# snuspl/rnb

Measured on AMD Instinct MI355X. Metric: videos/sec (whole node) + p50/p99 end-to-end latency, R(2+1)D-34 8-frame clips, higher is better.
Workload: dtype fp32

## Files before the change

csrc/conv_h3.hip:

```cpp
#include <type_traits>
#include <hip/hip_runtime.h>
#include <stdint.h>

#include "x6d_common.h"

#include "h3_common.h"

#ifdef H3_PHASE_TIMING
__device__ unsigned long long* h3_phase_buf;
#define H3_PHASE(k)                                                                   \
  do {                                                                                \
    if (threadIdx.x == 0 && (k) < 16) {                                               \
      h3_phase_buf[(size_t)blockIdx.x * 16 + (k)] = __builtin_amdgcn_s_memtime();     \
      if ((k) == 0) {                                                                 \
        unsigned hw, xcc;                                                             \
        asm volatile("s_getreg_b32 %0, hwreg(HW_REG_HW_ID)" : "=s"(hw));              \
        asm volatile("s_getreg_b32 %0, hwreg(HW_REG_XCC_ID)" : "=s"(xcc));            \
        h3_phase_buf[(size_t)blockIdx.x * 16 + 14] = ((unsigned long long)xcc << 32) | hw; \
      }                                                                               \
    }                                                                                 \
  } while (0)
#else
#define H3_PHASE(k) do {} while (0)
#endif
// ... 188 lines not shown

  const int nsteps16 = p.K_pad / 16;
  int s_begin = 0, s_end = nsteps16;
  if (p.KH == 1 && p.KW == 1 && p.KT > 1) {
    int n0, t0, n1, t1, hh, ww;
    f32_decode_row(p, p0, n0, t0, hh, ww);
    f32_decode_row(p, min(p0 + P_TILE, p.M) - 1, n1, t1, hh, ww);
    n0 = __builtin_amdgcn_readfirstlane(n0);
    n1 = __builtin_amdgcn_readfirstlane(n1);
    t0 = __builtin_amdgcn_readfirstlane(t0);
    t1 = __builtin_amdgcn_readfirstlane(t1);
    if (n0 == n1) {
      const int dt_lo = max(0, p.PT - t1 * p.ST);
      const int dt_hi = min(p.KT - 1, p.T - 1 + p.PT - t0 * p.ST);
      if (dt_hi >= dt_lo) {
        s_begin = (dt_lo * p.Cin_p) / 16;
        s_end = min(nsteps16, ((dt_hi + 1) * p.Cin_p + 15) / 16);
      }
    }
  }
  int t_begin = s_begin / 2, t_end = (s_end + 1) / 2;
  if (ksplit > 1) {
    const int len = t_end - t_begin;
    const int a = t_begin + (int)((long long)len * kidx / ksplit);
    const int b = t_begin + (int)((long long)len * (kidx + 1) / ksplit);
    t_begin = a;
    t_end = b;
  }
  const bool sums_mode = AFF && st.aff.sums != nullptr;
  if (t_begin < t_end) issue(t_begin, 0, !sums_mode);
  if constexpr (AFF) {
    if (sums_mode) {
      constexpr int NT = 64 * NW;
      constexpr int KG = (H3_AFF_SUMS_MAX + NT - 1) / NT;
      constexpr int KL = (H3_AFF_CLIPS * 64 + NT - 1) / NT;
      const int E = st.aff.nseg * p.Cin_p;
      double a1[KG + KL], a2[KG + KL];
      float gm[KG + KL], bt[KG + KL];
      int rows[KG + KL], dst[KG + KL];
#pragma unroll
      for (int k = 0; k < KG + KL; ++k) {
        int v = -1, c = 0;
        dst[k] = -1;
        if (k < KG) {
          const int i = threadIdx.x + k * NT;
          if (i < E) {
            v = i / p.Cin_p;
            c = i - v * p.Cin_p;
            dst[k] = i;
          }
        } else if (t_begin < t_end) {
          const int j = threadIdx.x + (k - KG) * NT;
          const int ci = j >> 6, sub = (j >> 5) & 1, ch = j & 15;
          const int clip = clip_lo + ci;
          if (j < H3_AFF_CLIPS * 64) {
            dst[k] = -2 - j;
            if (clip < p.N && clip * rows_per_clip < p0 + P_TILE) {
              v = st.in_seg[clip];
              c = ((2 * t_begin + sub) * 16) % p.Cin_p + ch;
            }
          }
        }
        const double* sp = st.aff.sums + (size_t)(v < 0 ? 0 : v) * 2 * st.aff.sums_c;
        a1[k] = v >= 0 ? sp[c] : 0.0;
        a2[k] = v >= 0 ? sp[st.aff.sums_c + c] : 0.0;
        gm[k] = v >= 0 ? st.aff.gamma[c] : 0.f;
        bt[k] = v >= 0 ? st.aff.beta[c] : 0.f;
        rows[k] = v >= 0 ? (st.aff.coffs[v + 1] - st.aff.coffs[v]) * st.aff.rpc : 0;
      }
      float* ssw = const_cast<float*>(st.in_ss);
      float* l0 = (float*)(lds + ACT_BYTES + W_BYTES);
#pragma unroll
      for (int k = 0; k < KG + KL; ++k) {
        if (dst[k] == -1) continue;
        float mu = 0.f, va = 0.f;
        if (rows[k] > 0) {
          const double m = a1[k] / (double)rows[k];
          mu = (float)m;
          va = (float)fmax(a2[k] / (double)rows[k] - m * m, 0.0);
        }
        const float sc = rows[k] > 0 ? gm[k] * rsqrtf(va + st.aff.eps) : 0.f;
        const float sh = rows[k] > 0 ? bt[k] - mu * sc : 0.f;
        if (dst[k] >= 0) {
          const int v = dst[k] / p.Cin_p, c = dst[k] - v * p.Cin_p;
          ssw[(size_t)v * 2 * p.Cin_p + c] = sc;
          ssw[(size_t)v * 2 * p.Cin_p + p.Cin_p + c] = sh;
        } else {
          const int j = -2 - dst[k];
          l0[j] = ((j >> 4) & 1) ? sh : sc;
        }
      }
    }
  }
  if (wave >= NW / 2) __builtin_amdgcn_s_setprio(1);
  x6d_wait_vm<0>();
  x6d_barrier();
  for (int t = t_begin; t < t_end; ++t) {
    const int it = t - t_begin;
    if (t + 1 < t_end) issue(t + 1, (it + 1) & 1);
    if constexpr (AFF) {
      const __attribute__((address_space(4))) int* tab =
          (const __attribute__((address_space(4))) int*)(p.ktab + t * 8);
      ey_cur[0] = tab[1];
      ey_cur[1] = tab[9];
    }
    H3B bf[TP];
#pragma unroll
    for (int tp = 0; tp < TP; ++tp) bf[tp] = load_b(it & 1, tp);
#pragma unroll
    for (int tc = 0; tc < TC; ++tc) mma_tc(it & 1, tc, bf);
    x6d_wait_vm<0>();
    x6d_barrier();
  }

  const float out_scale = st.out_scale;
#pragma unroll
  for (int tp = 0; tp < TP; ++tp)
#pragma unroll
    for (int tc = 0; tc < TC; ++tc) acc[tp][tc] *= out_scale;
  if (ksplit > 1) {
    const uint32_t ws_bytes = (uint32_t)min((long long)ksplit * p.M * p.Cout_p * 4, 0x7FFFFF00LL);
    const __amdgpu_buffer_rsrc_t wsr =
        __builtin_amdgcn_make_buffer_rsrc((void*)st.ws, (short)0, ws_bytes, 0x00020000);
#pragma unroll
    for (int tp = 0; tp < TP; ++tp) {
      const int m = p0 + (wp * TP + tp) * 16 + frow;
#pragma unroll
      for (int tc = 0; tc < TC; ++tc) {
        const int c = c0 + (wc * TC + tc) * 16 + 4 * fq;
        const uint32_t off = (m < p.M && c < p.Cout_p)
                                 ? (uint32_t)((((long long)kidx * p.M + m) * p.Cout_p + c) * 4)
                                 : X6D_INVALID;
        __builtin_amdgcn_raw_buffer_store_b128(acc[tp][tc], wsr, off, 0, 0);
      }
    }
    return;
  }
  x6d_epilogue<TP, TC, NW, C_TILE, ST>(p, st, acc, p0, p.M, p0 + P_TILE, c0, wp, wc, lane, lds,
                                       NS * BUF);
}

struct H3Band {
  int f, r0;
  int rows;
  int prows;
  int g0, u0;
  bool mixed;
};
template <bool ON>
static __device__ __forceinline__ int h3_per_chunk(int v) {
  if constexpr (ON) asm volatile("" : "+v"(v));
  return v;
}
template <bool STK, bool AFF>
static __device__ __forceinline__ void h3_patch_entry(const ConvF32Params& p, const H3Band& bd,
                                                      int it, int npx, int W2, int qd, int n0,
                                                      uint32_t& src, int& dst) {
  const int H = p.H, W = p.W;
  const int q = it >> 2;
  const int hy = q / W2, hx = q - hy * W2;
  const int x = hx - 1;
  int fy = bd.f, y = bd.r0 - 1 + hy;
  bool ok = it < 4 * npx && x >= 0 && x < W;
  if constexpr (STK) {
    const int u = bd.u0 - 1 + hy;
    fy = f32_fast_div(max(u, 0), p.mG, p.sG);
    y = u - fy * (H + 1);
    ok = ok && u >= 0 && y < H && fy < p.N * p.T;
  } else {
    ok = ok && y >= 0 && y < H;
  }
  src = ok ? (uint32_t)((((fy * H + y) * W + x) * p.Cin_p + qd * 4) * 4) : X6D_INVALID;
  dst = it < 4 * npx ? q * 128 : -1;
  if constexpr (STK && AFF) {
    if (ok) dst |= (f32_fast_div(fy, p.mTo, p.sTo) - n0) << 17;
  }
}
template <bool STK>
static __device__ __forceinline__ int h3_patch_pixel(const ConvF32Params& p, const H3Band& bd,
                                                     int pp, int R, int W2) {
  const int W = p.W;
  const int py = pp / W;
  if constexpr (STK) {
    const int hy = py + f32_fast_div(bd.g0 + py, p.mHo, p.sHo) - bd.f;
    return pp < bd.rows * W ? hy * W2 + (pp - py * W) : 0;
  } else {
    return pp < R * W ? py * W2 + (pp - py * W) : 0;
  }
}
static __device__ __forceinline__ void h3_entry_ss(const ConvF32Params& p, const X6DStats& st,
                                                   int n0, int d, int qd, int chunk,
                                                   x6f32x4& sc0, x6f32x4& sc1, x6f32x4& sh0,
                                                   x6f32x4& sh1) {
  const float* ss = st.in_ss + qd * 4 + chunk * 32 +
                    (size_t)st.in_seg[n0 + (d >> 17)] * 2 * p.Cin_p;
  sc0 = *(const x6f32x4*)ss;
  sc1 = *(const x6f32x4*)(ss + 16);
  sh0 = *(const x6f32x4*)(ss + p.Cin_p);
  sh1 = *(const x6f32x4*)(ss + p.Cin_p + 16);
}
template <bool STK, bool AFF>
static __device__ __forceinline__ H3Band h3_band(const ConvF32Params& p, const X6DStats& st,
                                                 int band, int R) {
  H3Band b;
  if constexpr (STK) {
    b.g0 = band * R;
    b.f = f32_fast_div(b.g0, p.mHo, p.sHo);
    b.r0 = b.g0 - b.f * p.H;
    b.rows = min(R, p.N * p.T * p.H - b.g0);
    const int fl = f32_fast_div(b.g0 + b.rows - 1, p.mHo, p.sHo);
    b.u0 = b.g0 + b.f;
    b.prows = b.rows + 2 + (fl - b.f);
    b.mixed = false;
    if constexpr (AFF)
      b.mixed = st.in_seg[f32_fast_div(b.f, p.mTo, p.sTo)] !=
                st.in_seg[f32_fast_div(fl, p.mTo, p.sTo)];
  } else {
    const int bands = (p.H + R - 1) / R;
    b.f = band / bands;
    b.r0 = (band - b.f * bands) * R;
    b.rows = min(R, p.H - b.r0);
    b.prows = R + 2;
    b.g0 = b.u0 = 0;
    b.mixed = false;
  }
  return b;
}

template <int NW, int TP, int TC, int HALO_PX, int G, bool ST, bool AFF, int MINB = 1,
          bool STK = false>
__global__ __launch_bounds__(64 * NW, MINB)
void conv_h3r_kernel(const ConvF32Params p, const X6DStats st) {
  constexpr int P_TILE = NW * TP * 16, C_TILE = TC * 16;
  constexpr int HALO_BYTES = HALO_PX * 128;
  constexpr int W_BYTES = C_TILE * 128;
  constexpr int W_TOTAL = C_TILE / 8;
  constexpr int W_INSTR = (W_TOTAL + NW - 1) / NW;
  constexpr int NT = 64 * NW;
  constexpr int ITEMS = (HALO_PX * 4 + NT - 1) / NT;
  static_assert(NT % 4 == 0, "a lane keeps one channel quad");
  __shared__ __attribute__((aligned(16))) char lds[HALO_BYTES + 2 * G * W_BYTES];
  char* const wbuf = lds + HALO_BYTES;

  const int lane = threadIdx.x & 63;
  const int wave = __builtin_amdgcn_readfirstlane(threadIdx.x >> 6);
  const int frow = lane & 15, fq = lane >> 4;
  const int W = p.W, H = p.H, W2 = p.W + 2;
  const int R = p.ST;

  const int nwg = gridDim.x, bid = blockIdx.x;
  const int q8 = nwg >> 3, r8 = nwg & 7, xcd = bid & 7;
  const int wgid = (xcd < r8 ? xcd * (q8 + 1) : r8 * (q8 + 1) + (xcd - r8) * q8) + (bid >> 3);
  const int ctile = wgid % p.n_ctiles;
  const int band = wgid / p.n_ctiles;
  const H3Band bd = h3_band<STK, AFF>(p, st, band, R);
  const int f = bd.f, r0 = bd.r0;
  const int c0 = ctile * C_TILE;
  const int p0 = (f * H + r0) * W;
  const int m_end = p0 + bd.rows * W;
  const int nck = p.Cin_p / 32;

  const x6d_u32x4 wr = x6d_rsrc(p.w, (uint32_t)(p.K_pad / 32) * (uint32_t)p.w_rows * 128u);
  auto issue_w = [&](int s, int buf) {
    const uint32_t wbase = ((uint32_t)s * (uint32_t)p.w_rows + (uint32_t)c0) * 128u;
#pragma unroll
    for (int j = 0; j < W_INSTR; ++j) {
      const int instr = (W_TOTAL % NW == 0) ? wave + NW * j : min(wave + NW * j, W_TOTAL - 1);
      x6d_dma16(wr, wbase + (uint32_t)(instr * 1024 + lane * 16),
                wbuf + buf * W_BYTES + instr * 1024);
    }
  };

  const __amdgpu_buffer_rsrc_t xr =
      __builtin_amdgcn_make_buffer_rsrc((void*)p.x, (short)0, p.x_bytes, 0x00020000);
  const int npx = bd.prows * W2;
  const int qd = threadIdx.x & 3;
  uint32_t src[ITEMS];
  int dst[ITEMS];
  static_assert(HALO_BYTES <= 1 << 17, "dst packs the entry's clip above bit 17");
  [[maybe_unused]] const int n0 = f32_fast_div(f, p.mTo, p.sTo);
#pragma unroll
  for (int i = 0; i < ITEMS; ++i) {
    h3_patch_entry<STK, AFF>(p, bd, threadIdx.x + i * NT, npx, W2, qd, n0, src[i], dst[i]);
  }
  const float* ssv = nullptr;
  if constexpr (AFF) ssv = st.in_ss + (size_t)st.in_seg[f / p.T] * 2 * p.Cin_p + qd * 4;
  const float in_scale = st.in_scale;
  constexpr int SB = MINB >= 4 ? 1 : AFF ? (NW > 8 ? 1 : (TP >= 4 ? 3 : ITEMS)) : ITEMS;
  auto stage = [&](int chunk, auto mix) {
    constexpr bool MIX = decltype(mix)::value;
    x6f32x4 sc0, sh0, sc1, sh1;
    if constexpr (AFF) {
      const float* ss = ssv + chunk * 32;
      sc0 = *(const x6f32x4*)ss;
      sc1 = *(const x6f32x4*)(ss + 16);
      sh0 = *(const x6f32x4*)(ss + p.Cin_p);
      sh1 = *(const x6f32x4*)(ss + p.Cin_p + 16);
    }
#pragma unroll
    for (int i0 = 0; i0 < ITEMS; i0 += SB) {
    x6f32x4 v0[SB], v1[SB];
#pragma unroll
    for (int k = 0; k < SB; ++k) {
      const int i = min(i0 + k, ITEMS - 1);
      const uint32_t o = src[i] == X6D_INVALID ? X6D_INVALID : src[i] + (uint32_t)(chunk * 128);
      v0[k] = __builtin_amdgcn_raw_buffer_load_b128(xr, o, 0, 0);
      v1[k] = __builtin_amdgcn_raw_buffer_load_b128(xr, o == X6D_INVALID ? o : o + 64u, 0, 0);
    }
#pragma unroll
    for (int k = 0; k < SB; ++k) {
      const int i = i0 + k;
      if (i >= ITEMS || dst[i] < 0) continue;
      const int d = h3_per_chunk<STK && AFF>(dst[i]), q = (d >> 7) & 1023;
      x6f32x4 a0 = v0[k], a1 = v1[k];
      if constexpr (AFF) {
        const float m = src[i] == X6D_INVALID ? 0.f : in_scale;
        if constexpr (MIX) h3_entry_ss(p, st, n0, d, qd, chunk, sc0, sc1, sh0, sh1);
#pragma unroll
        for (int j = 0; j < 4; ++j) {
          a0[j] = fmaxf(fmaf(a0[j], sc0[j], sh0[j]), 0.f) * m;
          a1[j] = fmaxf(fmaf(a1[j], sc1[j], sh1[j]), 0.f) * m;
        }
      } else {
        a0 *= in_scale;
        a1 *= in_scale;
      }
      uint32_t h[4], l[4];
      h3_split4(a0, h, l);
      h3_split4(a1, h + 2, l + 2);
      char* base = lds + (d & 0x1FFFF);
      *(wu32x4*)(base + (x6r_swz(2 * qd, q) << 4)) = (wu32x4){h[0], h[1], h[2], h[3]};
      *(wu32x4*)(base + (x6r_swz(2 * qd + 1, q) << 4)) = (wu32x4){l[0], l[1], l[2], l[3]};
    }
    }
  };

  int pq[TP];
#pragma unroll
  for (int tp = 0; tp < TP; ++tp) {
    const int pp = (wave * TP + tp) * 16 + frow;
    pq[tp] = h3_patch_pixel<STK>(p, bd, pp, R, W2);
  }

  x6f32x4 acc[TP][TC];
#pragma unroll
  for (int b = 0; b < TC; ++b) {
    const int c = c0 + b * 16 + 4 * fq;
    const float4 b4 = *(const float4*)(p.bias + c);
    const x6f32x4 bv = (x6f32x4){b4.x, b4.y, b4.z, b4.w} * st.acc_scale;
#pragma unroll
    for (int a = 0; a < TP; ++a) acc[a][b] = bv;
  }
  const int w_hh = x6_chunk(2 * fq, frow) << 4, w_ll = x6_chunk(2 * fq + 1, frow) << 4;

  constexpr int NG = (9 + G - 1) / G;
  auto issue_group = [&](int c, int g, int half) {
    for (int j = 0; j < G && g * G + j < 9; ++j) issue_w((g * G + j) * nck + c, half * G + j);
  };
  if (wave >= NW / 2) __builtin_amdgcn_s_setprio(1);
  H3_PHASE(0);
  issue_group(0, 0, 0);
  int half = 0;
  for (int c = 0; c < nck; ++c) {
    if constexpr (STK && AFF) {
      if (bd.mixed) stage(c, std::true_type{});
      else stage(c, std::false_type{});
    } else {
      stage(c, std::false_type{});
    }
    x6d_wait_vm<0>();
    x6d_barrier();
    H3_PHASE(1 + 2 * c);
#pragma unroll 1
    for (int g = 0; g < NG; ++g) {
      if (g + 1 < NG) issue_group(c, g + 1, half ^ 1);
      else if (c + 1 < nck) issue_group(c + 1, 0, half ^ 1);
      for (int j = 0; j < G && g * G + j < 9; ++j) {
        const int t = g * G + j;
        const int toff = (t / 3) * W2 + (t % 3);
        H3B bf[TP];
#pragma unroll
        for (int tp = 0; tp < TP; ++tp) {
          const int q = pq[tp] + toff;
          const char* base = lds + q * 128;
          bf[tp].h = *(const wu32x4*)(base + (x6r_swz(2 * fq, q) << 4));
          bf[tp].l = *(const wu32x4*)(base + (x6r_swz(2 * fq + 1, q) << 4));
        }
        const char* wb = wbuf + (half * G + j) * W_BYTES;
#pragma unroll
        for (int tc = 0; tc < TC; ++tc) {
          const char* wrow = wb + (tc * 16 + frow) * 128;
          const wu32x4 ah = *(const wu32x4*)(wrow + w_hh);
          const wu32x4 al = *(const wu32x4*)(wrow + w_ll);
#pragma unroll
          for (int tp = 0; tp < TP; ++tp) acc[tp][tc] = h3_mma(al, bf[tp].h, acc[tp][tc]);
#pragma unroll
          for (int tp = 0; tp < TP; ++tp) acc[tp][tc] = h3_mma(ah, bf[tp].l, acc[tp][tc]);
#pragma unroll
          for (int tp = 0; tp < TP; ++tp) acc[tp][tc] = h3_mma(ah, bf[tp].h, acc[tp][tc]);
        }
      }
      x6d_wait_vm<0>();
      x6d_barrier();
      half ^= 1;
    }
    H3_PHASE(2 + 2 * c);
  }
  x6d_epilogue<TP, TC, NW, C_TILE, ST, STK>(p, st, acc, p0, m_end, p0 + P_TILE, c0, wave, 0,
                                            lane, lds, HALO_BYTES + 2 * G * W_BYTES,
                                            st.out_scale);
  H3_PHASE(15);
}

template <int NW, int TP, int HALO_PX, int G, int MINB, bool ST, bool AFF, bool STK = false>
__global__ __launch_bounds__(64 * NW, MINB)
void conv_h3q_kernel(const ConvF32Params p, const X6DStats st) {
  constexpr int TC = 9;
  constexpr int P_TILE = NW * TP * 16, C_TILE = TC * 16;
  constexpr int HALO_BYTES = HALO_PX * 128;
  constexpr int W_BYTES = C_TILE * 128;
  constexpr int W_TOTAL = C_TILE / 8;
  constexpr int W_INSTR = (W_TOTAL + NW - 1) / NW;
  constexpr int NT = 64 * NW;
  constexpr int ITEMS = (HALO_PX * 4 + NT - 1) / NT;
  static_assert(TP <= TC - 1, "next-tap fragments are read during channel tiles 1..TP");
  __shared__ __attribute__((aligned(16))) char lds[HALO_BYTES + 2 * G * W_BYTES];
  char* const wbuf = lds + HALO_BYTES;

  const int lane = threadIdx.x & 63;
  const int wave = __builtin_amdgcn_readfirstlane(threadIdx.x >> 6);
  const int frow = lane & 15, fq = lane >> 4;
  const int W = p.W, H = p.H, W2 = p.W + 1;
  const int R = p.ST;

  const int nwg = gridDim.x, bid = blockIdx.x;
  const int q8 = nwg >> 3, r8 = nwg & 7, xcd = bid & 7;
  const int wgid = (xcd < r8 ? xcd * (q8 + 1) : r8 * (q8 + 1) + (xcd - r8) * q8) + (bid >> 3);
  const int ctile = wgid % p.n_ctiles;
  const int band = wgid / p.n_ctiles;
  const H3Band bd = h3_band<STK, AFF>(p, st, band, R);
  const int f = bd.f, r0 = bd.r0;
  const int c0 = ctile * C_TILE;
  const int p0 = (f * H + r0) * W;
  const int m_end = p0 + bd.rows * W;
  const int nck = p.Cin_p / 32;

  const x6d_u32x4 wr = x6d_rsrc(p.w, (uint32_t)(p.K_pad / 32) * (uint32_t)p.w_rows * 128u);
  auto issue_w = [&](int s, int buf) {
    const uint32_t wbase = ((uint32_t)s * (uint32_t)p.w_rows + (uint32_t)c0) * 128u;
#pragma unroll
    for (int j = 0; j < W_INSTR; ++j) {
      const int instr = (W_TOTAL % NW == 0) ? wave + NW * j : min(wave + NW * j, W_TOTAL - 1);
      x6d_dma16(wr, wbase + (uint32_t)(instr * 1024 + lane * 16),
                wbuf + buf * W_BYTES + instr * 1024);
    }
  };

  const __amdgpu_buffer_rsrc_t xr =
      __builtin_amdgcn_make_buffer_rsrc((void*)p.x, (short)0, p.x_bytes, 0x00020000);
  const int npx = bd.prows * W2 + 1;
  const int qd = threadIdx.x & 3;
  uint32_t src[ITEMS];
  int dst[ITEMS];
  static_assert(HALO_BYTES <= 1 << 17, "dst packs the entry's clip above bit 17");
  [[maybe_unused]] const int n0 = f32_fast_div(f, p.mTo, p.sTo);
#pragma unroll
  for (int i = 0; i < ITEMS; ++i) {
    h3_patch_entry<STK, AFF>(p, bd, threadIdx.x + i * NT, npx, W2, qd, n0, src[i], dst[i]);
  }
  const float* ssv = nullptr;
  if constexpr (AFF) ssv = st.in_ss + (size_t)st.in_seg[f / p.T] * 2 * p.Cin_p + qd * 4;
  const float in_scale = st.in_scale;
  constexpr int SB = AFF ? (NW == 4 && MINB == 1 ? 5 : 2) : 5;
  auto stage = [&](int chunk, auto mix) {
    constexpr bool MIX = decltype(mix)::value;
    x6f32x4 sc0, sh0, sc1, sh1;
    if constexpr (AFF) {
      const float* ss = ssv + chunk * 32;
      sc0 = *(const x6f32x4*)ss;
      sc1 = *(const x6f32x4*)(ss + 16);
      sh0 = *(const x6f32x4*)(ss + p.Cin_p);
      sh1 = *(const x6f32x4*)(ss + p.Cin_p + 16);
    }
#pragma unroll
    for (int i0 = 0; i0 < ITEMS; i0 += SB) {
      x6f32x4 v0[SB], v1[SB];
#pragma unroll
      for (int k = 0; k < SB; ++k) {
        const int i = min(i0 + k, ITEMS - 1);
        const uint32_t o = src[i] == X6D_INVALID ? X6D_INVALID : src[i] + (uint32_t)(chunk * 128);
        v0[k] = __builtin_amdgcn_raw_buffer_load_b128(xr, o, 0, 0);
        v1[k] = __builtin_amdgcn_raw_buffer_load_b128(xr, o == X6D_INVALID ? o : o + 64u, 0, 0);
      }
#pragma unroll
      for (int k = 0; k < SB; ++k) {
        const int i = i0 + k;
        if (i >= ITEMS || dst[i] < 0) continue;
        const int d = h3_per_chunk<STK && AFF>(dst[i]), q = (d >> 7) & 1023;
        x6f32x4 a0 = v0[k], a1 = v1[k];
        if constexpr (AFF) {
          const float m = src[i] == X6D_INVALID ? 0.f : in_scale;
          if constexpr (MIX) h3_entry_ss(p, st, n0, d, qd, chunk, sc0, sc1, sh0, sh1);
#pragma unroll
          for (int j = 0; j < 4; ++j) {
            a0[j] = fmaxf(fmaf(a0[j], sc0[j], sh0[j]), 0.f) * m;
            a1[j] = fmaxf(fmaf(a1[j], sc1[j], sh1[j]), 0.f) * m;
          }
        } else {
          a0 *= in_scale;
          a1 *= in_scale;
        }
        uint32_t h[4], l[4];
        h3_split4(a0, h, l);
        h3_split4(a1, h + 2, l + 2);
        char* base = lds + (d & 0x1FFFF);
        *(wu32x4*)(base + (x6r_swz(2 * qd, q) << 4)) = (wu32x4){h[0], h[1], h[2], h[3]};
        *(wu32x4*)(base + (x6r_swz(2 * qd + 1, q) << 4)) = (wu32x4){l[0], l[1], l[2], l[3]};
      }
    }
  };

  int pq[TP];
#pragma unroll
  for (int tp = 0; tp < TP; ++tp) {
    const int pp = (wave * TP + tp) * 16 + frow;
    pq[tp] = h3_patch_pixel<STK>(p, bd, pp, R, W2);
  }

  x6f32x4 acc[TP][TC];
#pragma unroll
  for (int b = 0; b < TC; ++b) {
    const int c = c0 + b * 16 + 4 * fq;
    const float4 b4 = *(const float4*)(p.bias + c);
    const x6f32x4 bv = (x6f32x4){b4.x, b4.y, b4.z, b4.w} * st.acc_scale;
#pragma unroll
    for (int a = 0; a < TP; ++a) acc[a][b] = bv;
  }
  const int w_hh = x6_chunk(2 * fq, frow) << 4, w_ll = x6_chunk(2 * fq + 1, frow) << 4;
  auto rd_bf = [&](H3B& b, int tap, int tp) {
    const int q = pq[tp] + (tap / 3) * W2 + (tap % 3);
    const char* base = lds + q * 128;
    b.h = *(const wu32x4*)(base + (x6r_swz(2 * fq, q) << 4));
    b.l = *(const wu32x4*)(base + (x6r_swz(2 * fq + 1, q) << 4));
  };
  auto rd_w = [&](wu32x4& ah, wu32x4& al, int jslot, int tc) {
    const char* wrow = wbuf + jslot * W_BYTES + (tc * 16 + frow) * 128;
    ah = *(const wu32x4*)(wrow + w_hh);
    al = *(const wu32x4*)(wrow + w_ll);
  };

  constexpr int NG = (9 + G - 1) / G;
  auto issue_group = [&](int c, int g, int half) {
    for (int j = 0; j < G && g * G + j < 9; ++j) issue_w((g * G + j) * nck + c, half * G + j);
  };
  H3_PHASE(0);
  issue_group(0, 0, 0);
  int half = 0;
  for (int c = 0; c < nck; ++c) {
    if constexpr (STK && AFF) {
      if (bd.mixed) stage(c, std::true_type{});
      else stage(c, std::false_type{});
    } else {
      stage(c, std::false_type{});
    }
    x6d_wait_vm<0>();
    x6d_barrier();
    H3_PHASE(1 + 2 * c);
#pragma unroll 1
    for (int g = 0; g < NG; ++g) {
      if (g + 1 < NG) issue_group(c, g + 1, half ^ 1);
      else if (c + 1 < nck) issue_group(c + 1, 0, half ^ 1);
      const int t0 = g * G;
      H3B bf[2][TP];
      wu32x4 wh[2], wl[2];
#pragma unroll
      for (int tp = 0; tp < TP; ++tp) rd_bf(bf[0][tp], t0, tp);
      rd_w(wh[0], wl[0], half * G, 0);
#pragma unroll
      for (int j = 0; j < G; ++j) {
        if (t0 + j >= 9) break;
        const bool more = j + 1 < G && t0 + j + 1 < 9;
#pragma unroll
        for (int tc = 0; tc < TC; ++tc) {
          const int cs = (j * TC + tc) & 1;
          if (tc + 1 < TC) rd_w(wh[cs ^ 1], wl[cs ^ 1], half * G + j, tc + 1);
          else if (more) rd_w(wh[cs ^ 1], wl[cs ^ 1], half * G + j + 1, 0);
          if (more && tc >= 1 && tc <= TP) rd_bf(bf[(j + 1) & 1][tc - 1], t0 + j + 1, tc - 1);
          const H3B (&b)[TP] = bf[j & 1];
#pragma unroll
          for (int tp = 0; tp < TP; ++tp) acc[tp][tc] = h3_mma(wl[cs], b[tp].h, acc[tp][tc]);
#pragma unroll
          for (int tp = 0; tp < TP; ++tp) acc[tp][tc] = h3_mma(wh[cs], b[tp].l, acc[tp][tc]);
#pragma unroll
          for (int tp = 0; tp < TP; ++tp) acc[tp][tc] = h3_mma(wh[cs], b[tp].h, acc[tp][tc]);
          __builtin_amdgcn_sched_barrier(0);
        }
      }
      x6d_wait_vm<0>();
      x6d_barrier();
      half ^= 1;
    }
    H3_PHASE(2 + 2 * c);
  }
  x6d_epilogue<TP, TC, NW, C_TILE, ST, STK>(p, st, acc, p0, m_end, p0 + P_TILE, c0, wave, 0,
                                            lane, lds, HALO_BYTES + 2 * G * W_BYTES,
                                            st.out_scale);
  H3_PHASE(15);
}

template <int NW, int TP, int TC, int HALO, int WB, int MINB, bool ST, bool AFF, int STK = 0>
__global__ __launch_bounds__(64 * NW, MINB)
void conv_h3t_kernel(const ConvF32Params p, const X6DStats st) {
  constexpr int ROWS = NW * TP * 16, C_TILE = TC * 16;
  static_assert(!STK || HALO == ROWS, "stacked: the patch is the block's T x P rows");
  constexpr int HALO_BYTES = HALO * 128;
  constexpr int TAP_BYTES = C_TILE * 128;
  constexpr int W_BYTES = 3 * TAP_BYTES;
  constexpr int W_TOTAL = W_BYTES / 1024;
  constexpr int W_INSTR = (W_TOTAL + NW - 1) / NW;
  constexpr int NT = 64 * NW;
  constexpr int ITEMS = (HALO * 4 + NT - 1) / NT;
  static_assert(NT % 4 == 0 && TAP_BYTES % 1024 == 0, "staging / DMA split");
  static_assert(TP <= TC * 3 - 1, "next-tap fragments are read during the channel tiles");
  __shared__ __attribute__((aligned(16))) char lds[HALO_BYTES + WB * W_BYTES];
  char* const wbuf = lds + HALO_BYTES;

  const int lane = threadIdx.x & 63;
  const int wave = __builtin_amdgcn_readfirstlane(threadIdx.x >> 6);
  const int frow = lane & 15, fq = lane >> 4;
  const int T = p.T, HW = p.H * p.W, P = p.ngroups;
  const int nck = (p.Cin_p + 31) / 32;

  const int nwg = gridDim.x, bid = blockIdx.x;
  const int q8 = nwg >> 3, r8 = nwg & 7, xcd = bid & 7;
  const int wgid = (xcd < r8 ? xcd * (q8 + 1) : r8 * (q8 + 1) + (xcd - r8) * q8) + (bid >> 3);
  const int ctile = wgid % p.n_ctiles;
  const int rest = wgid / p.n_ctiles;
  const int ptile = rest % p.n_ptiles;
  const int n = rest / p.n_ptiles;
  const int c0 = ctile * C_TILE, hw0 = ptile * P;

  const x6d_u32x4 wr = x6d_rsrc(p.w, (uint32_t)(p.K_pad / 32) * (uint32_t)p.w_rows * 128u);
  auto issue_w = [&](int c, int buf) {
#pragma unroll
    for (int j = 0; j < W_INSTR; ++j) {
      const int instr = (W_TOTAL % NW == 0) ? wave + NW * j : min(wave + NW * j, W_TOTAL - 1);
      const int k = instr / (TAP_BYTES / 1024), part = instr % (TAP_BYTES / 1024);
      const uint32_t s = (uint32_t)(k * nck + c);
      x6d_dma16(wr, (s * (uint32_t)p.w_rows + (uint32_t)c0) * 128u +
                        (uint32_t)(part * 1024 + lane * 16),
                wbuf + buf * W_BYTES + instr * 1024);
    }
  };

  const __amdgpu_buffer_rsrc_t xr =
      __builtin_amdgcn_make_buffer_rsrc((void*)p.x, (short)0, p.x_bytes, 0x00020000);
  const int nent = (T + 2) * P;
  const int qd = threadIdx.x & 3;
  uint32_t src[ITEMS];
  int dst[ITEMS];
  [[maybe_unused]] const int NG = p.N * HW, lgP = 31 - __clz(P);
  [[maybe_unused]] int n0 = 0, n1 = 0;
  [[maybe_unused]] bool mixed = false;
  if constexpr (STK) {
    n0 = __builtin_amdgcn_readfirstlane(f32_fast_div(hw0, p.mG, p.sG));
    n1 = __builtin_amdgcn_readfirstlane(f32_fast_div(min(hw0 + P, NG) - 1, p.mG, p.sG));
    if constexpr (AFF) mixed = st.in_seg[n0] != st.in_seg[n1];
#pragma unroll
// ... 473 lines not shown
                   const float* gamma, const float* beta, float eps, float* ss) {
  if (!sums || !coffs || !gamma || !beta || !ss) return -1;
  if (nseg <= 0 || C <= 0 || sums_c < C || rpc <= 0) return -2;
  BnAffSums a = {};
  a.sums = sums; a.sums_c = sums_c; a.nseg = nseg; a.rpc = rpc; a.coffs = coffs;
  a.gamma = gamma; a.beta = beta; a.eps = eps; a.ss = ss;
  g_bn_aff = a;
  g_bn_aff_used = 0;
  return 0;
}
void rnb_bn_aff_disarm() { g_bn_aff.ss = nullptr; }
int rnb_bn_aff_used() {
  const int u = g_bn_aff_used;
  g_bn_aff_used = 0;
  return u;
}

void rnb_h3_set_range_flag(int* flag) { g_h3_range_flag = flag; }
int* rnb_h3_range_flag() { return g_h3_range_flag; }

int rnb_conv_h3_num_configs() { return kNumH3Configs; }

int rnb_conv_h3_config_info(int id, int* p_tile, int* c_tile) {
  if (id < 0 || id >= kNumH3Configs) return -1;
  *p_tile = kH3Configs[id].p_tile;
  *c_tile = kH3Configs[id].c_tile;
  return 0;
}

int rnb_conv_h3_affine_ok(int config_id, int cin_p, int rows_per_clip) {
  if (config_id < 0 || config_id >= kNumH3Configs || cin_p % 16 != 0 || rows_per_clip <= 0)
    return 0;
  const int pt = kH3Configs[config_id].p_tile;
  return (pt - 1) / rows_per_clip + 2 <= H3_AFF_CLIPS ? 1 : 0;
}

int rnb_conv_h3_launch(const ConvF32Params* pp, int config_id, hipStream_t stream, double* sums,
                       const int* clip_seg, int stats_c, int ksplit, float* ws, float in_scale,
                       float out_scale, const float* in_ss, const int* in_seg) {
  if (config_id < 0 || config_id >= kNumH3Configs) return -1;
  ConvF32Params p = *pp;
  const ConvH3Config& cfg = kH3Configs[config_id];
  if (p.Cin_p % 4 != 0 || p.Cout_p % 4 != 0 || p.K_pad % 32 != 0) return -2;
  if (p.K_total > p.K_pad) return -3;
  if (p.M <= 0) return 0;
  if (p.y_stride < p.Cout_p || (p.res && p.res_stride < p.Cout_p)) return -4;
  if (p.y_stride % 4 != 0 || (p.res && p.res_stride % 4 != 0)) return -4;
  const long long xb = (long long)p.N * p.T * p.H * p.W * p.Cin_p * 4;
  if (xb > 0x7FFFFF00LL) return -5;
  if ((long long)p.M * p.y_stride * 4 > 0x7FFFFF00LL) return -6;
  if (p.res && (long long)p.M * p.res_stride * 4 > 0x7FFFFF00LL) return -6;
  if (p.KT > 8 || p.KH > 8 || p.KW > 8) return -10;
  if ((long long)(p.K_pad / 32) * p.w_rows * 128 > 0x7FFFFF00LL) return -11;
  if (!(in_scale > 0.f) || !(out_scale > 0.f)) return -15;
  p.x_bytes = (uint32_t)xb;
  f32_magic_div((uint32_t)p.Wo, &p.mWo, &p.sWo);
  f32_magic_div((uint32_t)p.Ho, &p.mHo, &p.sHo);
  f32_magic_div((uint32_t)p.To, &p.mTo, &p.sTo);
  p.row_mode = 0;
  p.n_ptiles = (p.M + cfg.p_tile - 1) / cfg.p_tile;
  p.n_ctiles = (p.Cout_p + cfg.c_tile - 1) / cfg.c_tile;
  const long long blocks = (long long)p.n_ptiles * p.n_ctiles;
  if (blocks > 0x7FFFFFFF) return -7;
  if (p.n_ctiles * cfg.c_tile > p.w_rows) return -8;
  if (!p.ktab) return -9;
  if (sums && (!clip_seg || stats_c < p.Cout_p)) return -12;
  X6DStats st;
  st.sums = sums;
  st.clip_seg = clip_seg;
  st.stats_c = stats_c;
  st.ksplit = 1;
  st.ws = nullptr;
  st.in_scale = in_scale;
  st.out_scale = out_scale;
  st.acc_scale = 1.f / out_scale;
  st.in_ss = in_ss;
  st.in_seg = in_seg;
  st.oflag = g_h3_range_flag;
  const bool aff = in_ss != nullptr;
  if (aff && (!in_seg || !rnb_conv_h3_affine_ok(config_id, p.Cin_p, p.To * p.Ho * p.Wo)))
    return -16;
  if (aff && g_bn_aff.ss == in_ss) {
    if (g_bn_aff.sums_c < p.Cin_p || (long long)g_bn_aff.nseg * p.Cin_p > H3_AFF_SUMS_MAX)
      return -18;
    st.aff = g_bn_aff;
    g_bn_aff_used = 1;
  }
  if (ksplit > 1) {
    if (!ws || ksplit > 16) return -14;
    st.ksplit = ksplit;
    st.ws = ws;
    hipLaunchKernelGGL(aff ? cfg.kernel_aff : cfg.kernel, dim3((unsigned)(blocks * ksplit)),
                       dim3(cfg.threads), 0, stream, p, st);
    return rnb_x6d_splitk_reduce(&p, &st, stream);
  }
  hipLaunchKernelGGL(aff ? (sums ? cfg.kernel_aff_st : cfg.kernel_aff)
                         : (sums ? cfg.kernel_st : cfg.kernel),
                     dim3((unsigned)blocks), dim3(cfg.threads), 0, stream, p, st);
  return (int)hipGetLastError();
}

typedef void (*ConvH3RKernel)(const ConvF32Params, const X6DStats);
struct ConvH3RConfig {
  int nw, tp, halo_px, q;
  ConvH3RKernel kernel[4];
  int halo_stk;
  ConvH3RKernel stacked[4];
};
#define H3RCFGM(NW, TP, HALO, G, MINB)                                             \
  {NW, TP, HALO, 0,                                                                \
   {conv_h3r_kernel<NW, TP, 9, HALO, G, false, false, MINB>,                       \
    conv_h3r_kernel<NW, TP, 9, HALO, G, true, false, MINB>,                        \
    conv_h3r_kernel<NW, TP, 9, HALO, G, false, true, MINB>,                        \
    conv_h3r_kernel<NW, TP, 9, HALO, G, true, true, MINB>},                        \
   HALO,                                                                           \
   {conv_h3r_kernel<NW, TP, 9, HALO, G, false, false, MINB, true>,                 \
    conv_h3r_kernel<NW, TP, 9, HALO, G, true, false, MINB, true>,                  \
    conv_h3r_kernel<NW, TP, 9, HALO, G, false, true, MINB, true>,                  \
    conv_h3r_kernel<NW, TP, 9, HALO, G, true, true, MINB, true>}}
#define H3RCFG(NW, TP, HALO, G) H3RCFGM(NW, TP, HALO, G, 1)
#define H3RCFG_PF(NW, TP, HALO, G)                                                 \
  {NW, TP, HALO, 0,                                                                \
   {conv_h3r_kernel<NW, TP, 9, HALO, G, false, false, 1>,                          \
    conv_h3r_kernel<NW, TP, 9, HALO, G, true, false, 1>,                           \
    conv_h3r_kernel<NW, TP, 9, HALO, G, false, true, 1>,                           \
    conv_h3r_kernel<NW, TP, 9, HALO, G, true, true, 1>},                           \
   0, {nullptr, nullptr, nullptr, nullptr}}
#define H3QCFG(NW, TP, HALO, HSTK, G, MINB)                                        \
  {NW, TP, HALO, 1,                                                                \
   {conv_h3q_kernel<NW, TP, HALO, G, MINB, false, false>,                          \
    conv_h3q_kernel<NW, TP, HALO, G, MINB, true, false>,                           \
    conv_h3q_kernel<NW, TP, HALO, G, MINB, false, true>,                           \
    conv_h3q_kernel<NW, TP, HALO, G, MINB, true, true>},                           \
   HSTK,                                                                           \
   {conv_h3q_kernel<NW, TP, HSTK, G, MINB, false, false, true>,                    \
    conv_h3q_kernel<NW, TP, HSTK, G, MINB, true, false, true>,                     \
    conv_h3q_kernel<NW, TP, HSTK, G, MINB, false, true, true>,                     \
    conv_h3q_kernel<NW, TP, HSTK, G, MINB, true, true, true>}}
#define H3QCFG_PF(NW, TP, HALO, G, MINB)                                           \
  {NW, TP, HALO, 1,                                                                \
   {conv_h3q_kernel<NW, TP, HALO, G, MINB, false, false>,                          \
    conv_h3q_kernel<NW, TP, HALO, G, MINB, true, false>,                           \
    conv_h3q_kernel<NW, TP, HALO, G, MINB, false, true>,                           \
    conv_h3q_kernel<NW, TP, HALO, G, MINB, true, true>},                           \
   0, {nullptr, nullptr, nullptr, nullptr}}
static const ConvH3RConfig kH3RConfigs[] = {
    H3RCFG(7, 4, 600, 1), H3RCFG_PF(14, 2, 600, 1), H3RCFG(7, 3, 480, 1),
    H3RCFG(7, 4, 600, 2), H3RCFG_PF(14, 2, 600, 2), H3RCFG(7, 3, 480, 2),
    H3QCFG(4, 7, 600, 600, 2, 1),
    H3QCFG(4, 4, 344, 352, 1, 2),
    H3QCFG_PF(8, 4, 640, 2, 1),
};

int rnb_conv_h3r_num_variants() { return (int)(sizeof(kH3RConfigs) / sizeof(kH3RConfigs[0])); }

static long long h3r_round_blocks(int variant) {
  static long long cache[16] = {};
  if (variant < 0 || variant >= 16) return 0;
  if (cache[variant] == 0) {
    int dev = 0, cus = 0, nb = 0;
    const ConvH3RConfig& cfg = kH3RConfigs[variant];
    if (hipGetDevice(&dev) == hipSuccess &&
        hipDeviceGetAttribute(&cus, hipDeviceAttributeMultiprocessorCount, dev) == hipSuccess &&
        hipOccupancyMaxActiveBlocksPerMultiprocessor(&nb, (const void*)cfg.kernel[0],
                                                     64 * cfg.nw, 0) == hipSuccess)
      cache[variant] = (long long)cus * nb;
    else
      (void)hipGetLastError();
    if (cache[variant] <= 0) cache[variant] = -1;
  }
  return cache[variant] > 0 ? cache[variant] : 0;
}

static int g_h3r_stack_small = 0;
void rnb_conv_h3r_stack_small(int on) { g_h3r_stack_small = on; }

static int h3r_rows(int variant, int H, int W, long long frames, int n_ctiles, bool* stacked) {
  const ConvH3RConfig& cfg = kH3RConfigs[variant];
  *stacked = false;
  if (H < 1 || W < 1) return 0;
  const int pitch = cfg.q ? W + 1 : W + 2, extra = cfg.q ? 1 : 0;
  const int R0 = cfg.nw * cfg.tp * 16 / W;
  const bool fits0 = R0 >= 1 && (R0 + 2) * pitch + extra <= cfg.halo_px;
  int R = R0;
  while (R >= 1 && (R + 2 + (R + H - 2) / H) * pitch + extra > cfg.halo_stk) --R;
  if (fits0 && (R < 1 || (H + R0 - 1) / R0 * R <= H)) return R0;
  if (fits0 && frames > 0 && !g_h3r_stack_small &&
      frames * ((H + R0 - 1) / R0) * n_ctiles <= h3r_round_blocks(variant))
    return R0;
  *stacked = R >= 1;
  return R >= 1 ? R : 0;
}

int rnb_conv_h3r_band_rows(int variant, int H, int W) {
  if (variant < 0 || variant >= rnb_conv_h3r_num_variants()) return 0;
  bool stacked;
  const int R = h3r_rows(variant, H, W, 0, 1, &stacked);
  return stacked ? R : (R < H ? R : H);
}

int rnb_conv_h3r_stacked(int variant, int N, int T, int H, int W, int Cout_p) {
  if (variant < 0 || variant >= rnb_conv_h3r_num_variants()) return 0;
  bool stacked;
  h3r_rows(variant, H, W, (long long)N * T, (Cout_p + 143) / 144, &stacked);
  return stacked ? 1 : 0;
}

int rnb_conv_h3r_pixels(int variant) {
  if (variant < 0 || variant >= rnb_conv_h3r_num_variants()) return 0;
  return kH3RConfigs[variant].nw * kH3RConfigs[variant].tp * 16;
}

long long rnb_conv_h3r_blocks(int variant, int N, int T, int H, int W, int Cout_p) {
  if (variant < 0 || variant >= rnb_conv_h3r_num_variants()) return 0;
  bool stacked;
  const long long frames = (long long)N * T;
  const int n_ctiles = (Cout_p + 143) / 144;
  const int R = h3r_rows(variant, H, W, frames, n_ctiles, &stacked);
  if (R == 0) return 0;
  const long long bands = stacked ? (frames * H + R - 1) / R : frames * ((H + R - 1) / R);
  return bands * n_ctiles;
}

int rnb_conv_h3r_occupancy(int variant, int stacked) {
  if (variant < 0 || variant >= rnb_conv_h3r_num_variants()) return -1;
  const ConvH3RConfig& cfg = kH3RConfigs[variant];
  int nb = 0;
  if (stacked && !cfg.stacked[0]) return -1;
  const hipError_t e = hipOccupancyMaxActiveBlocksPerMultiprocessor(
      &nb, (const void*)(stacked ? cfg.stacked[0] : cfg.kernel[0]), 64 * cfg.nw, 0);
  return e == hipSuccess ? nb : -(int)e;
}

int rnb_conv_h3r_launch(const ConvF32Params* pp, int variant, hipStream_t stream, double* sums,
                        const int* clip_seg, int stats_c, float in_scale, float out_scale,
                        const float* in_ss, const int* in_seg) {
  if (variant < 0 || variant >= rnb_conv_h3r_num_variants()) return -1;
  ConvF32Params p = *pp;
  const ConvH3RConfig& cfg = kH3RConfigs[variant];
  if (p.KT != 1 || p.KH != 3 || p.KW != 3 || p.PH != 1 || p.PW != 1 || p.PT != 0) return -2;
  if (p.SH != 1 || p.SW != 1 || p.ST != 1 || p.Cin_p % 32 != 0 || p.Cout_p % 4 != 0) return -2;
  if (p.K_pad < 9 * p.Cin_p || p.K_pad % 32 != 0) return -3;
  if (p.M <= 0) return 0;
  if (p.y_stride < p.Cout_p || p.y_stride % 4 != 0 || (p.res && (p.res_stride < p.Cout_p ||
                                                               p.res_stride % 4 != 0)))
    return -4;
  const long long xb = (long long)p.N * p.T * p.H * p.W * p.Cin_p * 4;
  if (xb > 0x7FFFFF00LL || (long long)p.M * p.y_stride * 4 > 0x7FFFFF00LL) return -5;
  if (p.res && (long long)p.M * p.res_stride * 4 > 0x7FFFFF00LL) return -6;
  bool stacked;
  const int R = h3r_rows(variant, p.H, p.W, (long long)p.N * p.T, (p.Cout_p + 143) / 144,
                         &stacked);
  if (R == 0) return -13;
  if ((long long)(p.K_pad / 32) * p.w_rows * 128 > 0x7FFFFF00LL) return -11;
  if (!(in_scale > 0.f) || !(out_scale > 0.f)) return -15;
  if (in_ss && !in_seg) return -16;
  p.x_bytes = (uint32_t)xb;
  f32_magic_div((uint32_t)p.Wo, &p.mWo, &p.sWo);
  f32_magic_div((uint32_t)p.Ho, &p.mHo, &p.sHo);
  f32_magic_div((uint32_t)p.To, &p.mTo, &p.sTo);
  f32_magic_div((uint32_t)p.H + 1u, &p.mG, &p.sG);
  p.ST = R;
  p.n_ctiles = (p.Cout_p + 143) / 144;
  if (p.n_ctiles * 144 > p.w_rows) return -8;
  const long long blocks = rnb_conv_h3r_blocks(variant, p.N, p.T, p.H, p.W, p.Cout_p);
  if (blocks > 0x7FFFFFFF) return -7;
  if (sums && (!clip_seg || stats_c < p.Cout_p)) return -12;
  X6DStats st;
  st.sums = sums;
  st.clip_seg = clip_seg;
  st.stats_c = stats_c;
  st.ksplit = 1;
  st.ws = nullptr;
  st.in_scale = in_scale;
  st.out_scale = out_scale;
  st.acc_scale = 1.f / out_scale;
  st.in_ss = in_ss;
  st.in_seg = in_seg;
  st.oflag = g_h3_range_flag;
  const int kid = (sums ? 1 : 0) + (in_ss ? 2 : 0);
  hipLaunchKernelGGL(stacked ? cfg.stacked[kid] : cfg.kernel[kid], dim3((unsigned)blocks),
                     dim3(64 * cfg.nw), 0, stream, p, st);
  return (int)hipGetLastError();
}

struct ConvH3TConfig {
  int rows, c_tile, halo, nw;
  void (*kernel)(const ConvF32Params, const X6DStats);
  void (*kernel_st)(const ConvF32Params, const X6DStats);
  void (*kernel_aff)(const ConvF32Params, const X6DStats);
  void (*kernel_aff_st)(const ConvF32Params, const X6DStats);
  int tp;
  void (*stacked[3][4])(const ConvF32Params, const X6DStats);
};
#define H3TSTK(NW, TP, TC, WB, MINB, STK)                                           \
  {conv_h3t_kernel<NW, TP, TC, NW * TP * 16, WB, MINB, false, false, STK>,          \
   conv_h3t_kernel<NW, TP, TC, NW * TP * 16, WB, MINB, true, false, STK>,           \
   conv_h3t_kernel<NW, TP, TC, NW * TP * 16, WB, MINB, false, true, STK>,           \
   conv_h3t_kernel<NW, TP, TC, NW * TP * 16, WB, MINB, true, true, STK>}
#define H3TPC(NW, TP, TC, HALO, WB, MINB)                                           \
  NW * TP * 16, TC * 16, HALO, NW,                                                   \
   conv_h3t_kernel<NW, TP, TC, HALO, WB, MINB, false, false>,                       \
   conv_h3t_kernel<NW, TP, TC, HALO, WB, MINB, true, false>,                        \
   conv_h3t_kernel<NW, TP, TC, HALO, WB, MINB, false, true>,                        \
   conv_h3t_kernel<NW, TP, TC, HALO, WB, MINB, true, true>, TP
#define H3TCFG(NW, TP, TC, HALO, WB, MINB)                                          \
  {H3TPC(NW, TP, TC, HALO, WB, MINB),                                               \
   {H3TSTK(NW, TP, TC, WB, MINB, 1), H3TSTK(NW, TP, TC, WB, MINB, 2),               \
    H3TSTK(NW, TP, TC, WB, MINB, 3)}}
#define H3TCFG_TP2(NW, TC, HALO, WB, MINB)                                          \
  {H3TPC(NW, 2, TC, HALO, WB, MINB),                                                \
   {H3TSTK(NW, 2, TC, WB, MINB, 1), {nullptr, nullptr, nullptr, nullptr},           \
    H3TSTK(NW, 2, TC, WB, MINB, 3)}}
static const ConvH3TConfig kH3TConfigs[] = {
    H3TCFG(8, 4, 4, 768, 2, 1), H3TCFG_TP2(8, 4, 512, 2, 1), H3TCFG_TP2(8, 8, 512, 2, 1),
    H3TCFG(4, 4, 4, 384, 1, 2),
};

int rnb_conv_h3t_num_variants() { return (int)(sizeof(kH3TConfigs) / sizeof(kH3TConfigs[0])); }

int rnb_conv_h3t_pixels(int variant, int T) {
  if (variant < 0 || variant >= rnb_conv_h3t_num_variants() || T < 2) return 0;
  const ConvH3TConfig& cfg = kH3TConfigs[variant];
  if (cfg.rows % T) return 0;
  const int P = cfg.rows / T;
  return (P % 16 == 0 && (T + 2) * P <= cfg.halo) ? P : 0;
}

static int g_h3t_form = 0;
void rnb_conv_h3t_form(int mode) { g_h3t_form = mode; }

static long long h3t_blocks(int variant, long long N, int T, int H, int W, int Cout_p,
                            int* stacked) {
  *stacked = 0;
  if (variant < 0 || variant >= rnb_conv_h3t_num_variants()) return 0;
  if (N < 1 || T < 2 || H < 1 || W < 1 || Cout_p < 1) return 0;
  const ConvH3TConfig& cfg = kH3TConfigs[variant];
  if (cfg.rows % T) return 0;
  const int P = cfg.rows / T;
  if (P % 16) return 0;
  const long long HW = (long long)H * W;
  const bool fits_pc = (T + 2) * P <= cfg.halo;
  const int stk_form = T == 2 ? 1 : T == cfg.tp ? 2 : T == 2 * cfg.tp ? 3 : 0;
  const bool fits_stk = stk_form && (P & (P - 1)) == 0 && N * HW + P <= 0x7FFFFFFFLL;
  if (!fits_pc && !fits_stk) return 0;
  const long long n_ctiles = (Cout_p + cfg.c_tile - 1) / cfg.c_tile;
  const long long pc = N * ((HW + P - 1) / P) * n_ctiles;
  const long long stk = (N * HW + P - 1) / P * n_ctiles;
  bool on;
  if (!fits_pc) on = true;
  else if (!fits_stk) on = false;
  else if (g_h3t_form != 0) on = g_h3t_form > 0;
  else on = stk < pc;
  *stacked = on ? stk_form : 0;
  return on ? stk : pc;
}

int rnb_conv_h3t_stacked(int variant, int N, int T, int H, int W, int Cout_p) {
  int stacked;
  h3t_blocks(variant, N, T, H, W, Cout_p, &stacked);
  return stacked ? 1 : 0;
}

long long rnb_conv_h3t_blocks(int variant, int N, int T, int H, int W, int Cout_p) {
  int stacked;
  return h3t_blocks(variant, N, T, H, W, Cout_p, &stacked);
}

int rnb_conv_h3t_occupancy(int variant, int stacked) {
  if (variant < 0 || variant >= rnb_conv_h3t_num_variants()) return -1;
  const ConvH3TConfig& cfg = kH3TConfigs[variant];
  int nb = 0;
  const hipError_t e = hipOccupancyMaxActiveBlocksPerMultiprocessor(
      &nb, (const void*)(stacked ? cfg.stacked[0][0] : cfg.kernel), 64 * cfg.nw, 0);
  return e == hipSuccess ? nb : -(int)e;
}

int rnb_conv_h3t_launch(const ConvF32Params* pp, int variant, hipStream_t stream, double* sums,
                        const int* clip_seg, int stats_c, float in_scale, float out_scale,
                        const float* in_ss, const int* in_seg) {
  if (variant < 0 || variant >= rnb_conv_h3t_num_variants()) return -1;
  ConvF32Params p = *pp;
  const ConvH3TConfig& cfg = kH3TConfigs[variant];
  if (p.KT != 3 || p.KH != 1 || p.KW != 1 || p.PT != 1 || p.PH != 0 || p.PW != 0) return -2;
  if (p.ST != 1 || p.SH != 1 || p.SW != 1 || p.Cin_p % 16 != 0 || p.Cout_p % 4 != 0) return -2;
  const int nck = (p.Cin_p + 31) / 32;
  if (p.K_pad != 3 * 32 * nck) return -3;
  if (p.M <= 0) return 0;
  if (p.M != p.N * p.T * p.H * p.W) return -3;
  if (p.y_stride < p.Cout_p || p.y_stride % 4 != 0 || (p.res && (p.res_stride < p.Cout_p ||
                                                               p.res_stride % 4 != 0)))
    return -4;
  const long long xb = (long long)p.N * p.T * p.H * p.W * p.Cin_p * 4;
  if (xb > 0x7FFFFF00LL || (long long)p.M * p.y_stride * 4 > 0x7FFFFF00LL) return -5;
  if (p.res && (long long)p.M * p.res_stride * 4 > 0x7FFFFF00LL) return -6;
  int stacked;
  const long long blocks = h3t_blocks(variant, p.N, p.T, p.H, p.W, p.Cout_p, &stacked);
  if (blocks == 0) return -13;
  const int P = cfg.rows / p.T;
  if ((long long)(p.K_pad / 32) * p.w_rows * 128 > 0x7FFFFF00LL) return -11;
  if (!(in_scale > 0.f) || !(out_scale > 0.f)) return -15;
  if (in_ss && !in_seg) return -16;
  p.x_bytes = (uint32_t)xb;
  p.ngroups = P;
  p.n_ctiles = (p.Cout_p + cfg.c_tile - 1) / cfg.c_tile;
  p.n_ptiles = stacked ? (int)(blocks / p.n_ctiles) : (p.H * p.W + P - 1) / P;
  f32_magic_div((uint32_t)(p.H * p.W), &p.mG, &p.sG);
  if (p.n_ctiles * cfg.c_tile > p.w_rows) return -8;
  if (blocks > 0x7FFFFFFF) return -7;
  if (sums && (!clip_seg || stats_c < p.Cout_p)) return -12;
  X6DStats st;
  st.sums = sums;
  st.clip_seg = clip_seg;
  st.stats_c = stats_c;
  st.ksplit = 1;
  st.ws = nullptr;
  st.in_scale = in_scale;
  st.out_scale = out_scale;
  st.acc_scale = 1.f / out_scale;
  st.in_ss = in_ss;
  st.in_seg = in_seg;
  st.oflag = g_h3_range_flag;
  const bool aff = in_ss != nullptr;
  hipLaunchKernelGGL(stacked ? cfg.stacked[stacked - 1][(sums ? 1 : 0) + (aff ? 2 : 0)]
                     : aff   ? (sums ? cfg.kernel_aff_st : cfg.kernel_aff)
                             : (sums ? cfg.kernel_st : cfg.kernel),
                     dim3((unsigned)blocks), dim3(64 * cfg.nw), 0, stream, p, st);
  return (int)hipGetLastError();
}

}
```

csrc/x6d_common.h:

```cpp
#pragma once
#include <hip/hip_runtime.h>
#include <stdint.h>

#include "conv_f32_common.h"
#include "x6_common.h"

#define X6D_INVALID 0xFFFFFFF0u

static __device__ __forceinline__ int x6d_swz(int c, int r) {
  return c ^ ((0x6C >> (2 * ((r >> 2) & 3))) & 3);
}

template <int N>
static __device__ __forceinline__ void x6d_wait_vm() {
  asm volatile("s_waitcnt vmcnt(%0)" ::"n"(N) : "memory");
}
static __device__ __forceinline__ void x6d_barrier() {
  asm volatile("s_waitcnt lgkmcnt(0)\n\ts_barrier" ::: "memory");
}

typedef unsigned int x6d_u32x4 __attribute__((ext_vector_type(4)));
static __device__ __forceinline__ x6d_u32x4 x6d_rsrc(const void* base, uint32_t bytes) {
  const uint64_t a = (uint64_t)base;
  return (x6d_u32x4){(uint32_t)a, (uint32_t)(a >> 32) & 0xFFFFu, bytes, 0x00020000u};
}
static __device__ __forceinline__ void x6d_dma16(const x6d_u32x4& rsrc, uint32_t voff,
                                                 const char* lds_dst) {
  asm volatile("buffer_load_dwordx4 %0, %1, 0 offen lds" ::"v"(voff), "s"(rsrc),
               "{m0}"((uint32_t)(uintptr_t)lds_dst)
               : "memory");
}

struct BnAffSums {
  const double* sums;
  int sums_c, nseg, rpc;
  const int* coffs;
  const float* gamma;
  const float* beta;
  float eps;
  float* ss;
};

struct X6DStats {
  double* sums;
  const int* clip_seg;
  int stats_c;
  int ksplit;
  float* ws;
  float in_scale, out_scale, acc_scale;
  const float* in_ss;
  const int* in_seg;
  int* oflag = nullptr;
  BnAffSums aff = {};
};

static __device__ __forceinline__ bool x6d_nonfinite(const x6f32x4& v) {
  return __builtin_amdgcn_classf(v[0], 0x207) | __builtin_amdgcn_classf(v[1], 0x207) |
         __builtin_amdgcn_classf(v[2], 0x207) | __builtin_amdgcn_classf(v[3], 0x207);
}

static __device__ __forceinline__ int x6r_swz(int slot, int q) {
  return slot ^ ((0x03701465 >> (4 * (q & 7))) & 7);
}

extern "C" int rnb_x6d_splitk_reduce(const ConvF32Params* p, const X6DStats* st,
                                     hipStream_t stream);

static __device__ __forceinline__ float x6d_dpp_add(float v, int ctrl_sel) {
  int t;
  const int iv = __float_as_int(v);
  switch (ctrl_sel) {
    case 0: t = __builtin_amdgcn_update_dpp(iv, iv, 0xB1, 0xF, 0xF, false); break;
    case 1: t = __builtin_amdgcn_update_dpp(iv, iv, 0x4E, 0xF, 0xF, false); break;
    case 2: t = __builtin_amdgcn_update_dpp(iv, iv, 0x141, 0xF, 0xF, false); break;
    default: t = __builtin_amdgcn_update_dpp(iv, iv, 0x140, 0xF, 0xF, false); break;
  }
  return v + __int_as_float(t);
}
static __device__ __forceinline__ float x6d_row16_sum(float v) {
  v = x6d_dpp_add(v, 0);
  v = x6d_dpp_add(v, 1);
  v = x6d_dpp_add(v, 2);
  return x6d_dpp_add(v, 3);
}

#define X6D_MSEG_MAX 8
template <int TP, int TC, int NW, int CT_ALL, bool ST, bool MSEG = false>
static __device__ __forceinline__ void x6d_epilogue(const ConvF32Params& p, const X6DStats& st,
                                                    x6f32x4 (&acc)[TP][TC], int p0, int m_end,
                                                    int p_hi, int c0, int wp, int wc, int lane,
                                                    char* lds, int lds_bytes,
                                                    float acc_mul = 1.f) {
  const int frow = lane & 15, fq = lane >> 4;
  const uint32_t y_bytes = (uint32_t)p.M * (uint32_t)p.y_stride * 4u;
  const __amdgpu_buffer_rsrc_t yr =
      __builtin_amdgcn_make_buffer_rsrc((void*)p.y, (short)0, y_bytes, 0x00020000);
  const bool has_res = p.res != nullptr;
  const __amdgpu_buffer_rsrc_t rr = __builtin_amdgcn_make_buffer_rsrc(
      (void*)(has_res ? p.res : p.y), (short)0,
      has_res ? (uint32_t)p.M * (uint32_t)p.res_stride * 4u : 0u, 0x00020000);
  bool bad = false;
  if constexpr (!ST) {
#pragma unroll
    for (int tp = 0; tp < TP; ++tp) {
      const int m = p0 + (wp * TP + tp) * 16 + frow;
      x6f32x4 r[TC];
#pragma unroll
      for (int tc = 0; tc < TC; ++tc) {
        const int c = c0 + (wc * TC + tc) * 16 + 4 * fq;
        const bool ok = has_res && m < m_end && c < p.Cout_p;
        r[tc] = has_res ? __builtin_amdgcn_raw_buffer_load_b128(
                              rr, ok ? (uint32_t)(m * p.res_stride + c) * 4u : X6D_INVALID, 0, 0)
                        : (x6f32x4){0.f, 0.f, 0.f, 0.f};
      }
#pragma unroll
      for (int tc = 0; tc < TC; ++tc) {
        const int c = c0 + (wc * TC + tc) * 16 + 4 * fq;
        const bool ok = m < m_end && c < p.Cout_p;
        x6f32x4 v = acc[tp][tc] * acc_mul + r[tc];
        if (st.oflag != nullptr && ok) bad |= x6d_nonfinite(v);
        if (p.relu) {
#pragma unroll
          for (int j = 0; j < 4; ++j) v[j] = fmaxf(v[j], 0.f);
        }
        __builtin_amdgcn_raw_buffer_store_b128(
            v, yr, ok ? (uint32_t)(m * p.y_stride + c) * 4u : X6D_INVALID, 0, 0);
      }
    }
  } else {
    constexpr int NT = 64 * NW;
    int na, nz, t_, h_, w_;
    f32_decode_row(p, p0, na, t_, h_, w_);
    f32_decode_row(p, min(p_hi, m_end) - 1, nz, t_, h_, w_);
    const int seg_lo = __builtin_amdgcn_readfirstlane(st.clip_seg[__builtin_amdgcn_readfirstlane(na)]);
    const int seg_hi = __builtin_amdgcn_readfirstlane(st.clip_seg[__builtin_amdgcn_readfirstlane(nz)]);
    const int nseg = seg_hi - seg_lo + 1;
    const bool in_lds = nseg * CT_ALL * 16 <= lds_bytes;
    const bool uni = MSEG ? nseg <= X6D_MSEG_MAX && in_lds : nseg == 1;
    [[maybe_unused]] int sl[MSEG ? TP : 1];
    if constexpr (MSEG) {
#pragma unroll
      for (int tp = 0; tp < TP; ++tp) {
        const int m = p0 + (wp * TP + tp) * 16 + frow;
        sl[tp] = m < m_end ? 0 : -1;
        if (nseg > 1 && uni && m < m_end) {
          int n;
          f32_decode_row(p, m, n, t_, h_, w_);
          sl[tp] = st.clip_seg[n] - seg_lo;
        }
      }
    }
    double* red = (double*)lds;
    if (in_lds)
      for (int i = threadIdx.x; i < nseg * CT_ALL * 2; i += NT) red[i] = 0.0;
    __syncthreads();
#pragma unroll
    for (int tc = 0; tc < TC; ++tc) {
      const int cl = (wc * TC + tc) * 16 + 4 * fq;
      const int c = c0 + cl;
      x6f32x4 r[TP];
#pragma unroll
      for (int tp = 0; tp < TP; ++tp) {
        const int m = p0 + (wp * TP + tp) * 16 + frow;
        const bool ok = has_res && m < m_end && c < p.Cout_p;
        r[tp] = has_res ? __builtin_amdgcn_raw_buffer_load_b128(
                              rr, ok ? (uint32_t)(m * p.res_stride + c) * 4u : X6D_INVALID, 0, 0)
                        : (x6f32x4){0.f, 0.f, 0.f, 0.f};
      }
      float s1[4] = {0.f, 0.f, 0.f, 0.f}, s2[4] = {0.f, 0.f, 0.f, 0.f};
#pragma unroll
      for (int tp = 0; tp < TP; ++tp) {
        const int m = p0 + (wp * TP + tp) * 16 + frow;
        const bool ok = m < m_end && c < p.Cout_p;
        x6f32x4 v = acc[tp][tc] * acc_mul + r[tp];
        if (st.oflag != nullptr && ok) bad |= x6d_nonfinite(v);
        if (p.relu) {
#pragma unroll
          for (int j = 0; j < 4; ++j) v[j] = fmaxf(v[j], 0.f);
        }
        __builtin_amdgcn_raw_buffer_store_b128(
            v, yr, ok ? (uint32_t)(m * p.y_stride + c) * 4u : X6D_INVALID, 0, 0);
        if constexpr (MSEG) r[tp] = v;
        if (!ok) continue;
#pragma unroll
        for (int j = 0; j < 4; ++j) {
          s1[j] += v[j];
          s2[j] = fmaf(v[j], v[j], s2[j]);
        }
      }
      if (uni) {
        if constexpr (MSEG) {
#pragma unroll 1
          for (int s = 0; s < nseg; ++s) {
            if (nseg > 1) {
#pragma unroll
              for (int j = 0; j < 4; ++j) s1[j] = s2[j] = 0.f;
#pragma unroll
              for (int tp = 0; tp < TP; ++tp) {
                if (sl[tp] != s) continue;
#pragma unroll
                for (int j = 0; j < 4; ++j) {
                  s1[j] += r[tp][j];
                  s2[j] = fmaf(r[tp][j], r[tp][j], s2[j]);
                }
// ... 72 lines not shown
```

rnb_amd/models/r2p1d/engine.py:

```python
from __future__ import annotations

import bisect
import os
import time
from typing import Dict, List, Optional, Sequence, Tuple

import torch

from ...ops.bn import BatchNormBatch
from ...ops.conv import ConvGeom, ConvLayer, StemConv, fold_bn, pad_to, CH_ALIGN
from ...ops.conv21 import FusedSTConv
from ...ops.conv_f32 import (F32_ALIGN, WINOT_MIN_T, ConvLayerF32, RangeGuard, full_range,
                              h3_enabled)
from ...ops.video import (Head, IN_CHANNELS_P, ndhwc_to_ncdhw, ncdhw_to_ndhwc,
                          packed_input_shape)
from .network import (DEFAULT_CLIP_LENGTH, LAYER_CHANNELS, LAYER_INPUT_CTHW,
                      LAYER_OUTPUT_CTHW, R2Plus1DLayerWrapper, SpatioTemporalConv,
                      check_clip_length, intermediate_channels, layer_geometry)

DEFAULT_BUCKETS = (1, 2, 3, 4, 5, 6, 8, 10, 12, 15, 16, 20, 24, 30, 32, 40, 45, 48,
                   60, 64, 80, 96, 128)


def geometric_buckets(max_clips: int, ratio: float = 1.125, dense: int = 8,
                      align: int = 4, fine_from: int = 0, fine_step: int = 8) -> List[int]:
    out = list(range(1, min(dense, max_clips) + 1))
    s = dense
    while s < max_clips:
        if fine_from and s >= fine_from:
            s = min(max_clips, (s // fine_step + 1) * fine_step)
        else:
            s = min(max_clips, max(s + align, -(-int(s * ratio) // align) * align))
        out.append(s)
    return sorted(set(out) | {max_clips})


def parse_bucket_step(step, max_clips: int) -> Optional[List[int]]:
    if step is None or step == "" or step == 0:
        return None
    if isinstance(step, str) and step.startswith("geo"):
        fine = int(step[3:]) if step[3:] else 0
        return geometric_buckets(max_clips, fine_from=96 if fine else 0, fine_step=fine or 8)
    n = int(step)
    return sorted(set(range(n, max_clips + 1, n)) | {1, max_clips})


def boundary_channels_p(layer_idx: int, dtype=torch.bfloat16) -> int:
    align = F32_ALIGN if dtype == torch.float32 else CH_ALIGN
    if layer_idx == 1:
        return align if dtype == torch.float32 else IN_CHANNELS_P
    return pad_to(LAYER_INPUT_CTHW[layer_idx][0], align)


def boundary_shape(layer_idx: int, n: int, dtype=torch.bfloat16,
                   clip_length: int = DEFAULT_CLIP_LENGTH) -> Tuple[int, ...]:
    c, t, h, w = layer_geometry(clip_length)[0][layer_idx]
    return (n, t, h, w, boundary_channels_p(layer_idx, dtype))


CONV_MAX_BYTES = 0x7FFFFF00
BN_MAX_ELEMS = 0x7FFFFFFF * 4


def activation_elems_per_clip(start_idx: int, end_idx: int, dtype=torch.float32,
                              clip_length: int = DEFAULT_CLIP_LENGTH) -> int:
    inp, out = layer_geometry(clip_length)
    f32 = dtype == torch.float32
    align = F32_ALIGN if f32 else CH_ALIGN
    worst = 0
    for idx in range(start_idx, end_idx + 1):
        c, t, h, w = inp[idx]
        cp = boundary_channels_p(idx, dtype)
        worst = max(worst, t * h * w * cp)
        cin, cout = LAYER_CHANNELS[idx]
        ho, wo = (h // 2, w // 2) if idx != 2 else (h, w)
        kernel = (3, 7, 7) if idx == 1 else (3, 3, 3)
        mids = [intermediate_channels(cin, cout, kernel)]
        if idx > 1:
            mids.append(intermediate_channels(cout, cout, kernel))
        midp = max(pad_to(m, 16 if f32 else align) for m in mids)
        worst = max(worst, t * ho * wo * midp)
        if out[idx] is not None:
            co, to, ho2, wo2 = out[idx]
            worst = max(worst, to * ho2 * wo2 * pad_to(co, align))
    return worst


def max_clips_limit(start_idx: int, end_idx: int, dtype=torch.float32,
                    clip_length: int = DEFAULT_CLIP_LENGTH) -> int:
    per = activation_elems_per_clip(start_idx, end_idx, dtype, clip_length)
    if dtype == torch.float32:
        return BN_MAX_ELEMS // per
    return CONV_MAX_BYTES // (2 * per)


def check_max_clips(max_clips: int, start_idx: int, end_idx: int, dtype=torch.float32,
                    clip_length: int = DEFAULT_CLIP_LENGTH) -> int:
    fit = max_clips_limit(start_idx, end_idx, dtype, clip_length)
    if int(max_clips) > fit:
        raise ValueError("max_clips %d is too large at clip_length %d for layers %d..%d (%s): "
                         "the largest activation passes the kernels' per-launch limit; the "
                         "largest max_clips that fits is %d"
                         % (max_clips, clip_length, start_idx, end_idx,
                            "fp32" if dtype == torch.float32 else "bf16", fit))
    return int(max_clips)


class PlanOp:
    __slots__ = ("kind", "layer", "src", "dst", "res", "bn", "bn_relu", "fuse")

    def __init__(self, kind, layer, src, dst, res=None, bn=None, bn_relu=False):
        self.kind, self.layer, self.src, self.dst, self.res = kind, layer, src, dst, res
        self.bn, self.bn_relu = bn, bn_relu
        self.fuse = None


class R2P1DEngine:
    def __init__(self, net: R2Plus1DLayerWrapper, device: torch.device,
                 backend: str = "hip", bn_mode: str = "eval", dtype=torch.bfloat16,
                 clip_length: int = DEFAULT_CLIP_LENGTH):
        self.clip_length = check_clip_length(clip_length)
        self.layer_in, self.layer_out = layer_geometry(self.clip_length)
        if backend not in ("hip", "torch", "module"):
            raise ValueError("unknown backend %r" % backend)
        if bn_mode not in ("eval", "batch"):
            raise ValueError("bn_mode must be 'eval' or 'batch'")
        dtype = _as_dtype(dtype)
        if dtype not in (torch.bfloat16, torch.float32):
            raise ValueError("dtype must be bfloat16 or float32, got %s" % dtype)
        self.net = net
        self.device = device
        self.backend = backend
        self.bn_mode = bn_mode
        self.dtype = dtype
        self.f32 = dtype == torch.float32
        self.pack_stem = os.environ.get("RNB_STEM_PACK", "1") != "0" and not self.f32
        self.start_idx, self.end_idx = net.start_idx, net.end_idx
        self.num_classes = getattr(net, "num_classes", 400)
        self.ops: List[PlanOp] = []
        self.head: Optional[Head] = None
        self._n = 0
        self.fused_choices: Dict[str, Optional[int]] = {}
        if backend == "module":
            self.module = net.to(device)
            self.module.train(bn_mode == "batch")
        else:
            self._build(net.res2plus1d)
            if self.end_idx == 5:
                self.head = Head(net.linear, device)
        self.range_guard = (RangeGuard() if backend == "hip" and self.f32 and h3_enabled()
                            and device.type == "cuda"
                            and os.environ.get("RNB_H3_GUARD", "1") != "0" else None)
        self._run_flat: Optional[torch.Tensor] = None
        self._run_pre: Optional[torch.Tensor] = None
        if (self.range_guard is not None and self.bn_mode == "batch"
                and os.environ.get("RNB_RUNNING_SHADOW", "1") != "0"):
            self._flatten_running()

    def _flatten_running(self) -> None:
        bns = [op.bn for op in self.ops if op.bn is not None]
        if not bns:
            return
        step = [pad_to(b.channels, 64) for b in bns]
        flat = torch.zeros(2 * sum(step), dtype=torch.float32, device=self.device)
        at = 0
        for b, s in zip(bns, step):
            for name in ("running_mean", "running_var"):
                view = flat[at:at + b.channels]
                view.copy_(getattr(b, name))
                setattr(b, name, view)
                at += s
        self._run_flat = flat

    def running_shadow(self) -> Optional[torch.Tensor]:
        return None if self._run_flat is None else torch.empty_like(self._run_flat)

    def _name(self) -> str:
        self._n += 1
        return "t%d" % self._n

    def _conv(self, conv: torch.nn.Conv3d, bn, relu: bool, name: str,
              src: str, dst: str, cin_pad: int = 0, cout_pad: int = 0) -> ConvLayer:
        w, b = fold_bn(conv.weight, conv.bias, bn)
        geom = ConvGeom(cin=conv.in_channels, cout=conv.out_channels,
                        kernel=tuple(conv.kernel_size), stride=tuple(conv.stride),
                        padding=tuple(conv.padding),
                        align=F32_ALIGN if self.f32 else CH_ALIGN,
                        cin_pad=cin_pad, cout_pad=cout_pad)
        T, H, W = self._thw[src]
        self._thw[dst] = geom.out_thw(T, H, W)
        nominal = geom
        kt, pt, st = geom.kernel[0], geom.padding[0], geom.stride[0]
        if T == 1 and kt == 2 * pt + 1 and st == 1 and kt > 1:
            w = w[:, :, pt:pt + 1].contiguous()
            geom = ConvGeom(cin=geom.cin, cout=geom.cout, kernel=(1,) + geom.kernel[1:],
                            stride=geom.stride, padding=(0,) + geom.padding[1:],
                            align=geom.align, cin_pad=cin_pad, cout_pad=cout_pad)
        if self.f32:
            layer = ConvLayerF32(w, b, geom, relu, self.device, name)
        elif self.pack_stem and StemConv.eligible(geom):
            layer = StemConv(w, b, geom, relu, self.device, name)
        else:
            layer = ConvLayer(w, b, geom, relu, self.device, name)
        layer.nominal_geom = nominal
        return layer

    def _stconv(self, st: SpatioTemporalConv, src: str, post_bn, relu: bool,
                res: Optional[str], name: str) -> str:
        mid = self._name()
        tc = st.temporal_conv
        T = self._thw[src][0]
        pad = 0
        if (self.f32 and tuple(tc.kernel_size) == (3, 1, 1) and tuple(tc.stride) == (1, 1, 1)
                and tuple(tc.padding) == (1, 0, 0) and tc.in_channels % 16
                and T >= WINOT_MIN_T and os.environ.get("RNB_PAD_MID16", "1") != "0"):
            pad = (tc.in_channels + 15) // 16 * 16
        self._append(st.spatial_conv, st.bn, True, None, name + ".spatial", src, mid,
                     cout_pad=pad)
        dst = self._name()
        self._append(st.temporal_conv, post_bn, relu, res, name + ".temporal", mid, dst,
                     cin_pad=pad)
        sp, tp = self.ops[-2], self.ops[-1]
        if (not self.f32 and sp.bn is None and tp.bn is None
                and FusedSTConv.eligible(sp.layer, tp.layer)):
            sp.fuse = FusedSTConv(sp.layer, tp.layer)
        return dst

    def _append(self, conv, bn, relu: bool, res: Optional[str], name: str, src: str, dst: str,
                cin_pad: int = 0, cout_pad: int = 0):
        if self.bn_mode == "batch" and bn is not None:
            layer = self._conv(conv, None, False, name, src, dst, cin_pad, cout_pad)
            if self.f32 and os.environ.get("RNB_BN_EPILOGUE_STATS", "1") == "1":
                layer.tune_with_stats = True
            bnop = BatchNormBatch(bn, layer.geom.cout_p, self.device)
            self.ops.append(PlanOp("conv", layer, src, dst, res, bn=bnop, bn_relu=relu))
        else:
            self.ops.append(PlanOp("conv", self._conv(conv, bn, relu, name, src, dst, cin_pad,
                                                      cout_pad), src, dst, res))

    def _block(self, blk, src: str, name: str) -> str:
        if blk.downsample:
            res = self._stconv(blk.downsampleconv, src, blk.downsamplebn, False, None,
                               name + ".downsample")
        else:
            res = src
        h = self._stconv(blk.conv1, src, blk.bn1, True, None, name + ".conv1")
        return self._stconv(blk.conv2, h, blk.bn2, True, res, name + ".conv2")

    def _build(self, body):
        cur = "x"
        self._thw = {"x": tuple(self.layer_in[self.start_idx][1:])}
        for idx in range(self.start_idx, self.end_idx + 1):
            if idx == 1:
                cur = self._stconv(body.conv1, cur, None, False, None, "conv1")
            else:
                layer = getattr(body, "conv%d" % idx)
                cur = self._block(layer.block1, cur, "conv%d.block1" % idx)
                for j, blk in enumerate(layer.blocks):
                    cur = self._block(blk, cur, "conv%d.blocks.%d" % (idx, j))
        self.out_name = cur
        last = {}
        for i, op in enumerate(self.ops):
            last[op.src] = i
            if op.res is not None:
                last[op.res] = i
        self._free_after = [[] for _ in self.ops]
        for name, i in last.items():
            if name not in ("x", self.out_name):
                self._free_after[i].append(name)
        uses = {}
        for op in self.ops:
            uses[op.src] = uses.get(op.src, 0) + 1
            if op.res is not None:
                uses[op.res] = uses.get(op.res, 0) + 1
        h3_defer = os.environ.get("RNB_H3_DEFER", "1") != "0"
        self._defer_ok = [
            i + 1 < len(self.ops) and op.bn is not None and op.bn_relu and op.res is None
            and self.f32 and uses.get(op.dst, 0) == 1 and self.ops[i + 1].src == op.dst
            and (getattr(self.ops[i + 1].layer, "winot_ok", False)
                 or (h3_defer and h3_enabled() and self.ops[i + 1].layer.geom.cin_p % 16 == 0))
            for i, op in enumerate(self.ops)]
        if self.bn_mode == "batch" and self.f32:
            for i, ok in enumerate(self._defer_ok):
                if ok and not getattr(self.ops[i + 1].layer, "winot_ok", False):
                    self.ops[i + 1].layer.tune_with_affine = True

    @property
    def in_channels_p(self) -> int:
        return boundary_channels_p(self.start_idx, self.dtype)

    def input_shape(self, n: int, packed: bool = False) -> Tuple[int, ...]:
        shape = boundary_shape(self.start_idx, n, self.dtype, self.clip_length)
        if not packed:
            return shape
        if not self.accepts_packed_input:
            raise ValueError("this engine's first op does not take a packed input")
        return packed_input_shape(*shape[:4])

    @property
    def accepts_packed_input(self) -> bool:
        return (self.backend != "module" and bool(self.ops)
                and isinstance(self.ops[0].layer, StemConv) and self.ops[0].bn is None)

    def output_shape(self, n: int) -> Tuple[int, ...]:
        if self.end_idx == 5:
            return (n, self.num_classes)
        return boundary_shape(self.end_idx + 1, n, self.dtype, self.clip_length)

    def output_dtype(self):
        return torch.float32 if self.end_idx == 5 else self.dtype

    def flops_per_clip(self) -> int:
        total = 0
        c, t, h, w = self.layer_in[self.start_idx]
        shapes = {"x": (t, h, w)}
        for op in self.ops:
            g = getattr(op.layer, "nominal_geom", op.layer.geom)
            T, H, W = shapes[op.src]
            total += g.flops(1, T, H, W)
            shapes[op.dst] = g.out_thw(T, H, W)
        if self.head is not None:
            total += 2 * self.head.channels * self.head.num_classes
        return total

    def conv_layers(self) -> List[ConvLayer]:
        return [op.layer for op in self.ops if op.kind == "conv"]

    def uses_h3(self) -> bool:
        from ...ops.conv_f32 import is_h3
        for layer in self.conv_layers():
            cfg = getattr(layer, "_config", None)
            if isinstance(cfg, dict) and any(is_h3(c) for c in cfg.values()):
                return True
        return False

    @property
    def supports_out_indirect(self) -> bool:
        return (self.backend == "hip" and self.f32 and self.bn_mode == "batch"
                and self.end_idx < 5 and bool(self.ops) and self.ops[-1].bn is not None)

    def forward(self, x: torch.Tensor, out: Optional[torch.Tensor] = None,
                packed: bool = False, clip_offsets=None,
                clip_offsets_dev: Optional[torch.Tensor] = None,
                out_indirect: Optional[torch.Tensor] = None,
                running_shadow: Optional[torch.Tensor] = None) -> torch.Tensor:
        if packed and not self.accepts_packed_input:
            raise ValueError("this engine's first op does not take a packed input")
        if self.backend == "module":
            cin = LAYER_INPUT_CTHW[self.start_idx][0]
            if x.dim() == 5 and x.shape[-1] == self.in_channels_p and x.shape[1] != cin:
                x = ndhwc_to_ncdhw(x, cin)
            y = self.module(x.to(self.device).float())
            if self.end_idx == 5:
                return y.float()
            return ncdhw_to_ndhwc(y, boundary_channels_p(self.end_idx + 1, self.dtype),
                                  dtype=self.dtype)
        if x.shape[0] == 0:
            return torch.zeros(self.output_shape(0), dtype=self.output_dtype(),
                               device=x.device)
        hip = self.backend == "hip"
        if running_shadow is not None and self._run_flat is not None:
            running_shadow.copy_(self._run_flat)
        if hip and self.range_guard is not None:
            self.range_guard.activate()
        bufs: Dict[str, torch.Tensor] = {"x": x}
        coffs = None
        defer = os.environ.get("RNB_BN_DEFER", "1") != "0"
        stats_fuse = os.environ.get("RNB_BN_EPILOGUE_STATS", "1") == "1"
        clip_seg = None
        if self.bn_mode == "batch" and clip_offsets_dev is not None and hip:
            coffs = clip_offsets_dev
            clip_offsets = None
        elif self.bn_mode == "batch" and clip_offsets is not None:
            clip_offsets = [int(o) for o in clip_offsets]
            if clip_offsets[0] != 0 or clip_offsets[-1] != x.shape[0]:
                raise ValueError("clip_offsets must span [0, %d]" % x.shape[0])
            if hip:
                coffs = torch.tensor(clip_offsets, dtype=torch.int32).to(x.device,
                                                                          non_blocking=True)
        from ...ops import bn as bn_mod
        batch_running = (hip and self.f32 and self.bn_mode == "batch"
                         and os.environ.get("RNB_BN_BATCH_RUNNING", "1") == "1")
        if batch_running:
            from ...ops.native import kernels
            kernels().bn_seg_set_defer_running(True)
            bn_mod._RUN_SINK[0] = []
        try:
            y, coffs = self._forward_ops(x, bufs, coffs, clip_offsets, hip, defer, stats_fuse,
                                         clip_seg, packed, out_indirect)
            if batch_running and bn_mod._RUN_SINK[0]:
                self._running_batched(bn_mod._RUN_SINK[0], coffs)
        finally:
            if batch_running:
                kernels().bn_seg_set_defer_running(False)
                bn_mod._RUN_SINK[0] = None
            if hip and self.range_guard is not None:
                from ...ops.native import kernels as _k
                _k().h3_set_range_flag(0)
        if self.head is not None:
            y = self.head.forward(y, out) if hip else self.head.forward_torch(y)
        elif out is not None:
            out.copy_(y)
            y = out
        return y

    def _running_batched(self, bns, coffs) -> None:
        from ...ops.bn import running_table_channels, running_table_key, running_update_table
        from ...ops.native import kernels
        key = running_table_key(bns)
        cache = self.__dict__.setdefault("_run_tables", {})
        tab = cache.get(key)
        if tab is None:
            tab = cache[key] = running_update_table(bns, self.device)
        kernels().bn_seg_running_batched(tab.data_ptr(), len(bns), running_table_channels(bns),
                                         coffs.data_ptr(), coffs.numel() - 1,
                                         torch.cuda.current_stream(self.device).cuda_stream)

    def _forward_ops(self, x, bufs, coffs, clip_offsets, hip, defer, stats_fuse, clip_seg,
                     packed, out_indirect):
        skip = False
        pending = None
        free_after = self._free_after
        from ...ops import bn as bn_mod
        aff_max = min(2304, int(os.environ.get("RNB_BN_AFF_SUMS_MAX", "2304"))) if hip else 0
        aff_videos = int(os.environ.get("RNB_BN_AFF_SUMS_VIDEOS", "1"))
        pending_aff = None
        from ...ops.native import kernels as _kn

        def consume(fn):
            nonlocal pending_aff
            if pending_aff is None:
                return fn()
            _kn().bn_aff_arm(*pending_aff)
            try:
                out = fn()
                if not _kn().bn_aff_used():
                    raise RuntimeError("a deferred BN's rows were left to a conv that did not "
                                       "compute them from the sums")
                return out
            finally:
                _kn().bn_aff_disarm()
                pending_aff = None

        for i, op in enumerate(self.ops):
            if skip:
                skip = False
                for name in free_after[i]:
                    bufs.pop(name, None)
                continue
            src = bufs[op.src]
            if hip and op.fuse is not None and op.fuse.use_for(src.shape):
                nxt = self.ops[i + 1]
                res = bufs[nxt.res] if nxt.res is not None else None
                bufs[nxt.dst] = op.fuse.forward_hip(src, res)
                skip = True
                for name in free_after[i]:
                    bufs.pop(name, None)
                continue
            res = bufs[op.res] if op.res is not None else None
            if op.bn is not None:
                if hip:
                    kw = {}
                    if pending is not None:
                        kw["in_affine"] = pending
                        pending = None
                    sums = None
                    if (self.f32 and stats_fuse
                            and op.layer.emits_output_stats(src.shape)):
                        if clip_seg is None:
                            clip_seg = self._clip_segments(coffs, x.shape[0], x.device)
                        nvid = 1 if coffs is None else coffs.numel() - 1
                        sums = op.bn.epilogue_sums(nvid, x.device)
                        kw["out_stats"] = (sums, clip_seg)
                    if coffs is None and self.f32:
                        coffs = torch.tensor([0, x.shape[0]], dtype=torch.int32,
                                             device=x.device)
                    y = consume(lambda: op.layer.forward_hip(src, None, **kw))
                    thw = y.shape[1] * y.shape[2] * y.shape[3]
                    deferred = (defer and self._defer_ok[i] and self.f32
                                and self.ops[i + 1].layer.accepts_input_affine(y.shape))
                    if deferred:
                        if clip_seg is None:
                            clip_seg = self._clip_segments(coffs, x.shape[0], x.device)
                        if (sums is not None and aff_max > 0 and bn_mod._RUN_SINK[0] is not None
                                and coffs.numel() - 1 <= aff_videos
                                and (coffs.numel() - 1) * op.bn.channels_p <= aff_max
                                and self.ops[i + 1].layer.takes_sums_affine(y.shape)):
                            ss, pending_aff = op.bn.aff_args(coffs, sums, thw)
                            bn_mod._RUN_SINK[0].append((op.bn, sums, thw))
                            pending = (ss, clip_seg)
                            self.bn_aff_sums = getattr(self, "bn_aff_sums", 0) + 1
                        else:
                            pending = (op.bn.scale_shift_f32(y, coffs, sums, rpc=thw), clip_seg)
                    else:
                        ind = out_indirect if i == len(self.ops) - 1 else None
                        from ...ops import bn as bn_mod
                        if (sums is not None and bn_mod._RUN_SINK[0] is not None
                                and os.environ.get("RNB_BN_APPLY_SUMS", "1") != "0"):
                            y = op.bn.apply_from_sums(y, res, op.bn_relu, out=y, segments=coffs,
                                                      sums=sums, rpc=thw, out_ind=ind)
                        else:
                            y = op.bn.forward_hip(y, res, op.bn_relu, out=y, segments=coffs,
                                                  sums=sums, rpc=thw, out_ind=ind)
                else:
                    y = op.layer.forward_torch(src, None, out_dtype=self.dtype)
                    y = op.bn.forward_torch(y, res, op.bn_relu, out_dtype=self.dtype,
                                            clip_offsets=clip_offsets)
            elif packed and i == 0:
                y = (op.layer.forward_hip(src, res, prepacked=True) if hip
                     else op.layer.forward_torch(src, res, prepacked=True))
            elif hip:
                if pending is not None:
                    aff = pending
                    y = consume(lambda: op.layer.forward_hip(src, res, in_affine=aff))
                    pending = None
                else:
                    y = op.layer.forward_hip(src, res)
            else:
                y = op.layer.forward_torch(src, res, out_dtype=self.dtype)
            bufs[op.dst] = y
            del src, res
            for name in free_after[i]:
                bufs.pop(name, None)
        return bufs[self.out_name], coffs

    __call__ = forward

    def forward_checked(self, x: torch.Tensor, out: Optional[torch.Tensor] = None,
                        clip_offsets=None) -> torch.Tensor:
        if self.range_guard is not None and self._run_flat is not None:
            if self._run_pre is None:
                self._run_pre = self.running_shadow()
        y = self.forward(x, out=out, clip_offsets=clip_offsets, running_shadow=self._run_pre)
        if self.range_guard is not None:
            torch.cuda.current_stream(self.device).synchronize()
            self.range_fallback(x, y, clip_offsets, pre=self._run_pre)
        return y

    def range_fallback(self, x: torch.Tensor, y: torch.Tensor, clip_offsets=None,
                       pre: Optional[torch.Tensor] = None) -> bool:
        g = self.range_guard
        if g is None or not g.tripped():
            return False
        g.reset()
        snap = None
        if pre is not None and self._run_flat is not None:
            self._run_flat.copy_(pre)
        else:
            bns = [op.bn for op in self.ops
                   if op.bn is not None and getattr(op.bn, "update_running", False)
                   and hasattr(op.bn, "running_mean")]
            snap = [(b, b.running_mean.clone(), b.running_var.clone()) for b in bns]
        with full_range():
            z = self.forward(x, clip_offsets=clip_offsets)
        for b, rm, rv in snap or ():
            b.running_mean.copy_(rm)
            b.running_var.copy_(rv)
        y.copy_(z)
        torch.cuda.current_stream(self.device).synchronize()
        g.reset()
        g.fallbacks += 1
        return True

    @staticmethod
    def _clip_segments(coffs: Optional[torch.Tensor], n: int, device) -> torch.Tensor:
        if coffs is None:
            return torch.zeros(n, dtype=torch.int32, device=device)
        idx = torch.arange(n, dtype=coffs.dtype, device=device)
        seg = torch.searchsorted(coffs[1:].contiguous(), idx, right=True)
        return seg.clamp_(max=coffs.numel() - 2).to(torch.int32).contiguous()

    def autotune(self, n: int, reps: int = 3) -> Dict[str, int]:
        assert self.backend == "hip"
        self.fused_choices = {}
        if self.range_guard is not None:
            from ...ops.native import kernels
            kernels().h3_set_range_flag(0)
        x = torch.randn(self.input_shape(n), device=self.device).to(self.dtype)
        bufs = {"x": x}
        chosen = {}
        for i, op in enumerate(self.ops):
            src = bufs[op.src]
            res = bufs[op.res] if op.res is not None else None
            if op.bn is not None:
                res = None
            chosen[op.layer.name] = op.layer.autotune(src, res, reps)
            bufs[op.dst] = op.layer.forward_hip(src, res)
            if self.f32:
                del src, res
                for name in self._free_after[i]:
                    bufs.pop(name, None)
        for i, op in enumerate(self.ops):
            if op.fuse is None or not op.fuse.supported(bufs[op.src].shape):
                continue
            nxt = self.ops[i + 1]
            src = bufs[op.src]
            res = bufs[nxt.res] if nxt.res is not None else None
            best, t_best = None, _time(
                lambda: nxt.layer.forward_hip(op.layer.forward_hip(src), res), reps)
            for v in op.fuse.VARIANTS:
                t = _time(lambda: op.fuse.forward_hip(src, res, variant=v), reps)
                if t < t_best:
                    best, t_best = v, t
            op.fuse.set_choice(src.shape, best)
            self.fused_choices[op.fuse.name] = best
        torch.cuda.synchronize(self.device)
        del bufs
        torch.cuda.empty_cache()
        return chosen


def _as_dtype(d):
    if isinstance(d, torch.dtype):
        return d
    names = {"bf16": torch.bfloat16, "bfloat16": torch.bfloat16, "fp32": torch.float32,
             "float32": torch.float32, "float": torch.float32}
    if d not in names:
        raise ValueError("unknown dtype %r (use 'fp32' or 'bf16')" % (d,))
    return names[d]


def _time(fn, reps: int) -> float:
    fn()
    start, end = torch.cuda.Event(enable_timing=True), torch.cuda.Event(enable_timing=True)
    start.record()
    for _ in range(reps):
        fn()
    end.record()
    end.synchronize()
    return start.elapsed_time(end) / reps


class GraphedEngine:

    def __init__(self, engine: R2P1DEngine, max_clips: int,
                 buckets: Sequence[int] = DEFAULT_BUCKETS, autotune: bool = True,
                 warmup: int = 1):
        assert engine.backend == "hip"
        if engine.bn_mode == "batch" and not engine.f32:
            raise ValueError("graphed bn_mode='batch' (per-video statistics) is fp32 only")
        self.engine = engine
        self.clip_length = engine.clip_length
        check_max_clips(max_clips, engine.start_idx, engine.end_idx, engine.dtype,
                        engine.clip_length)
        self.batch_bn = engine.bn_mode == "batch"
        self.offsets: Dict[int, torch.Tensor] = {}
        self._pinned = [torch.zeros(max_clips + 1, dtype=torch.int32).pin_memory()
                        if self.batch_bn and torch.cuda.is_available() else None
                        for _ in range(4)]
        self._pinned_ev = [None] * 4
        self._pinned_i = 0
        self.device = engine.device
        self.buckets = sorted({b for b in buckets if b < max_clips} | {max_clips})
        self.autotune = autotune
        self.warmup = warmup
        self.graphs: Dict[int, Tuple[torch.cuda.CUDAGraph, torch.Tensor, torch.Tensor]] = {}
        self.pool = None
        self.capture_s = 0.0
        self._last = None
        self._run_pre: Dict[int, torch.Tensor] = {}
        self._replays: Dict[int, int] = {}
        self.indirect_out = engine.supports_out_indirect and torch.cuda.is_available()
        self._dst: Dict[int, torch.Tensor] = {}
        self._dst_val: Dict[int, int] = {}
        self._pinned_dst = [torch.zeros(1, dtype=torch.int64).pin_memory()
                            if self.indirect_out else None for _ in range(4)]
        self._pinned_dst_ev = [None] * 4
        self._pinned_dst_i = 0

    @property
    def range_guard(self):
        return self.engine.range_guard

    def uses_h3(self) -> bool:
        return self.engine.uses_h3()

# ... 167 lines not shown
```

rnb_amd/ops/conv_f32.py:

```python
from __future__ import annotations

import math
import os
from typing import Dict, Optional, Tuple

import torch
import torch.nn.functional as F

from . import tuning
from .conv import ConvGeom, pad_to

F32_ALIGN = 4
F32_BK = 32
F32_ROW_SLACK = 256


_DEV_NAMES: Dict[int, str] = {}


def _device_name(device) -> str:
    if device is None or getattr(device, "type", "cpu") != "cuda":
        return "cpu"
    idx = device.index if device.index is not None else torch.cuda.current_device()
    if idx not in _DEV_NAMES:
# ... 195 lines not shown
    u32 = wmat.float().cpu()
    h = u32.bfloat16()
    r = u32 - h.float()
    m = r.bfloat16()
    lo = (r - m.float()).bfloat16()
    steps = K // 16

    def lay(t):
        return t.reshape(rows, steps, 4, 4)
    hh, mm, ll = lay(h), lay(m), lay(lo)
    chunks = torch.stack([torch.cat([hh, mm], -1), torch.cat([hh, ll], -1)], dim=-2)
    logical = chunks.reshape(rows, steps, 8, 8)
    sw = torch.tensor([_X6_S[(rr % 16) >> 1] for rr in range(rows)], dtype=torch.int64)
    idx = torch.arange(8, dtype=torch.int64)[None, :] ^ sw[:, None]
    phys = logical.gather(2, idx[:, None, :, None].expand_as(logical))
    return phys.permute(1, 0, 2, 3).contiguous().view(torch.int16)


_WINO_SWZ = (0, 2, 3, 1)


def h3w_weights(w: torch.Tensor, cin_p: int, cout: int, tc: int):
    co, ci = w.shape[:2]
    g = w.detach().double().cpu().reshape(co, ci, 3, 3)
    G = torch.tensor(_WINO_G, dtype=torch.float64)
    u = torch.einsum("ik,ockl,jl->ocij", G, g, G).reshape(co, ci, 16)
    ct = 16 * tc
    nb = (cout + ct - 1) // ct
    full = torch.zeros(nb * ct, cin_p, 16, dtype=torch.float64)
    full[:co, :ci] = u
    m = float(full.abs().max()) if full.numel() else 0.0
    sw = 0 if m == 0.0 else H3_W_TOP_LOG2 - int(math.floor(math.log2(m)))
    a = full * (2.0 ** sw)
    h = a.half()
    lo = (a - h.double()).half()

    def lay(t):
        return t.reshape(nb, ct, cin_p // 16, 4, 4, 16).permute(2, 0, 5, 1, 3, 4)
    logical = torch.cat([lay(h), lay(lo)], -1)
    s = torch.tensor([_WINO_SWZ[(r % 16) >> 2] for r in range(ct)], dtype=torch.int64)
    idx = torch.arange(4, dtype=torch.int64)[None, :] ^ s[:, None]
    phys = logical.gather(4, idx[None, None, None, :, :, None].expand_as(logical))
    return phys.contiguous().view(torch.int16), sw


def x6_enabled() -> bool:
    return os.environ.get("RNB_X6", "1") != "0"


def wino_default(temporal: bool) -> int:
    if temporal:
        return WINOTX_BASE if x6_enabled() else WINOT_DEFAULT
    return WINO_DEFAULT

_WINO_G = ((1.0, 0.0, 0.0), (0.5, 0.5, 0.5), (0.5, -0.5, 0.5), (0.0, 0.0, 1.0))


def winograd_weights(w: torch.Tensor, cout: int, tc: int, x6: bool = False) -> torch.Tensor:
    co, ci = w.shape[:2]
    g = w.detach().double().reshape(co, ci, 3, 3)
    G = torch.tensor(_WINO_G, dtype=torch.float64)
    u = torch.einsum("ik,ockl,jl->oc ij".replace(" ", ""), G, g, G)
    ct = 16 * tc
    nb = (cout + ct - 1) // ct
    full = torch.zeros(nb * ct, ci, 16, dtype=torch.float64)
    full[:co] = u.reshape(co, ci, 16)
    if x6:
        return x6_pack(full, tc)
    t = full.reshape(nb, ct, ci // 16, 16, 16).permute(2, 0, 4, 1, 3)
    return t.contiguous().float()


_X6_S = (0, 1, 0, 1, 6, 7, 6, 7)


def x6_pack(u: torch.Tensor, tc: int) -> torch.Tensor:
    rows, ci, X = u.shape
    ct = 16 * tc
    nb = rows // ct
    u32 = u.float()
    h = u32.bfloat16()
    r = u32 - h.float()
    m = r.bfloat16()
    lo = (r - m.float()).bfloat16()

    def lay(t):
        return t.reshape(nb, ct, ci // 16, 4, 4, X).permute(2, 0, 5, 1, 3, 4)
    hh, mm, ll = lay(h), lay(m), lay(lo)
    chunks = torch.stack([torch.cat([hh, mm], -1), torch.cat([hh, ll], -1)], dim=-2)
    logical = chunks.reshape(ci // 16, nb, X, ct, 8, 8)
    s = torch.tensor([_X6_S[(rr % 16) >> 1] for rr in range(ct)], dtype=torch.int64)
    idx = torch.arange(8, dtype=torch.int64)[None, :] ^ s[:, None]
    phys = logical.gather(4, idx[None, None, None, :, :, None].expand_as(logical))
    return phys.contiguous().view(torch.int16)


_WINO_G43 = ((1 / 4, 0.0, 0.0), (-1 / 6, -1 / 6, -1 / 6), (-1 / 6, 1 / 6, -1 / 6),
             (1 / 24, 1 / 12, 1 / 6), (1 / 24, -1 / 12, 1 / 6), (0.0, 0.0, 1.0))


def winograd_t_weights(w: torch.Tensor, cout: int, tc: int, x6: bool = False) -> torch.Tensor:
    co, ci = w.shape[:2]
    g = w.detach().double().reshape(co, ci, 3)
    G = torch.tensor(_WINO_G43, dtype=torch.float64)
    u = torch.einsum("ik,ock->oci", G, g)
    ct = 16 * tc
    nb = (cout + ct - 1) // ct
    full = torch.zeros(nb * ct, ci, 6, dtype=torch.float64)
    full[:co] = u
    if x6:
        return x6_pack(full, tc)
    t = full.reshape(nb, ct, ci // 16, 16, 6).permute(2, 0, 4, 1, 3)
    return t.contiguous().float()


class ConvLayerF32:

    dtype = torch.float32

    def __init__(self, weight: torch.Tensor, bias: torch.Tensor, geom: ConvGeom,
                 relu: bool, device: torch.device, name: str = ""):
        assert geom.align == F32_ALIGN, geom
        assert weight.shape == (geom.cout, geom.cin) + tuple(geom.kernel), (weight.shape, geom)
        self.geom = geom
        self.relu = bool(relu)
        self.name = name
        self.device = device
        kt, kh, kw = geom.kernel
        cin_p, cout_p = geom.cin_p, geom.cout_p
        self.k_total = kt * kh * kw * cin_p
        self.k_pad = pad_to(self.k_total, F32_BK)
        w = torch.zeros(geom.cout, kt, kh, kw, cin_p, dtype=torch.float32)
        w[..., :geom.cin] = weight.detach().float().permute(0, 2, 3, 4, 1)
        wmat = torch.zeros(cout_p + F32_ROW_SLACK, self.k_pad, dtype=torch.float32)
        wmat[:geom.cout, :self.k_total] = w.reshape(geom.cout, -1)
        b = torch.zeros(cout_p + F32_ROW_SLACK, dtype=torch.float32)
        b[:geom.cout] = bias.detach().float()
        self.wmat = wmat.to(device).contiguous()
        self.bias = b.to(device).contiguous()
        self.w_ref = weight.detach().float().to(device)
        self.b_ref = bias.detach().float().to(device)
        self._config: Dict[Tuple[int, int, int, int], int] = {}
        self._ktab: Dict[Tuple[int, int, int], torch.Tensor] = {}
        self.wino_ok = (geom.kernel == (1, 3, 3) and geom.stride == (1, 1, 1)
                        and geom.padding == (0, 1, 1) and geom.cin_p % 16 == 0)
        self.winot_ok = (geom.kernel == (3, 1, 1) and geom.stride == (1, 1, 1)
                         and geom.padding == (1, 0, 0) and geom.cin_p % 16 == 0)
        self.wino_ids = (WINO_SPATIAL if self.wino_ok else
                         WINO_TEMPORAL if self.winot_ok else set())
        self._wino_u: Dict[Tuple[int, int], torch.Tensor] = {}
        self.k16 = pad_to(self.k_total, 16)
        self.tune_with_stats = False
        self.tune_with_affine = False
        self._x6d = None
        self._h3d = None
        self._h3t = None
        self._h3stem = None
        self._x6k_ws: Dict[int, torch.Tensor] = {}
        self._h3w: Dict[int, Tuple[torch.Tensor, int]] = {}

    def ksplit_for(self, cid: int, x_shape) -> int:
        from .native import kernels
        if is_h3k(cid):
            pt, ct = kernels().h3_configs[H3K_CONFIGS[cid - H3K_BASE]]
            nsteps = self.k_pad // 32
        else:
            pt, ct = kernels().x6_configs[X6K_CONFIGS[cid - X6K_BASE]]
            nsteps = self.k16 // 16
        N, T, H, W, _ = x_shape
        To, Ho, Wo = self.geom.out_thw(T, H, W)
        blocks = math.ceil(N * To * Ho * Wo / pt) * math.ceil(self.geom.cout_p / ct)
        return int(max(1, min(16, X6K_TARGET_BLOCKS // max(blocks, 1), nsteps // 8)))

    def x6k_workspace(self, numel: int) -> torch.Tensor:
        ws = self._x6k_ws.get(numel)
        if ws is None:
            ws = self._x6k_ws[numel] = torch.empty(numel, dtype=torch.float32, device=self.device)
        return ws

    def x6d_buffers(self):
        if self._x6d is None:
            rows = self.geom.cout_p + X6_ROW_SLACK
            w = torch.zeros(rows, self.k16, dtype=torch.float32)
            w[:self.geom.cout, :self.k_total] = self.wmat[:self.geom.cout, :self.k_total].cpu()
            b = torch.zeros(rows, dtype=torch.float32)
            b[:self.geom.cout] = self.bias[:self.geom.cout].cpu()
            self._x6d = (x6_direct_weights(w).to(self.device), b.to(self.device))
        return self._x6d

    def h3d_buffers(self):
        if self._h3d is None:
            rows = self.geom.cout_p + X6_ROW_SLACK
            w = torch.zeros(rows, self.k_pad, dtype=torch.float32)
            w[:self.geom.cout, :self.k_total] = self.wmat[:self.geom.cout, :self.k_total].cpu()
            b = torch.zeros(rows, dtype=torch.float32)
            b[:self.geom.cout] = self.bias[:self.geom.cout].cpu()
            sw = h3_weight_scale_log2(w)
            self._h3d = (h3_direct_weights(w, sw).to(self.device), b.to(self.device),
                         float(2.0 ** H3_IN_LOG2), float(2.0 ** -(H3_IN_LOG2 + sw)))
        return self._h3d

    @property
    def h3t_k_pad(self) -> int:
        return 3 * 32 * ((self.geom.cin_p + 31) // 32)

    def h3t_buffers(self):
        if self.geom.cin_p % 32 == 0:
            return self.h3d_buffers()
        if self._h3t is None:
            rows, cin, kp = self.geom.cout_p + X6_ROW_SLACK, self.geom.cin_p, self.h3t_k_pad
            w = torch.zeros(rows, kp, dtype=torch.float32)
            tap = kp // 3
            src = self.wmat[:self.geom.cout, :self.k_total].cpu()
            for k in range(3):
                w[:self.geom.cout, k * tap:k * tap + cin] = src[:, k * cin:(k + 1) * cin]
            b = torch.zeros(rows, dtype=torch.float32)
            b[:self.geom.cout] = self.bias[:self.geom.cout].cpu()
            sw = h3_weight_scale_log2(w)
            self._h3t = (h3_direct_weights(w, sw).to(self.device), b.to(self.device),
                         float(2.0 ** H3_IN_LOG2), float(2.0 ** -(H3_IN_LOG2 + sw)))
        return self._h3t

    def h3t_ok(self, x_shape=None) -> bool:
        return (self.winot_ok and self.geom.cin_p % 16 == 0
                and (x_shape is None or x_shape[1] >= 2))

    def h3t_fits(self, variant: int, x_shape) -> bool:
        from .native import kernels
        if x_shape is None:
            return True
        N, T, H, W, _ = x_shape
        return kernels().conv_h3t_blocks(variant, N, T, H, W, self.geom.cout_p) > 0

    def h3p_ok(self, x_shape=None) -> bool:
        if not self.h3t_ok(x_shape) or os.environ.get("RNB_H3P", "1") == "0":
            return False
        from .native import kernels
        if x_shape is None:
            return kernels().conv_h3p_ok(8, 16, 16, self.geom.cin_p, self.geom.cout_p)
        _, T, H, W, _ = x_shape
        return kernels().conv_h3p_ok(T, H, W, self.geom.cin_p, self.geom.cout_p)

    def h3u_fits(self, variant: int, x_shape) -> bool:
        from .native import kernels
        return x_shape is None or kernels().conv_h3u_pixels(variant, x_shape[1]) > 0

    def wino_u(self, tc: int, m: int = 2, co0: int = 0, nco: Optional[int] = None,
               x6: bool = False) -> torch.Tensor:
        nco = self.geom.cout_p - co0 if nco is None else nco
        key = (m, tc, co0, nco, x6)
        u = self._wino_u.get(key)
        if u is None:
            fn = {2: winograd_weights, -4: winograd_t_weights}[m]
            w = self.w_ref[co0:co0 + nco].cpu()
            if w.shape[1] < self.geom.cin_p:
                w = torch.cat([w, w.new_zeros((w.shape[0], self.geom.cin_p - w.shape[1])
                                              + tuple(w.shape[2:]))], dim=1)
            u = self._wino_u[key] = fn(w, nco, tc, x6=x6).to(self.device)
        return u

    def h3w_u(self, tc: int) -> Tuple[torch.Tensor, int]:
        got = self._h3w.get(tc)
        if got is None:
            u, sw = h3w_weights(self.w_ref, self.geom.cin_p, self.geom.cout_p, tc)
            got = self._h3w[tc] = (u.to(self.device), sw)
        return got

    def _launch_h3w(self, x, y, residual, cid, stream, in_affine=None, out_stats=None):
        from .native import WinoParams, kernels
        g = self.geom
        N, T, H, W, C = x.shape
        if not (self.wino_ok and x.is_contiguous() and y.is_contiguous() and C == g.cin_p
                and tuple(y.shape[:4]) == (N, T, H, W) and y.shape[-1] >= g.cout_p
                and (residual is None or (residual.is_contiguous()
                                          and tuple(residual.shape[:4]) == (N, T, H, W)
                                          and residual.shape[-1] >= g.cout_p))):
            raise ValueError("%s: h3w operands do not match the conv geometry: x %s y %s"
                             % (self.name, tuple(x.shape), tuple(y.shape)))
        k = kernels()
        variant = cid - H3W_BASE
        u, sw = self.h3w_u(k.conv_h3w_tc(variant))
        p = WinoParams()
        p.x, p.u = x.data_ptr(), u.data_ptr()
        p.bias = self.bias.data_ptr()
        p.res = residual.data_ptr() if residual is not None else None
        p.y = y.data_ptr()
        p.F, p.H, p.W, p.Cin = N * T, H, W, C
        p.Cout = g.cout_p
        p.y_stride = y.shape[-1]
        p.res_stride = residual.shape[-1] if residual is not None else 0
        p.relu = 1 if self.relu else 0
        p.clip_frames = T
        if in_affine is not None:
            ss, aseg = in_affine
            if (ss.dim() != 3 or ss.shape[1:] != (2, C) or ss.dtype != torch.float32
                    or not ss.is_contiguous() or aseg.dtype != torch.int32
                    or aseg.numel() != N or not aseg.is_contiguous()):
                raise ValueError("%s: input BN scale/shift %s / clip_seg %s do not match x %s"
                                 % (self.name, tuple(ss.shape), tuple(aseg.shape),
                                    tuple(x.shape)))
            p.in_ss, p.clip_seg = ss.data_ptr(), aseg.data_ptr()
        out_seg = 0
        if out_stats is not None:
            sums, clip_seg = out_stats
            if (sums.dim() != 3 or sums.shape[1] != 2 or sums.shape[2] < g.cout_p
                    or sums.dtype != torch.float64 or not sums.is_contiguous()
# ... 72 lines not shown
        g = self.geom
        N, T, H, W, C = x.shape
        if not (x.is_contiguous() and y.is_contiguous() and C == g.cin_p
                and tuple(y.shape[:4]) == (N, T, H, W) and y.shape[-1] >= g.cout_p
                and (residual is None or (residual.is_contiguous()
                                          and tuple(residual.shape[:4]) == (N, T, H, W)
                                          and residual.shape[-1] >= g.cout_p))):
            raise ValueError("%s: Winograd operands do not match the conv geometry: x %s y %s "
                             "res %s" % (self.name, tuple(x.shape), tuple(y.shape),
                                         None if residual is None else tuple(residual.shape)))
        p = WinoParams()
        p.x = x.data_ptr()
        if ft:
            p.F, p.H, p.W = N, T, H * W
        else:
            p.F, p.H, p.W = N * T, H, W
        p.Cin = C
        assert p.F * p.H * p.W * C == x.numel()
        p.y_stride = y.shape[-1]
        p.res_stride = residual.shape[-1] if residual is not None else 0
        p.relu = 1 if self.relu else 0
        if in_affine is not None:
            ss, clip_seg = in_affine
            if not ft:
                raise ValueError("%s: deferred input BN needs the temporal Winograd kernel"
                                 % self.name)
            if (ss.dim() != 3 or ss.shape[1:] != (2, C) or ss.dtype != torch.float32
                    or not ss.is_contiguous() or clip_seg.dtype != torch.int32
                    or clip_seg.numel() != N):
                raise ValueError("%s: input BN scale/shift %s / clip_seg %s do not match x %s"
                                 % (self.name, tuple(ss.shape), tuple(clip_seg.shape),
                                    tuple(x.shape)))
            p.in_ss, p.clip_seg = ss.data_ptr(), clip_seg.data_ptr()
        sums = None
        if out_stats is not None:
            sums, clip_seg = out_stats
            if (sums.dim() != 3 or sums.shape[1] != 2 or sums.shape[2] < g.cout_p
                    or sums.dtype != torch.float64 or not sums.is_contiguous()
                    or clip_seg.dtype != torch.int32 or clip_seg.numel() != N
                    or (in_affine is not None and in_affine[1].data_ptr() != clip_seg.data_ptr())):
                raise ValueError("%s: output BN sums %s / clip_seg %s do not match y %s"
                                 % (self.name, tuple(sums.shape), tuple(clip_seg.shape),
                                    tuple(y.shape)))
            p.clip_seg = clip_seg.data_ptr()
            p.clip_frames, p.stats_c = T, sums.shape[2]
        k = kernels()
        launch = ((k.winot_x6 if ft else k.wino_x6) if x6 else
                  (k.winot_f32 if ft else k.wino_f32))
        for co0, nco, tc, variant in self.wino_parts(cid):
            u = self.wino_u(tc, m, co0, nco, x6=x6)
            assert u.shape[0] * 16 == C and u.shape[1] * 16 * tc >= nco
            p.u = u.data_ptr()
            p.bias = self.bias.data_ptr() + 4 * co0
            p.res = residual.data_ptr() + 4 * co0 if residual is not None else None
            p.y = y.data_ptr() + 4 * co0
            p.Cout = nco
            if sums is not None:
                p.out_stats = sums.data_ptr() + 8 * co0
            launch(p, variant, stream.cuda_stream)

    def out_shape(self, x_shape) -> Tuple[int, int, int, int, int]:
        N, T, H, W, _ = x_shape
        To, Ho, Wo = self.geom.out_thw(T, H, W)
        return (N, To, Ho, Wo, self.geom.cout_p)

    def ktab(self, T: int, H: int, W: int, device) -> torch.Tensor:
        key = (T, H, W)
        tab = self._ktab.get(key)
        if tab is None:
            g = self.geom
            kt, kh, kw = g.kernel
            if max(kt, kh, kw) > 8:
                raise ValueError("kernel extent > 8 not supported by the gather table")
            k = torch.arange(self.k_pad // 4, dtype=torch.int64) * 4
            tap, c = k // g.cin_p, k % g.cin_p
            dw, dh, dt = tap % kw, (tap // kw) % kh, tap // (kw * kh)
            delta = (((dt * H + dh) * W + dw) * g.cin_p + c) * 4
            req = (1 << dt) | (1 << (8 + dh)) | (1 << (16 + dw))
            valid = k < self.k_total
            delta = torch.where(valid, delta, torch.zeros_like(delta))
            req = torch.where(valid, req, torch.full_like(req, -(1 << 31)))
            tab = torch.stack([delta, req], dim=1).to(torch.int32).contiguous().to(device)
            self._ktab[key] = tab
        return tab

    def params(self, x: torch.Tensor, y: torch.Tensor, residual: Optional[torch.Tensor],
               n0: int = 0, n1: Optional[int] = None, x6: bool = False, h3: bool = False,
               h3t: bool = False):
        from .native import ConvParams
        g = self.geom
        N, T, H, W, C = x.shape
        n1 = N if n1 is None else n1
        if C != g.cin_p:
            raise ValueError("%s: input has %d channels, expected %d" % (self.name, C, g.cin_p))
        _, To, Ho, Wo, Co = y.shape
        xs, ys = T * H * W * C * 4, To * Ho * Wo * Co * 4
        p = ConvParams()
        p.x = x.data_ptr() + n0 * xs
        p.w, p.bias = self.wmat.data_ptr(), self.bias.data_ptr()
        if residual is not None:
            p.res = residual.data_ptr() + n0 * To * Ho * Wo * residual.shape[-1] * 4
        else:
            p.res = None
        p.y = y.data_ptr() + n0 * ys
        p.N, p.T, p.H, p.W, p.Cin_p = n1 - n0, T, H, W, g.cin_p
        p.To, p.Ho, p.Wo = To, Ho, Wo
        p.KT, p.KH, p.KW = g.kernel
        p.ST, p.SH, p.SW = g.stride
        p.PT, p.PH, p.PW = g.padding
        p.Cout_p = g.cout_p
        p.y_stride = Co
        p.res_stride = residual.shape[-1] if residual is not None else 0
        p.K_total, p.K_pad = self.k_total, self.k_pad
        p.M = (n1 - n0) * To * Ho * Wo
        p.relu = 1 if self.relu else 0
        p.w_rows = self.wmat.shape[0]
        p.ktab = self.ktab(T, H, W, x.device).data_ptr()
        p.row_mode = 0
        if h3t:
            wx, bx, _, _ = self.h3t_buffers()
            p.w, p.bias = wx.data_ptr(), bx.data_ptr()
            p.K_pad, p.w_rows = self.h3t_k_pad, bx.shape[0]
        elif h3:
            wx, bx, _, _ = self.h3d_buffers()
            p.w, p.bias = wx.data_ptr(), bx.data_ptr()
            p.K_pad, p.w_rows = self.k_pad, bx.shape[0]
        elif x6:
            wx, bx = self.x6d_buffers()
            p.w, p.bias = wx.data_ptr(), bx.data_ptr()
            p.K_pad, p.w_rows = self.k16, bx.shape[0]
        return p

    def chunk_clips(self, x_shape, y_shape, res_stride: int = 0) -> int:
        from .native import kernels
        limit = kernels().f32_max_bytes
        _, T, H, W, C = x_shape
        _, To, Ho, Wo, Co = y_shape
        per = max(T * H * W * C, To * Ho * Wo * max(Co, res_stride)) * 4
        return max(1, limit // per)

    def heuristic_config(self, M: int) -> int:
        from .native import kernels
        best, best_cost = 0, None
        cp = self.geom.cout_p
        for cid, (pt, ct) in enumerate(kernels().f32_configs):
            nblk = math.ceil(M / pt) * math.ceil(cp / ct)
            work = math.ceil(M / pt) * pt * math.ceil(cp / ct) * ct
            waves = math.ceil(nblk / 512.0)
            cost = work * (1.0 + 8.0 / pt + 8.0 / ct) * (waves * 512.0 / max(nblk, 1)) ** 0.5
            if best_cost is None or cost < best_cost:
                best, best_cost = cid, cost
        return best

    def _tune_key(self, x_shape, device) -> str:
        kind = ("f32st" if self.tune_with_stats else "f32") + \
            ("aff" if self.tune_with_affine else "")
        return tuning.make_key(kind, self.geom, tuple(x_shape[:4]), _device_name(device))

    def config_for(self, x_shape) -> int:
        cid = self._config_for(x_shape)
        if _FULL_RANGE[0] and is_h3(cid):
            N, T, H, W, _ = x_shape
            To, Ho, Wo = self.geom.out_thw(T, H, W)
            cid = self.heuristic_config(N * To * Ho * Wo)
            if os.environ.get("RNB_WINOGRAD", "1") != "0":
                if self.wino_ok:
                    cid = wino_default(False)
                elif self.winot_ok and T >= WINOT_MIN_T:
                    cid = wino_default(True)
        return cid

    def _config_for(self, x_shape) -> int:
        key = tuple(x_shape[:4])
        cid = self._config.get(key)
        if cid is None:
            tkey = self._tune_key(x_shape, self.device)
            cid = tuning.get(tkey)
            if cid is None:
                N, T, H, W, _ = x_shape
                cid = tuning.nearest(tkey, N * T * H * W)
            if cid is not None and cid in WINO_ALL and cid not in self.wino_ids:
                cid = None
            if cid is not None and is_x6d(cid) and not is_h3(cid) and not x6_enabled():
                cid = None
            if cid is not None and is_h3(cid) and not h3_enabled():
                cid = None
            if (cid is not None and cid not in WINO_ALL and not is_x6d(cid)
                    and cid >= len(_configs())):
                cid = None
            if cid is None:
                N, T, H, W, _ = x_shape
                To, Ho, Wo = self.geom.out_thw(T, H, W)
                cid = self.heuristic_config(N * To * Ho * Wo)
                if os.environ.get("RNB_WINOGRAD", "1") != "0":
                    if self.wino_ok:
                        cid = wino_default(False)
                    elif self.winot_ok and T >= WINOT_MIN_T:
                        cid = wino_default(True)
            self._config[key] = cid
        return cid

    def h3r_ok(self, x_shape=None) -> bool:
        return self.wino_ok and self.geom.cin_p % 32 == 0

    def h3r_fits(self, variant: int, x_shape, efficient: bool = True) -> bool:
        if x_shape is None:
            return True
        from .native import kernels
        _, T, H, W, _ = x_shape
        rows = kernels().conv_h3r_band_rows(variant, H, W)
        if rows < 1:
            return False
        return not efficient or 2 * rows * W >= kernels().conv_h3r_pixels(variant)

    def h3stem_ok(self, x_shape=None) -> bool:
        g = self.geom
        return (tuple(g.kernel) == (1, 7, 7) and tuple(g.stride) == (1, 2, 2)
                and tuple(g.padding) == (0, 3, 3) and g.cin_p == 4)

    def h3stem_fits(self, variant: int, x_shape, efficient: bool = True) -> bool:
        if x_shape is None:
            return True
        from .native import kernels
        _, T, H, W, _ = x_shape
        _, Ho, Wo = self.geom.out_thw(T, H, W)
        rows = kernels().conv_h3stem_rows(variant, Ho, Wo)
        if rows < 1:
            return False
        return not efficient or 2 * rows * Wo >= H3STEM_PIXELS[variant]

    def h3stem_buffers(self):
        if self._h3stem is None:
            rows = self.geom.cout_p + X6_ROW_SLACK
            w = torch.zeros(rows, 7 * 32, dtype=torch.float32)
            src = self.wmat[:self.geom.cout, :self.k_total].cpu()
            for dy in range(7):
                w[:self.geom.cout, dy * 32:dy * 32 + 28] = src[:, dy * 28:(dy + 1) * 28]
            b = torch.zeros(rows, dtype=torch.float32)
            b[:self.geom.cout] = self.bias[:self.geom.cout].cpu()
            sw = h3_weight_scale_log2(w)
            self._h3stem = (h3_direct_weights(w, sw).to(self.device), b.to(self.device),
                            float(2.0 ** H3_IN_LOG2), float(2.0 ** -(H3_IN_LOG2 + sw)))
        return self._h3stem

    def h3s_ok(self, x_shape=None) -> bool:
        g = self.geom
        return (tuple(g.kernel) == (1, 3, 3) and tuple(g.stride) == (1, 2, 2)
                and tuple(g.padding) == (0, 1, 1) and g.cin_p % 32 == 0)

    def h3s_fits(self, variant: int, x_shape, efficient: bool = True) -> bool:
        if x_shape is None:
            return True
        from .native import kernels
        _, T, H, W, _ = x_shape
        _, Ho, Wo = self.geom.out_thw(T, H, W)
        rows = kernels().conv_h3s_rows(variant, Ho, Wo)
        if rows < 1:
            return False
        return not efficient or 2 * rows * Wo >= H3S_PIXELS[variant]

    def affine_ok(self, cid: int, x_shape) -> bool:
        if is_h3s(cid) or is_h3stem(cid):
            return False
        if (cid in WINO_TEMPORAL or is_h3r(cid) or is_h3t(cid) or is_h3u(cid)
                or is_h3p(cid) or is_h3w(cid)):
            return True
        if not is_h3(cid):
            return False
        from .native import kernels
        conf = H3K_CONFIGS[cid - H3K_BASE] if is_h3k(cid) else cid - H3D_BASE
        _, T, H, W, _ = x_shape
        To, Ho, Wo = self.geom.out_thw(T, H, W)
        return kernels().conv_h3_affine_ok(conf, self.geom.cin_p, To * Ho * Wo)

    def _launch_all(self, x, y, residual, cid, stream, in_affine=None, out_stats=None):
        from .native import kernels
        k = kernels()
        N = x.shape[0]
        if cid in WINO_ALL:
            step = self.chunk_clips(x.shape, y.shape,
                                    residual.shape[-1] if residual is not None else 0)
            for n0 in range(0, N, step):
                n1 = min(N, n0 + step)
                aff = None if in_affine is None else (in_affine[0], in_affine[1][n0:n1])
                ost = None if out_stats is None else (out_stats[0], out_stats[1][n0:n1])
                self._launch_wino(x[n0:n1], y[n0:n1],
                                  residual[n0:n1] if residual is not None else None, cid,
                                  stream, aff, ost)
            return
        if is_h3w(cid):
            step = self.chunk_clips(x.shape, y.shape,
                                    residual.shape[-1] if residual is not None else 0)
            for n0 in range(0, N, step):
                n1 = min(N, n0 + step)
                aff = None if in_affine is None else (in_affine[0], in_affine[1][n0:n1])
                ost = None if out_stats is None else (out_stats[0], out_stats[1][n0:n1])
                self._launch_h3w(x[n0:n1], y[n0:n1],
                                 residual[n0:n1] if residual is not None else None, cid,
                                 stream, aff, ost)
            return
        x6 = is_x6d(cid)
        if (in_affine is not None and not is_h3(cid)) or (out_stats is not None and not x6):
            raise ValueError("%s: fused input BN needs a temporal Winograd or h3 config, "
                             "output BN statistics a Winograd, x6 or h3 direct config"
                             % self.name)
        if in_affine is not None:
            ss, aseg = in_affine
            C = x.shape[-1]
            if (ss.dim() != 3 or ss.shape[1:] != (2, C) or ss.dtype != torch.float32
                    or not ss.is_contiguous() or aseg.dtype != torch.int32
                    or aseg.numel() != N or not aseg.is_contiguous()):
                raise ValueError("%s: input BN scale/shift %s / clip_seg %s do not match x %s"
                                 % (self.name, tuple(ss.shape), tuple(aseg.shape),
                                    tuple(x.shape)))
        if out_stats is not None:
            sums, clip_seg = out_stats
            if (sums.dim() != 3 or sums.shape[1] != 2 or sums.shape[2] < self.geom.cout_p
                    or sums.dtype != torch.float64 or not sums.is_contiguous()
                    or clip_seg.dtype != torch.int32 or clip_seg.numel() != N
                    or not clip_seg.is_contiguous()):
                raise ValueError("%s: output BN sums %s / clip_seg %s do not match y %s"
                                 % (self.name, tuple(sums.shape), tuple(clip_seg.shape),
                                    tuple(y.shape)))
        step = self.chunk_clips(x.shape, y.shape,
                                residual.shape[-1] if residual is not None else 0)
        h3 = is_h3(cid)
        h3t = is_h3t(cid) or is_h3u(cid) or is_h3p(cid)
        for n0 in range(0, N, step):
            p = self.params(x, y, residual, n0, min(N, n0 + step), x6=x6 and not h3, h3=h3,
                            h3t=h3t)
            if h3t:
                _, _, s_in, s_out = self.h3t_buffers()
                aff = ((in_affine[0].data_ptr(), in_affine[1].data_ptr() + 4 * n0)
                       if in_affine is not None else (0, 0))
                launch, v = ((k.conv_h3u, cid - H3U_BASE) if is_h3u(cid)
                             else (k.conv_h3p, H3P_BPC[cid - H3P_BASE]) if is_h3p(cid)
                             else (k.conv_h3t, cid - H3T_BASE))
                if out_stats is not None:
                    launch(p, v, stream.cuda_stream, s_in, s_out,
                           out_stats[0].data_ptr(), out_stats[1].data_ptr() + 4 * n0,
                           out_stats[0].shape[2], *aff)
                else:
                    launch(p, v, stream.cuda_stream, s_in, s_out, 0, 0, 0, *aff)
            elif is_h3stem(cid):
                if in_affine is not None:
                    raise ValueError("%s: the stem kernel takes no input BN" % self.name)
                wx, bx, s_in, s_out = self.h3stem_buffers()
                p.w, p.bias = wx.data_ptr(), bx.data_ptr()
                p.K_pad, p.w_rows = 7 * 32, bx.shape[0]
                if out_stats is not None:
                    k.conv_h3stem(p, cid - H3STEM_BASE, stream.cuda_stream, s_in, s_out,
                                  out_stats[0].data_ptr(), out_stats[1].data_ptr() + 4 * n0,
                                  out_stats[0].shape[2])
                else:
                    k.conv_h3stem(p, cid - H3STEM_BASE, stream.cuda_stream, s_in, s_out)
            elif is_h3s(cid):
                if in_affine is not None:
                    raise ValueError("%s: the stride-2 row-band kernel takes no input BN"
                                     % self.name)
                _, _, s_in, s_out = self.h3d_buffers()
                if out_stats is not None:
                    k.conv_h3s(p, cid - H3S_BASE, stream.cuda_stream, s_in, s_out,
                               out_stats[0].data_ptr(), out_stats[1].data_ptr() + 4 * n0,
                               out_stats[0].shape[2])
                else:
                    k.conv_h3s(p, cid - H3S_BASE, stream.cuda_stream, s_in, s_out)
            elif is_h3r(cid):
                _, _, s_in, s_out = self.h3d_buffers()
                aff = ((in_affine[0].data_ptr(), in_affine[1].data_ptr() + 4 * n0)
                       if in_affine is not None else (0, 0))
                if out_stats is not None:
                    k.conv_h3r(p, cid - H3R_BASE, stream.cuda_stream, s_in, s_out,
                               out_stats[0].data_ptr(), out_stats[1].data_ptr() + 4 * n0,
                               out_stats[0].shape[2], *aff)
                else:
                    k.conv_h3r(p, cid - H3R_BASE, stream.cuda_stream, s_in, s_out, 0, 0, 0, *aff)
            elif h3:
                _, _, s_in, s_out = self.h3d_buffers()
                ks, ws = 1, None
                conf = cid - H3D_BASE
                if is_h3k(cid):
                    conf = H3K_CONFIGS[cid - H3K_BASE]
                    ks = self.ksplit_for(cid, x[n0:min(N, n0 + step)].shape)
                    ws = self.x6k_workspace(ks * p.M * self.geom.cout_p) if ks > 1 else None
                aff = ((in_affine[0].data_ptr(), in_affine[1].data_ptr() + 4 * n0)
                       if in_affine is not None else (0, 0))
                if out_stats is not None:
                    k.conv_h3(p, conf, stream.cuda_stream, s_in, s_out, out_stats[0].data_ptr(),
                              out_stats[1].data_ptr() + 4 * n0, out_stats[0].shape[2], ks,
                              ws.data_ptr() if ws is not None else 0, *aff)
                else:
                    k.conv_h3(p, conf, stream.cuda_stream, s_in, s_out, 0, 0, 0, ks,
                              ws.data_ptr() if ws is not None else 0, *aff)
            elif is_x6r(cid):
                if not self.wino_ok:
                    raise ValueError("%s: the row-band x6 kernel takes 1x3x3 stride-1 convs"
                                     % self.name)
                if out_stats is not None:
                    k.conv_x6r(p, cid - X6R_BASE, stream.cuda_stream, out_stats[0].data_ptr(),
                               out_stats[1].data_ptr() + 4 * n0, out_stats[0].shape[2])
                else:
                    k.conv_x6r(p, cid - X6R_BASE, stream.cuda_stream)
            elif is_x6k(cid):
                ks = self.ksplit_for(cid, x[n0:min(N, n0 + step)].shape)
                ws = self.x6k_workspace(ks * p.M * self.geom.cout_p) if ks > 1 else None
                if out_stats is not None:
                    k.conv_x6(p, X6K_CONFIGS[cid - X6K_BASE], stream.cuda_stream,
                              out_stats[0].data_ptr(), out_stats[1].data_ptr() + 4 * n0,
                              out_stats[0].shape[2], ks, ws.data_ptr() if ws is not None else 0)
                else:
                    k.conv_x6(p, X6K_CONFIGS[cid - X6K_BASE], stream.cuda_stream, 0, 0, 0, ks,
                              ws.data_ptr() if ws is not None else 0)
            elif x6 and out_stats is not None:
                k.conv_x6(p, cid - X6D_BASE, stream.cuda_stream, out_stats[0].data_ptr(),
                          out_stats[1].data_ptr() + 4 * n0, out_stats[0].shape[2])
            elif x6:
                k.conv_x6(p, cid - X6D_BASE, stream.cuda_stream)
            else:
                k.conv_f32(p, cid, stream.cuda_stream)

    def autotune(self, x: torch.Tensor, residual: Optional[torch.Tensor] = None,
                 reps: int = 3) -> int:
        from .native import kernels
        tkey = self._tune_key(x.shape, x.device)
        cached = tuning.get(tkey)
        if cached is not None and (cached < len(kernels().f32_configs) or
                                   cached in self.wino_ids or
                                   (is_h3(cached) and h3_enabled()) or
                                   (is_x6d(cached) and not is_h3(cached) and x6_enabled())):
            self._config[tuple(x.shape[:4])] = cached
            tuning.count("read")
            return cached
        tuning.count("tuned")
        y = torch.empty(self.out_shape(x.shape), dtype=torch.float32, device=x.device)
        stream = torch.cuda.current_stream(x.device)
        verbose = os.environ.get("RNB_TUNE_VERBOSE") == "1"
        cands, ost, aff = self.candidates(x.shape), None, None
        if self.tune_with_stats:
            cands = [c for c in cands if c in WINO_ALL or is_x6d(c)] or cands
            ost = (torch.zeros((1, 2, self.geom.cout_p), dtype=torch.float64, device=x.device),
                   torch.zeros(x.shape[0], dtype=torch.int32, device=x.device))
        if self.tune_with_affine:
            ok = [c for c in cands if self.affine_ok(c, x.shape)]
            if ok:
                cands = ok
                ss = torch.ones((1, 2, x.shape[-1]), dtype=torch.float32, device=x.device)
                ss[:, 1] = 0.0
                aff = (ss, torch.zeros(x.shape[0], dtype=torch.int32, device=x.device))
        def time_one(cid, n):
            o = ost if ost is not None and (cid in WINO_ALL or is_x6d(cid)) else None
            a = aff if aff is not None and self.affine_ok(cid, x.shape) else None
            self._launch_all(x, y, residual, cid, stream, in_affine=a, out_stats=o)
            start = torch.cuda.Event(enable_timing=True)
            end = torch.cuda.Event(enable_timing=True)
            start.record(stream)
            for _ in range(n):
                self._launch_all(x, y, residual, cid, stream, in_affine=a, out_stats=o)
            end.record(stream)
            end.synchronize()
            return start.elapsed_time(end) / n

        times = {}
        t0 = time_one(cands[0], reps)
        min_ms = float(os.environ.get("RNB_TUNE_MIN_MS", "0.5"))
        if min_ms > 0 and t0 > 0:
            reps = max(reps, min(64, int(math.ceil(min_ms / t0))))
        rounds = max(1, int(os.environ.get("RNB_TUNE_ROUNDS", "2")))
        for rnd in range(rounds):
            for cid in (cands if rnd % 2 == 0 else cands[::-1]):
                if verbose:
                    print("[tune] %s x=%s res=%s cid=%d" % (
                        self.name, tuple(x.shape), None if residual is None else
                        tuple(residual.shape), cid), flush=True)
                t = time_one(cid, reps)
                times[cid] = min(times.get(cid, t), t)
        best = min(cands, key=lambda c: times[c])
        self._config[tuple(x.shape[:4])] = best
        tuning.put(tkey, best)
        return best

    def emits_output_stats(self, x_shape) -> bool:
        cid = self.config_for(x_shape)
        return cid in WINO_ALL or is_x6d(cid)

    def takes_sums_affine(self, x_shape) -> bool:
        cid = self.config_for(x_shape)
        if not is_h3(cid) or is_h3w(cid) or is_h3t(cid) or is_h3u(cid) or is_h3p(cid) \
                or is_h3stem(cid) or is_h3s(cid) or is_h3r(cid):
            return False
        return self.affine_ok(cid, x_shape)

    def accepts_input_affine(self, x_shape) -> bool:
        return self.affine_ok(self.config_for(x_shape), x_shape)

    def forward_hip(self, x: torch.Tensor, residual: Optional[torch.Tensor] = None,
                    out: Optional[torch.Tensor] = None, config: Optional[int] = None,
                    in_affine=None, out_stats=None):
        if x.dtype != torch.float32 or not x.is_contiguous():
            raise ValueError("%s: expected contiguous fp32 NDHWC input" % self.name)
        y = out if out is not None else torch.empty(self.out_shape(x.shape),
                                                    dtype=torch.float32, device=x.device)
        if tuple(y.shape[:4]) != tuple(self.out_shape(x.shape)[:4]) or y.dtype != torch.float32:
            raise ValueError("%s: output %s does not match" % (self.name, tuple(y.shape)))
        if residual is not None:
            if residual.shape[:4] != y.shape[:4] or residual.dtype != torch.float32 \
                    or not residual.is_contiguous():
                raise ValueError("%s: residual %s does not match output %s"
                                 % (self.name, tuple(residual.shape), tuple(y.shape)))
        if x.shape[0] == 0:
            return y
        cid = self.config_for(x.shape) if config is None else config
        self._launch_all(x, y, residual, cid, torch.cuda.current_stream(x.device), in_affine,
                         out_stats)
        return y

    def forward_torch(self, x: torch.Tensor, residual: Optional[torch.Tensor] = None,
                      out_dtype=torch.float32):
        g = self.geom
        xin = x[..., :g.cin].float().permute(0, 4, 1, 2, 3)
        y = F.conv3d(xin, self.w_ref.to(x.device), self.b_ref.to(x.device),
                     stride=g.stride, padding=g.padding)
        y = y.permute(0, 2, 3, 4, 1)
        if residual is not None:
            y = y + residual[..., :g.cout].float()
        if self.relu:
            y = torch.relu(y)
        if g.cout_p != g.cout:
            y = F.pad(y, (0, g.cout_p - g.cout))
        return y.to(out_dtype).contiguous()
```

rnb_amd/ops/native.py:

```python
from __future__ import annotations

import ctypes
import os
import struct
import threading
from typing import Optional

_HERE = os.path.dirname(os.path.abspath(__file__))
NATIVE_DIR = os.path.join(os.path.dirname(_HERE), "_native")

_lock = threading.Lock()
_libs = {}


class NativeUnavailable(RuntimeError):
    pass


def _lib_path(name: str) -> str:
    return os.path.join(NATIVE_DIR, name)


def _load(name: str, build_if_missing: bool = True) -> ctypes.CDLL:
    with _lock:
# ... 189 lines not shown
        for base in ("rnb_jpeg_idct", "rnb_jpeg_huff", "rnb_jpeg_huff_subseq"):
            fn = getattr(lib, base + "_s")
            fn.argtypes = getattr(lib, base).argtypes[:-1] + [ctypes.c_int, ctypes.c_void_p]
            fn.restype = ctypes.c_int
        lib.rnb_jpeg_idct_r.argtypes = lib.rnb_jpeg_idct.argtypes[:-1] + \
            [ctypes.c_int, ctypes.c_int, ctypes.c_void_p]
        lib.rnb_jpeg_idct_r.restype = ctypes.c_int
        lib.rnb_preprocess.argtypes = [ctypes.c_void_p, ctypes.c_void_p, ctypes.c_longlong,
                                       ctypes.POINTER(ctypes.c_float),
                                       ctypes.POINTER(ctypes.c_float), ctypes.c_void_p]
        lib.rnb_stem_pack.argtypes = [ctypes.c_void_p, ctypes.c_void_p, ctypes.c_longlong,
                                      ctypes.c_int, ctypes.c_int, ctypes.c_void_p]
        lib.rnb_preprocess_packed.argtypes = [ctypes.c_void_p, ctypes.c_void_p,
                                              ctypes.c_longlong, ctypes.c_int, ctypes.c_int,
                                              ctypes.POINTER(ctypes.c_float),
                                              ctypes.POINTER(ctypes.c_float), ctypes.c_void_p]
        lib.rnb_head.argtypes = [ctypes.c_void_p, ctypes.c_void_p, ctypes.c_void_p,
                                 ctypes.c_void_p, ctypes.c_void_p, ctypes.c_int, ctypes.c_int,
                                 ctypes.c_int, ctypes.c_int, ctypes.c_int, ctypes.c_void_p]
        lib.rnb_bn_scratch_floats.argtypes = [ctypes.c_int, ctypes.c_int]
        lib.rnb_bn_scratch_floats.restype = ctypes.c_longlong
        lib.rnb_bn_stats.argtypes = [ctypes.c_void_p, ctypes.c_int, ctypes.c_int, ctypes.c_int,
                                     ctypes.c_void_p, ctypes.c_void_p, ctypes.c_void_p,
                                     ctypes.c_void_p]
        lib.rnb_bn_apply.argtypes = [ctypes.c_void_p, ctypes.c_void_p, ctypes.c_void_p,
                                     ctypes.c_void_p, ctypes.c_void_p, ctypes.c_void_p,
                                     ctypes.c_void_p, ctypes.c_float, ctypes.c_int,
                                     ctypes.c_longlong, ctypes.c_int, ctypes.c_int,
                                     ctypes.c_int, ctypes.c_int, ctypes.c_void_p]
        lib.rnb_bn_seg_bps.argtypes = [ctypes.c_int, ctypes.c_int, ctypes.c_longlong]
        lib.rnb_bn_seg_set_bps.argtypes = [ctypes.c_int]
        if os.environ.get("RNB_BN_BPS"):
            lib.rnb_bn_seg_set_bps(int(os.environ["RNB_BN_BPS"]))
        lib.rnb_bn_aff_arm.argtypes = [ctypes.c_void_p, ctypes.c_int, ctypes.c_void_p,
                                       ctypes.c_int, ctypes.c_int, ctypes.c_int, ctypes.c_void_p,
                                       ctypes.c_void_p, ctypes.c_float, ctypes.c_void_p]
        lib.rnb_bn_aff_arm.restype = ctypes.c_int
        lib.rnb_bn_aff_disarm.argtypes = []
        lib.rnb_bn_aff_disarm.restype = None
        lib.rnb_bn_aff_used.argtypes = []
        lib.rnb_bn_aff_used.restype = ctypes.c_int
        lib.rnb_bn_set_apply_blk.argtypes = [ctypes.c_int]
        lib.rnb_bn_set_apply_blk.restype = None
        if "RNB_BN_APPLY_BLK" in os.environ:
            lib.rnb_bn_set_apply_blk(int(os.environ["RNB_BN_APPLY_BLK"]))
        lib.rnb_bn_seg_set_fused_finalize.argtypes = [ctypes.c_int]
        if os.environ.get("RNB_BN_FUSED_FINALIZE"):
            lib.rnb_bn_seg_set_fused_finalize(int(os.environ["RNB_BN_FUSED_FINALIZE"]))
        lib.rnb_bn_seg_scratch_floats.argtypes = [ctypes.c_int, ctypes.c_int, ctypes.c_longlong]
        lib.rnb_bn_seg_scratch_floats.restype = ctypes.c_longlong
        lib.rnb_bn_seg_stats_f32.argtypes = [
            ctypes.c_void_p, ctypes.c_void_p, ctypes.c_int, ctypes.c_int, ctypes.c_longlong,
            ctypes.c_int, ctypes.c_int, ctypes.c_void_p, ctypes.c_longlong,
            ctypes.c_void_p, ctypes.c_void_p, ctypes.c_void_p, ctypes.c_float, ctypes.c_float,
            ctypes.c_int, ctypes.c_void_p, ctypes.c_void_p, ctypes.c_void_p, ctypes.c_void_p,
            ctypes.c_void_p, ctypes.c_void_p]
        lib.rnb_bn_seg_stats_from_sums_f32.argtypes = [
            ctypes.c_void_p, ctypes.c_int, ctypes.c_void_p, ctypes.c_int, ctypes.c_int,
            ctypes.c_int, ctypes.c_void_p, ctypes.c_void_p, ctypes.c_void_p, ctypes.c_float,
            ctypes.c_float, ctypes.c_int, ctypes.c_void_p, ctypes.c_void_p, ctypes.c_void_p,
            ctypes.c_void_p, ctypes.c_void_p, ctypes.c_void_p]
        lib.rnb_bn_seg_apply_f32.argtypes = [
            ctypes.c_void_p, ctypes.c_void_p, ctypes.c_void_p, ctypes.c_void_p, ctypes.c_int,
            ctypes.c_int, ctypes.c_void_p, ctypes.c_int, ctypes.c_longlong, ctypes.c_int,
            ctypes.c_int, ctypes.c_int, ctypes.c_int, ctypes.c_void_p]
        lib.rnb_bn_seg_apply_f32_ind.argtypes = (lib.rnb_bn_seg_apply_f32.argtypes[:-1]
                                                 + [ctypes.c_void_p, ctypes.c_void_p])
        lib.rnb_bn_seg_apply_sums_f32.argtypes = [
            ctypes.c_void_p, ctypes.c_void_p, ctypes.c_void_p, ctypes.c_void_p, ctypes.c_int,
            ctypes.c_int, ctypes.c_void_p, ctypes.c_int, ctypes.c_void_p, ctypes.c_void_p,
            ctypes.c_float, ctypes.c_int, ctypes.c_longlong, ctypes.c_int, ctypes.c_int,
            ctypes.c_int, ctypes.c_int, ctypes.c_void_p, ctypes.c_void_p]
        lib.rnb_bn_seg_ss_from_sums_f32.argtypes = [
            ctypes.c_void_p, ctypes.c_int, ctypes.c_void_p, ctypes.c_int, ctypes.c_int,
            ctypes.c_int, ctypes.c_void_p, ctypes.c_void_p, ctypes.c_float, ctypes.c_void_p,
            ctypes.c_void_p, ctypes.c_void_p, ctypes.c_void_p]
        lib.rnb_bn_seg_set_defer_running.argtypes = [ctypes.c_int]
        lib.rnb_bn_seg_set_defer_running.restype = None
        lib.rnb_bn_seg_defers_running.argtypes = [ctypes.c_int, ctypes.c_int]
        lib.rnb_bn_seg_running_batched.argtypes = [ctypes.c_void_p, ctypes.c_int, ctypes.c_int,
                                                   ctypes.c_void_p, ctypes.c_int, ctypes.c_void_p]
        self.bn_run_entry_size = lib.rnb_bn_seg_running_entry_size()
        lib.rnb_bn_seg_walk_apply_f32.argtypes = [
            ctypes.c_void_p, ctypes.c_int, ctypes.c_void_p, ctypes.c_void_p, ctypes.c_int,
            ctypes.c_int, ctypes.c_int, ctypes.c_void_p, ctypes.c_void_p, ctypes.c_float,
            ctypes.c_float, ctypes.c_int, ctypes.c_void_p, ctypes.c_void_p, ctypes.c_void_p,
            ctypes.c_void_p, ctypes.c_void_p, ctypes.c_void_p, ctypes.c_void_p, ctypes.c_void_p,
            ctypes.c_int, ctypes.c_longlong, ctypes.c_int, ctypes.c_int, ctypes.c_int,
            ctypes.c_void_p]
        lib.rnb_video_reduce.argtypes = [ctypes.c_void_p, ctypes.c_void_p, ctypes.c_void_p,
                                         ctypes.c_void_p, ctypes.c_int, ctypes.c_int,
                                         ctypes.c_void_p]
        lib.rnb_halo_launch_v.argtypes = [ctypes.POINTER(HaloParams), ctypes.c_int,
                                          ctypes.c_void_p]
        lib.rnb_halo_launch_v.restype = ctypes.c_int
        lib.rnb_halo_lds_bytes_v.argtypes = [ctypes.c_int] * 5
        lib.rnb_temporal_launch.argtypes = [ctypes.POINTER(TemporalParams), ctypes.c_int,
                                            ctypes.c_int, ctypes.c_void_p]
        lib.rnb_temporal_launch.restype = ctypes.c_int
        lib.rnb_temporal_lds_bytes.argtypes = [ctypes.c_int] * 3
        lib.rnb_conv21_launch.argtypes = [ctypes.POINTER(Conv21Params), ctypes.c_void_p]
        lib.rnb_conv21_launch.restype = ctypes.c_int
        lib.rnb_conv21s_launch.argtypes = [ctypes.POINTER(Conv21Params), ctypes.c_void_p]
        lib.rnb_conv21s_launch.restype = ctypes.c_int
        lib.rnb_conv21_supported.argtypes = [ctypes.c_int] * 3
        lib.rnb_conv21_fits.argtypes = [ctypes.c_int] * 6
        if lib.rnb_conv21_params_size() != ctypes.sizeof(Conv21Params):
            raise NativeUnavailable("Conv21Params layout mismatch: rebuild")
        if lib.rnb_temporal_params_size() != ctypes.sizeof(TemporalParams):
            raise NativeUnavailable("TemporalParams layout mismatch: rebuild")
        if lib.rnb_halo_params_size() != ctypes.sizeof(HaloParams):
            raise NativeUnavailable("HaloParams layout mismatch: rebuild")
        if lib.rnb_conv_params_size() != ctypes.sizeof(ConvParams):
            raise NativeUnavailable("ConvParams layout mismatch (%d vs %d): rebuild"
                                    % (lib.rnb_conv_params_size(),
                                       ctypes.sizeof(ConvParams)))
        lib.rnb_conv_f32_launch.argtypes = [ctypes.POINTER(ConvParams), ctypes.c_int,
                                            ctypes.c_void_p]
        lib.rnb_conv_f32_launch.restype = ctypes.c_int
        lib.rnb_conv_f32_config_info.argtypes = [ctypes.c_int, ctypes.POINTER(ctypes.c_int),
                                                 ctypes.POINTER(ctypes.c_int)]
        lib.rnb_conv_f32_max_bytes.restype = ctypes.c_longlong
        lib.rnb_conv_x6_launch.argtypes = [ctypes.POINTER(ConvParams), ctypes.c_int,
                                           ctypes.c_void_p]
        lib.rnb_conv_x6_launch.restype = ctypes.c_int
        lib.rnb_conv_x6_launch_stats.argtypes = [ctypes.POINTER(ConvParams), ctypes.c_int,
                                                 ctypes.c_void_p, ctypes.c_void_p,
                                                 ctypes.c_void_p, ctypes.c_int]
        lib.rnb_conv_x6_launch_stats.restype = ctypes.c_int
        lib.rnb_conv_x6_launch_splitk.argtypes = [ctypes.POINTER(ConvParams), ctypes.c_int,
                                                  ctypes.c_void_p, ctypes.c_void_p,
                                                  ctypes.c_void_p, ctypes.c_int, ctypes.c_int,
                                                  ctypes.c_void_p]
        lib.rnb_conv_x6_launch_splitk.restype = ctypes.c_int
        lib.rnb_conv_x6r_launch.argtypes = [ctypes.POINTER(ConvParams), ctypes.c_int,
                                            ctypes.c_void_p, ctypes.c_void_p,
                                            ctypes.c_void_p, ctypes.c_int]
        lib.rnb_conv_x6r_launch.restype = ctypes.c_int
        lib.rnb_conv_x6_config_info.argtypes = [ctypes.c_int, ctypes.POINTER(ctypes.c_int),
                                                ctypes.POINTER(ctypes.c_int)]
        lib.rnb_conv_h3_launch.argtypes = [ctypes.POINTER(ConvParams), ctypes.c_int,
                                           ctypes.c_void_p, ctypes.c_void_p, ctypes.c_void_p,
                                           ctypes.c_int, ctypes.c_int, ctypes.c_void_p,
                                           ctypes.c_float, ctypes.c_float, ctypes.c_void_p,
                                           ctypes.c_void_p]
        lib.rnb_conv_h3_launch.restype = ctypes.c_int
        lib.rnb_conv_h3_affine_ok.argtypes = [ctypes.c_int, ctypes.c_int, ctypes.c_int]
        lib.rnb_conv_h3_affine_ok.restype = ctypes.c_int
        lib.rnb_conv_h3r_launch.argtypes = [ctypes.POINTER(ConvParams), ctypes.c_int,
                                            ctypes.c_void_p, ctypes.c_void_p, ctypes.c_void_p,
                                            ctypes.c_int, ctypes.c_float, ctypes.c_float,
                                            ctypes.c_void_p, ctypes.c_void_p]
        lib.rnb_conv_h3r_launch.restype = ctypes.c_int
        lib.rnb_conv_h3r_band_rows.argtypes = [ctypes.c_int] * 3
        lib.rnb_conv_h3r_band_rows.restype = ctypes.c_int
        lib.rnb_conv_h3r_pixels.argtypes = [ctypes.c_int]
        lib.rnb_conv_h3r_pixels.restype = ctypes.c_int
        lib.rnb_conv_h3r_blocks.argtypes = [ctypes.c_int] * 6
        lib.rnb_conv_h3r_blocks.restype = ctypes.c_longlong
        lib.rnb_conv_h3r_stacked.argtypes = [ctypes.c_int] * 6
        lib.rnb_conv_h3r_stacked.restype = ctypes.c_int
        lib.rnb_conv_h3r_stack_small.argtypes = [ctypes.c_int]
        lib.rnb_conv_h3r_stack_small.restype = None
        lib.rnb_conv_h3r_occupancy.argtypes = [ctypes.c_int] * 2
        lib.rnb_conv_h3r_occupancy.restype = ctypes.c_int
        lib.rnb_conv_h3t_launch.argtypes = lib.rnb_conv_h3r_launch.argtypes
        lib.rnb_conv_h3t_launch.restype = ctypes.c_int
        lib.rnb_conv_h3t_pixels.argtypes = [ctypes.c_int, ctypes.c_int]
        lib.rnb_conv_h3t_blocks.argtypes = [ctypes.c_int] * 6
        lib.rnb_conv_h3t_blocks.restype = ctypes.c_longlong
        lib.rnb_conv_h3t_stacked.argtypes = [ctypes.c_int] * 6
        lib.rnb_conv_h3t_stacked.restype = ctypes.c_int
        lib.rnb_conv_h3t_form.argtypes = [ctypes.c_int]
        lib.rnb_conv_h3t_form.restype = None
        lib.rnb_conv_h3t_occupancy.argtypes = [ctypes.c_int] * 2
        lib.rnb_conv_h3t_occupancy.restype = ctypes.c_int
        self.exp = None
        exp_path = os.path.join(NATIVE_DIR, "exp", "librnb_h3exp.so")
        if os.path.exists(exp_path) and os.environ.get("RNB_EXP_KERNELS", "1") != "0":
            try:
                self.exp = ctypes.CDLL(exp_path)
            except OSError:
                self.exp = None
        if self.exp is not None:
            ex = self.exp
            ex.rnb_conv_h3u_launch.argtypes = lib.rnb_conv_h3r_launch.argtypes
            ex.rnb_conv_h3u_launch.restype = ctypes.c_int
            ex.rnb_conv_h3u_pixels.argtypes = [ctypes.c_int, ctypes.c_int]
            ex.rnb_conv_h3u_pixels.restype = ctypes.c_int
            ex.rnb_conv_h3s_launch.argtypes = [ctypes.POINTER(ConvParams), ctypes.c_int,
                                               ctypes.c_void_p, ctypes.c_void_p,
                                               ctypes.c_void_p, ctypes.c_int, ctypes.c_float,
                                               ctypes.c_float]
            ex.rnb_conv_h3s_launch.restype = ctypes.c_int
            ex.rnb_conv_h3s_rows.argtypes = [ctypes.c_int, ctypes.c_int, ctypes.c_int]
            ex.rnb_conv_h3s_rows.restype = ctypes.c_int
        lib.rnb_conv_h3stem_launch.argtypes = [ctypes.POINTER(ConvParams), ctypes.c_int,
                                               ctypes.c_void_p, ctypes.c_void_p,
                                               ctypes.c_void_p, ctypes.c_int, ctypes.c_float,
                                               ctypes.c_float]
        lib.rnb_conv_h3stem_launch.restype = ctypes.c_int
        lib.rnb_conv_h3stem_rows.argtypes = [ctypes.c_int, ctypes.c_int, ctypes.c_int]
        lib.rnb_conv_h3stem_rows.restype = ctypes.c_int
        lib.rnb_conv_h3p_launch.argtypes = [ctypes.POINTER(ConvParams), ctypes.c_int,
                                            ctypes.c_void_p, ctypes.c_void_p, ctypes.c_void_p,
                                            ctypes.c_int, ctypes.c_float, ctypes.c_float,
                                            ctypes.c_void_p, ctypes.c_void_p]
        lib.rnb_conv_h3p_launch.restype = ctypes.c_int
        lib.rnb_conv_h3p_ok.argtypes = [ctypes.c_int] * 5
        lib.rnb_conv_h3p_ok.restype = ctypes.c_int
        lib.rnb_conv_h3w_launch.argtypes = [ctypes.c_void_p, ctypes.c_int, ctypes.c_void_p,
                                            ctypes.c_float, ctypes.c_float, ctypes.c_void_p]
        lib.rnb_conv_h3w_launch.restype = ctypes.c_int
        lib.rnb_conv_h3w_tc.argtypes = [ctypes.c_int]
        lib.rnb_conv_h3w_tc.restype = ctypes.c_int
        lib.rnb_h3_set_range_flag.argtypes = [ctypes.c_void_p]
        lib.rnb_h3_set_range_flag.restype = None
        lib.rnb_conv_h3t_pixels.restype = ctypes.c_int
        lib.rnb_conv_h3_config_info.argtypes = [ctypes.c_int, ctypes.POINTER(ctypes.c_int),
                                                ctypes.POINTER(ctypes.c_int)]
        lib.rnb_preprocess_f32.argtypes = [ctypes.c_void_p, ctypes.c_void_p, ctypes.c_longlong,
                                           ctypes.POINTER(ctypes.c_float),
                                           ctypes.POINTER(ctypes.c_float), ctypes.c_void_p]
        lib.rnb_head_f32.argtypes = [ctypes.c_void_p, ctypes.c_void_p, ctypes.c_void_p,
                                     ctypes.c_void_p, ctypes.c_void_p, ctypes.c_int,
                                     ctypes.c_int, ctypes.c_int, ctypes.c_int, ctypes.c_int,
                                     ctypes.c_void_p]
        lib.rnb_wino_f32_launch.argtypes = [ctypes.POINTER(WinoParams), ctypes.c_int,
                                            ctypes.c_void_p]
        lib.rnb_wino_f32_launch.restype = ctypes.c_int
        lib.rnb_winot_f32_launch.argtypes = [ctypes.POINTER(WinoParams), ctypes.c_int,
                                             ctypes.c_void_p]
        lib.rnb_winot_f32_launch.restype = ctypes.c_int
        for fn in (lib.rnb_wino_x6_launch, lib.rnb_winot_x6_launch):
            fn.argtypes = [ctypes.POINTER(WinoParams), ctypes.c_int, ctypes.c_void_p]
            fn.restype = ctypes.c_int
        if lib.rnb_wino_params_size() != ctypes.sizeof(WinoParams):
            raise NativeUnavailable("WinoParams layout mismatch: rebuild")
        if lib.rnb_conv_f32_params_size() != ctypes.sizeof(ConvParams):
            raise NativeUnavailable("ConvF32Params layout mismatch: rebuild")
        self.f32_configs = []
        for i in range(lib.rnb_conv_f32_num_configs()):
            p, c = ctypes.c_int(), ctypes.c_int()
            lib.rnb_conv_f32_config_info(i, ctypes.byref(p), ctypes.byref(c))
            self.f32_configs.append((p.value, c.value))
        self.f32_max_bytes = lib.rnb_conv_f32_max_bytes()
        self.x6r_variants = lib.rnb_conv_x6r_num_variants()
        self.h3r_variants = lib.rnb_conv_h3r_num_variants()
        self.h3t_variants = lib.rnb_conv_h3t_num_variants()
        self.h3w_variants = lib.rnb_conv_h3w_num_variants()
        self.h3u_variants = self.exp.rnb_conv_h3u_num_variants() if self.exp else 0
        self.h3s_variants = self.exp.rnb_conv_h3s_num_variants() if self.exp else 0
        self.h3stem_variants = lib.rnb_conv_h3stem_num_variants()
        self.x6_configs = []
        for i in range(lib.rnb_conv_x6_num_configs()):
            p, c = ctypes.c_int(), ctypes.c_int()
            lib.rnb_conv_x6_config_info(i, ctypes.byref(p), ctypes.byref(c))
            self.x6_configs.append((p.value, c.value))
        self.h3_configs = []
        for i in range(lib.rnb_conv_h3_num_configs()):
            p, c = ctypes.c_int(), ctypes.c_int()
            lib.rnb_conv_h3_config_info(i, ctypes.byref(p), ctypes.byref(c))
            self.h3_configs.append((p.value, c.value))
        self.configs = []
        self.stages = []
        for i in range(lib.rnb_conv_num_configs()):
            p, c = ctypes.c_int(), ctypes.c_int()
            lib.rnb_conv_config_info(i, ctypes.byref(p), ctypes.byref(c))
            self.configs.append((p.value, c.value))
            self.stages.append(lib.rnb_conv_config_stages(i))

    def conv(self, params: ConvParams, config_id: int, stream: int) -> None:
        _check(self.lib.rnb_conv_launch(ctypes.byref(params), config_id, stream),
               "conv (config %d)" % config_id)

    def conv_f32(self, params: ConvParams, config_id: int, stream: int) -> None:
        _check(self.lib.rnb_conv_f32_launch(ctypes.byref(params), config_id, stream),
               "conv_f32 (config %d)" % config_id)

    def conv_x6(self, params: ConvParams, config_id: int, stream: int, sums: int = 0,
                clip_seg: int = 0, stats_c: int = 0, ksplit: int = 1, ws: int = 0) -> None:
        _check(self.lib.rnb_conv_x6_launch_splitk(ctypes.byref(params), config_id, stream,
                                                  sums or None, clip_seg or None, stats_c,
                                                  ksplit, ws or None),
               "conv_x6 (config %d, ksplit %d)" % (config_id, ksplit))

    def conv_h3(self, params: ConvParams, config_id: int, stream: int, in_scale: float,
                out_scale: float, sums: int = 0, clip_seg: int = 0, stats_c: int = 0,
                ksplit: int = 1, ws: int = 0, in_ss: int = 0, in_seg: int = 0) -> None:
        _check(self.lib.rnb_conv_h3_launch(ctypes.byref(params), config_id, stream,
                                           sums or None, clip_seg or None, stats_c, ksplit,
                                           ws or None, in_scale, out_scale, in_ss or None,
                                           in_seg or None),
               "conv_h3 (config %d, ksplit %d)" % (config_id, ksplit))

    def bn_aff_arm(self, sums, sums_c, coffs, nseg, rpc, C, gamma, beta, eps, ss) -> None:
        _check(self.lib.rnb_bn_aff_arm(sums, sums_c, coffs, nseg, rpc, C, gamma, beta, eps, ss),
               "bn_aff_arm")

    def bn_aff_disarm(self) -> None:
        self.lib.rnb_bn_aff_disarm()

    def bn_aff_used(self) -> bool:
        return bool(self.lib.rnb_bn_aff_used())

    def bn_set_apply_blk(self, on: bool) -> None:
        self.lib.rnb_bn_set_apply_blk(1 if on else 0)

    def h3_set_range_flag(self, dev_ptr: int) -> None:
        self.lib.rnb_h3_set_range_flag(dev_ptr or None)

    def conv_h3r(self, params: ConvParams, variant: int, stream: int, in_scale: float,
                 out_scale: float, sums: int = 0, clip_seg: int = 0, stats_c: int = 0,
                 in_ss: int = 0, in_seg: int = 0) -> None:
        _check(self.lib.rnb_conv_h3r_launch(ctypes.byref(params), variant, stream,
                                            sums or None, clip_seg or None, stats_c, in_scale,
                                            out_scale, in_ss or None, in_seg or None),
               "conv_h3r (variant %d)" % variant)

    def conv_h3r_band_rows(self, variant: int, H: int, W: int) -> int:
        return self.lib.rnb_conv_h3r_band_rows(variant, H, W)

    def conv_h3r_pixels(self, variant: int) -> int:
        return self.lib.rnb_conv_h3r_pixels(variant)

    def conv_h3r_blocks(self, variant: int, N: int, T: int, H: int, W: int, cout_p: int) -> int:
        return self.lib.rnb_conv_h3r_blocks(variant, N, T, H, W, cout_p)

    def conv_h3r_stacked(self, variant: int, N: int, T: int, H: int, W: int,
                         cout_p: int) -> bool:
        return bool(self.lib.rnb_conv_h3r_stacked(variant, N, T, H, W, cout_p))

    def conv_h3r_stack_small(self, on: bool) -> None:
        self.lib.rnb_conv_h3r_stack_small(1 if on else 0)

    def conv_h3r_occupancy(self, variant: int, stacked: bool) -> int:
        return self.lib.rnb_conv_h3r_occupancy(variant, 1 if stacked else 0)

    def conv_h3t(self, params: ConvParams, variant: int, stream: int, in_scale: float,
                 out_scale: float, sums: int = 0, clip_seg: int = 0, stats_c: int = 0,
                 in_ss: int = 0, in_seg: int = 0) -> None:
        _check(self.lib.rnb_conv_h3t_launch(ctypes.byref(params), variant, stream,
                                            sums or None, clip_seg or None, stats_c, in_scale,
                                            out_scale, in_ss or None, in_seg or None),
               "conv_h3t (variant %d)" % variant)

    def conv_h3u(self, params: ConvParams, variant: int, stream: int, in_scale: float,
                 out_scale: float, sums: int = 0, clip_seg: int = 0, stats_c: int = 0,
                 in_ss: int = 0, in_seg: int = 0) -> None:
        _check(self.exp.rnb_conv_h3u_launch(ctypes.byref(params), variant, stream,
                                            sums or None, clip_seg or None, stats_c, in_scale,
                                            out_scale, in_ss or None, in_seg or None),
               "conv_h3u (variant %d)" % variant)

    def conv_h3s(self, params: ConvParams, variant: int, stream: int, in_scale: float,
                 out_scale: float, sums: int = 0, clip_seg: int = 0, stats_c: int = 0) -> None:
        _check(self.exp.rnb_conv_h3s_launch(ctypes.byref(params), variant, stream,
                                            sums or None, clip_seg or None, stats_c, in_scale,
                                            out_scale),
               "conv_h3s (variant %d)" % variant)

    def conv_h3stem(self, params: ConvParams, variant: int, stream: int, in_scale: float,
                    out_scale: float, sums: int = 0, clip_seg: int = 0, stats_c: int = 0) -> None:
        _check(self.lib.rnb_conv_h3stem_launch(ctypes.byref(params), variant, stream,
                                               sums or None, clip_seg or None, stats_c, in_scale,
                                               out_scale),
               "conv_h3stem (variant %d)" % variant)

    def conv_h3p(self, params: ConvParams, blocks_per_cu: int, stream: int, in_scale: float,
                 out_scale: float, sums: int = 0, clip_seg: int = 0, stats_c: int = 0,
                 in_ss: int = 0, in_seg: int = 0) -> None:
        _check(self.lib.rnb_conv_h3p_launch(ctypes.byref(params), blocks_per_cu, stream,
                                            sums or None, clip_seg or None, stats_c, in_scale,
                                            out_scale, in_ss or None, in_seg or None),
               "conv_h3p (%d blocks per CU)" % blocks_per_cu)

    def conv_h3w(self, params: "WinoParams", variant: int, stream: int, in_scale: float,
                 out_scale: float, out_seg: int = 0) -> None:
        _check(self.lib.rnb_conv_h3w_launch(ctypes.byref(params), variant, stream, in_scale,
                                            out_scale, out_seg or None),
               "conv_h3w (variant %d)" % variant)

    def conv_h3w_tc(self, variant: int) -> int:
        return int(self.lib.rnb_conv_h3w_tc(variant))

    def conv_h3p_ok(self, T: int, H: int, W: int, Cin_p: int, Cout_p: int) -> bool:
        return bool(self.lib.rnb_conv_h3p_ok(T, H, W, Cin_p, Cout_p))

    def conv_h3stem_rows(self, variant: int, Ho: int, Wo: int) -> int:
        return int(self.lib.rnb_conv_h3stem_rows(variant, Ho, Wo))

    def conv_h3s_rows(self, variant: int, Ho: int, Wo: int) -> int:
        return int(self.exp.rnb_conv_h3s_rows(variant, Ho, Wo)) if self.exp else 0

    def conv_h3u_pixels(self, variant: int, T: int) -> int:
        return int(self.exp.rnb_conv_h3u_pixels(variant, T)) if self.exp else 0

    def conv_h3t_pixels(self, variant: int, T: int) -> int:
        return int(self.lib.rnb_conv_h3t_pixels(variant, T))

    def conv_h3t_blocks(self, variant: int, N: int, T: int, H: int, W: int, cout_p: int) -> int:
        return int(self.lib.rnb_conv_h3t_blocks(variant, N, T, H, W, cout_p))

    def conv_h3t_stacked(self, variant: int, N: int, T: int, H: int, W: int,
                         cout_p: int) -> bool:
        return bool(self.lib.rnb_conv_h3t_stacked(variant, N, T, H, W, cout_p))

    def conv_h3t_form(self, mode: int) -> None:
        self.lib.rnb_conv_h3t_form(mode)

    def conv_h3t_occupancy(self, variant: int, stacked: bool) -> int:
        return self.lib.rnb_conv_h3t_occupancy(variant, 1 if stacked else 0)

    def conv_h3_affine_ok(self, config_id: int, cin_p: int, rows_per_clip: int) -> bool:
        return bool(self.lib.rnb_conv_h3_affine_ok(config_id, cin_p, rows_per_clip))

    def conv_x6r(self, params: ConvParams, variant: int, stream: int, sums: int = 0,
                 clip_seg: int = 0, stats_c: int = 0) -> None:
        _check(self.lib.rnb_conv_x6r_launch(ctypes.byref(params), variant, stream,
                                            sums or None, clip_seg or None, stats_c),
               "conv_x6r (variant %d)" % variant)

    def wino_f32(self, params: "WinoParams", variant: int, stream: int) -> None:
        _check(self.lib.rnb_wino_f32_launch(ctypes.byref(params), variant, stream),
               "conv_wino_f32 (variant %d)" % variant)

    def winot_f32(self, params: "WinoParams", variant: int, stream: int) -> None:
        _check(self.lib.rnb_winot_f32_launch(ctypes.byref(params), variant, stream),
               "conv_winot_f32 (variant %d)" % variant)

    def wino_x6(self, params: "WinoParams", variant: int, stream: int) -> None:
        _check(self.lib.rnb_wino_x6_launch(ctypes.byref(params), variant, stream),
               "conv_wino_x6 (variant %d)" % variant)

    def winot_x6(self, params: "WinoParams", variant: int, stream: int) -> None:
        _check(self.lib.rnb_winot_x6_launch(ctypes.byref(params), variant, stream),
               "conv_winot_x6 (variant %d)" % variant)

    def preprocess_f32(self, in_ptr, out_ptr, npix, mean, std, stream):
        m = (ctypes.c_float * 3)(*mean)
        s = (ctypes.c_float * 3)(*std)
        _check(self.lib.rnb_preprocess_f32(in_ptr, out_ptr, npix, m, s, stream),
               "preprocess_f32")

    def head_f32(self, x_ptr, w_ptr, b_ptr, out_ptr, pooled_ptr, N, S, C, Cs, ncls, stream):
        _check(self.lib.rnb_head_f32(x_ptr, w_ptr, b_ptr, out_ptr, pooled_ptr, N, S, C, Cs,
                                     ncls, stream), "head_f32")

    def halo(self, params: HaloParams, stream: int, variant: int = 2) -> None:
        _check(self.lib.rnb_halo_launch_v(ctypes.byref(params), variant, stream), "conv_halo")

    def temporal(self, params: TemporalParams, num_cus: int, blocks_per_cu: int,
                 stream: int) -> None:
        _check(self.lib.rnb_temporal_launch(ctypes.byref(params), num_cus, blocks_per_cu,
                                            stream), "conv_temporal")

    def conv21(self, params: Conv21Params, stream: int, variant: int = 1) -> None:
        fn = self.lib.rnb_conv21s_launch if variant == 1 else self.lib.rnb_conv21_launch
        _check(fn(ctypes.byref(params), stream), "conv21 (variant %d)" % variant)

    def conv21_supported(self, T: int, H: int, W: int) -> bool:
        return bool(self.lib.rnb_conv21_supported(T, H, W))

    def conv21_fits(self, N: int, T: int, H: int, W: int, y_stride: int = 64,
                    res_stride: int = 64) -> bool:
        return bool(self.lib.rnb_conv21_fits(N, T, H, W, y_stride, res_stride))

    def temporal_lds_bytes(self, T: int, cin_p: int, cout_p: int) -> int:
        return self.lib.rnb_temporal_lds_bytes(T, cin_p, cout_p)

    def halo_lds_bytes(self, frames: int, H: int, W: int, cin: int, variant: int = 2) -> int:
        return self.lib.rnb_halo_lds_bytes_v(frames, H, W, cin, variant)
# ... 512 lines not shown
```

Baseline: 1726.

## Fuse residual add, BN and ReLU into the h3r/h3q conv input load

Adds a RES template path to the h3r and h3q conv kernels. While staging its input halo, the kernel applies the deferred block BN affine, adds the residual tensor and applies ReLU, and writes the block output to a side buffer (only from the first channel tile). This replaces a separate BN-apply-with-residual pass over memory before the next conv. The engine enables it by default for eligible consumers, and the autotuner times candidates with the fused path. In exchange, the staging loop issues extra residual loads and side stores, and the load batch size is smaller, which may cost latency hiding or registers.

New measurement: 1736 (median of 6 runs). No clear change (+0.6%).

```diff
diff --git a/csrc/conv_h3.hip b/csrc/conv_h3.hip
--- a/csrc/conv_h3.hip
+++ b/csrc/conv_h3.hip
@@ -364,10 +364,11 @@
   if constexpr (ON) asm volatile("" : "+v"(v));
   return v;
 }
-template <bool STK, bool AFF>
+template <bool STK, bool AFF, bool RES = false>
 static __device__ __forceinline__ void h3_patch_entry(const ConvF32Params& p, const H3Band& bd,
                                                       int it, int npx, int W2, int qd, int n0,
-                                                      uint32_t& src, int& dst) {
+                                                      uint32_t& src, int& dst, bool side = false,
+                                                      int clip_lo = 0, int clip_hi = 0) {
   const int H = p.H, W = p.W;
   const int q = it >> 2;
   const int hy = q / W2, hx = q - hy * W2;
@@ -386,6 +387,16 @@
   dst = it < 4 * npx ? q * 128 : -1;
   if constexpr (STK && AFF) {
     if (ok) dst |= (f32_fast_div(fy, p.mTo, p.sTo) - n0) << 17;
+  }
+  if constexpr (RES) {
+    if (ok) {
+      const int g = fy * H + y - (bd.f * H + bd.r0);
+      const int clip = f32_fast_div(fy, p.mTo, p.sTo);
+      if (side && g >= 0 && g < bd.rows) dst |= 1;
+      if (clip < clip_lo || clip >= clip_hi) dst |= 2;
+    } else if (it < 4 * npx) {
+      dst |= 2;
+    }
   }
 }
 template <bool STK>
@@ -440,9 +451,10 @@
 }
 
 template <int NW, int TP, int TC, int HALO_PX, int G, bool ST, bool AFF, int MINB = 1,
-          bool STK = false>
+          bool STK = false, bool RES = false>
 __global__ __launch_bounds__(64 * NW, MINB)
 void conv_h3r_kernel(const ConvF32Params p, const X6DStats st) {
+  static_assert(!RES || AFF, "the residual on load comes with the input BN");
   constexpr int P_TILE = NW * TP * 16, C_TILE = TC * 16;
   constexpr int HALO_BYTES = HALO_PX * 128;
   constexpr int W_BYTES = C_TILE * 128;
@@ -491,14 +503,25 @@
   int dst[ITEMS];
   static_assert(HALO_BYTES <= 1 << 17, "dst packs the entry's clip above bit 17");
   [[maybe_unused]] const int n0 = f32_fast_div(f, p.mTo, p.sTo);
+  [[maybe_unused]] __amdgpu_buffer_rsrc_t rr = xr, yr = xr;
+  [[maybe_unused]] int clip_lo = 0, clip_hi = 0;
+  if constexpr (RES) {
+    rr = __builtin_amdgcn_make_buffer_rsrc((void*)st.in_res, (short)0, p.x_bytes, 0x00020000);
+    yr = __builtin_amdgcn_make_buffer_rsrc((void*)st.y_side, (short)0, p.x_bytes, 0x00020000);
+    clip_lo = st.res_coffs[0];
+    clip_hi = st.res_coffs[st.res_nseg];
+  }
 #pragma unroll
   for (int i = 0; i < ITEMS; ++i) {
-    h3_patch_entry<STK, AFF>(p, bd, threadIdx.x + i * NT, npx, W2, qd, n0, src[i], dst[i]);
+    h3_patch_entry<STK, AFF, RES>(p, bd, threadIdx.x + i * NT, npx, W2, qd, n0, src[i], dst[i],
+                                  ctile == 0, clip_lo, clip_hi);
   }
   const float* ssv = nullptr;
   if constexpr (AFF) ssv = st.in_ss + (size_t)st.in_seg[f / p.T] * 2 * p.Cin_p + qd * 4;
   const float in_scale = st.in_scale;
-  constexpr int SB = MINB >= 4 ? 1 : AFF ? (NW > 8 ? 1 : (TP >= 4 ? 3 : ITEMS)) : ITEMS;
+  constexpr int SB = MINB >= 4 ? 1
+                     : AFF     ? (NW > 8 ? 1 : (TP >= 4 ? (RES ? 2 : 3) : (RES ? 3 : ITEMS)))
+                               : ITEMS;
   auto stage = [&](int chunk, auto mix) {
     constexpr bool MIX = decltype(mix)::value;
     x6f32x4 sc0, sh0, sc1, sh1;
@@ -512,27 +535,46 @@
 #pragma unroll
     for (int i0 = 0; i0 < ITEMS; i0 += SB) {
     x6f32x4 v0[SB], v1[SB];
+    [[maybe_unused]] x6f32x4 r0[RES ? SB : 1], r1[RES ? SB : 1];
 #pragma unroll
     for (int k = 0; k < SB; ++k) {
       const int i = min(i0 + k, ITEMS - 1);
       const uint32_t o = src[i] == X6D_INVALID ? X6D_INVALID : src[i] + (uint32_t)(chunk * 128);
       v0[k] = __builtin_amdgcn_raw_buffer_load_b128(xr, o, 0, 0);
       v1[k] = __builtin_amdgcn_raw_buffer_load_b128(xr, o == X6D_INVALID ? o : o + 64u, 0, 0);
+      if constexpr (RES) {
+        r0[k] = __builtin_amdgcn_raw_buffer_load_b128(rr, o, 0, 0);
+        r1[k] = __builtin_amdgcn_raw_buffer_load_b128(rr, o == X6D_INVALID ? o : o + 64u, 0, 0);
+      }
     }
 #pragma unroll
     for (int k = 0; k < SB; ++k) {
       const int i = i0 + k;
       if (i >= ITEMS || dst[i] < 0) continue;
-      const int d = h3_per_chunk<STK && AFF>(dst[i]), q = (d >> 7) & 1023;
+      const int d = h3_per_chunk<(STK && AFF) || RES>(dst[i]), q = (d >> 7) & 1023;
       x6f32x4 a0 = v0[k], a1 = v1[k];
       if constexpr (AFF) {
         const float m = src[i] == X6D_INVALID ? 0.f : in_scale;
         if constexpr (MIX) h3_entry_ss(p, st, n0, d, qd, chunk, sc0, sc1, sh0, sh1);
+        if constexpr (RES) {
+          const bool pad = (d & 2) != 0;
+#pragma unroll
+          for (int j = 0; j < 4; ++j) {
+            a0[j] = pad ? 0.f : fmaxf(fmaf(a0[j], sc0[j], sh0[j]) + r0[k][j], 0.f);
+            a1[j] = pad ? 0.f : fmaxf(fmaf(a1[j], sc1[j], sh1[j]) + r1[k][j], 0.f);
+          }
+          const uint32_t so = (d & 1) ? src[i] + (uint32_t)(chunk * 128) : X6D_INVALID;
+          __builtin_amdgcn_raw_buffer_store_b128(a0, yr, so, 0, 0);
+          __builtin_amdgcn_raw_buffer_store_b128(a1, yr, so == X6D_INVALID ? so : so + 64u, 0, 0);
+          a0 *= in_scale;
+          a1 *= in_scale;
+        } else {
 #pragma unroll
         for (int j = 0; j < 4; ++j) {
           a0[j] = fmaxf(fmaf(a0[j], sc0[j], sh0[j]), 0.f) * m;
           a1[j] = fmaxf(fmaf(a1[j], sc1[j], sh1[j]), 0.f) * m;
         }
+        }
       } else {
         a0 *= in_scale;
         a1 *= in_scale;
@@ -540,7 +582,7 @@
       uint32_t h[4], l[4];
       h3_split4(a0, h, l);
       h3_split4(a1, h + 2, l + 2);
-      char* base = lds + (d & 0x1FFFF);
+      char* base = lds + (d & 0x1FF80);
       *(wu32x4*)(base + (x6r_swz(2 * qd, q) << 4)) = (wu32x4){h[0], h[1], h[2], h[3]};
       *(wu32x4*)(base + (x6r_swz(2 * qd + 1, q) << 4)) = (wu32x4){l[0], l[1], l[2], l[3]};
     }
@@ -624,9 +666,11 @@
   H3_PHASE(15);
 }
 
-template <int NW, int TP, int HALO_PX, int G, int MINB, bool ST, bool AFF, bool STK = false>
+template <int NW, int TP, int HALO_PX, int G, int MINB, bool ST, bool AFF, bool STK = false,
+          bool RES = false>
 __global__ __launch_bounds__(64 * NW, MINB)
 void conv_h3q_kernel(const ConvF32Params p, const X6DStats st) {
+  static_assert(!RES || AFF, "the residual on load comes with the input BN");
   constexpr int TC = 9;
   constexpr int P_TILE = NW * TP * 16, C_TILE = TC * 16;
   constexpr int HALO_BYTES = HALO_PX * 128;
@@ -676,14 +720,23 @@
   int dst[ITEMS];
   static_assert(HALO_BYTES <= 1 << 17, "dst packs the entry's clip above bit 17");
   [[maybe_unused]] const int n0 = f32_fast_div(f, p.mTo, p.sTo);
+  [[maybe_unused]] __amdgpu_buffer_rsrc_t rr = xr, yr = xr;
+  [[maybe_unused]] int clip_lo = 0, clip_hi = 0;
+  if constexpr (RES) {
+    rr = __builtin_amdgcn_make_buffer_rsrc((void*)st.in_res, (short)0, p.x_bytes, 0x00020000);
+    yr = __builtin_amdgcn_make_buffer_rsrc((void*)st.y_side, (short)0, p.x_bytes, 0x00020000);
+    clip_lo = st.res_coffs[0];
+    clip_hi = st.res_coffs[st.res_nseg];
+  }
 #pragma unroll
   for (int i = 0; i < ITEMS; ++i) {
-    h3_patch_entry<STK, AFF>(p, bd, threadIdx.x + i * NT, npx, W2, qd, n0, src[i], dst[i]);
+    h3_patch_entry<STK, AFF, RES>(p, bd, threadIdx.x + i * NT, npx, W2, qd, n0, src[i], dst[i],
+                                  ctile == 0, clip_lo, clip_hi);
   }
   const float* ssv = nullptr;
   if constexpr (AFF) ssv = st.in_ss + (size_t)st.in_seg[f / p.T] * 2 * p.Cin_p + qd * 4;
   const float in_scale = st.in_scale;
-  constexpr int SB = AFF ? (NW == 4 && MINB == 1 ? 5 : 2) : 5;
+  constexpr int SB = AFF ? (NW == 4 && MINB == 1 ? (RES ? 3 : 5) : 2) : 5;
   auto stage = [&](int chunk, auto mix) {
     constexpr bool MIX = decltype(mix)::value;
     x6f32x4 sc0, sh0, sc1, sh1;
@@ -697,27 +750,46 @@
 #pragma unroll
     for (int i0 = 0; i0 < ITEMS; i0 += SB) {
       x6f32x4 v0[SB], v1[SB];
+      [[maybe_unused]] x6f32x4 r0[RES ? SB : 1], r1[RES ? SB : 1];
 #pragma unroll
       for (int k = 0; k < SB; ++k) {
         const int i = min(i0 + k, ITEMS - 1);
         const uint32_t o = src[i] == X6D_INVALID ? X6D_INVALID : src[i] + (uint32_t)(chunk * 128);
         v0[k] = __builtin_amdgcn_raw_buffer_load_b128(xr, o, 0, 0);
         v1[k] = __builtin_amdgcn_raw_buffer_load_b128(xr, o == X6D_INVALID ? o : o + 64u, 0, 0);
+        if constexpr (RES) {
+          r0[k] = __builtin_amdgcn_raw_buffer_load_b128(rr, o, 0, 0);
+          r1[k] = __builtin_amdgcn_raw_buffer_load_b128(rr, o == X6D_INVALID ? o : o + 64u, 0, 0);
+        }
       }
 #pragma unroll
       for (int k = 0; k < SB; ++k) {
         const int i = i0 + k;
         if (i >= ITEMS || dst[i] < 0) continue;
-        const int d = h3_per_chunk<STK && AFF>(dst[i]), q = (d >> 7) & 1023;
+        const int d = h3_per_chunk<(STK && AFF) || RES>(dst[i]), q = (d >> 7) & 1023;
         x6f32x4 a0 = v0[k], a1 = v1[k];
         if constexpr (AFF) {
           const float m = src[i] == X6D_INVALID ? 0.f : in_scale;
           if constexpr (MIX) h3_entry_ss(p, st, n0, d, qd, chunk, sc0, sc1, sh0, sh1);
+          if constexpr (RES) {
+            const bool pad = (d & 2) != 0;
+#pragma unroll
+            for (int j = 0; j < 4; ++j) {
+              a0[j] = pad ? 0.f : fmaxf(fmaf(a0[j], sc0[j], sh0[j]) + r0[k][j], 0.f);
+              a1[j] = pad ? 0.f : fmaxf(fmaf(a1[j], sc1[j], sh1[j]) + r1[k][j], 0.f);
+            }
+            const uint32_t so = (d & 1) ? src[i] + (uint32_t)(chunk * 128) : X6D_INVALID;
+            __builtin_amdgcn_raw_buffer_store_b128(a0, yr, so, 0, 0);
+            __builtin_amdgcn_raw_buffer_store_b128(a1, yr, so == X6D_INVALID ? so : so + 64u, 0, 0);
+            a0 *= in_scale;
+            a1 *= in_scale;
+          } else {
 #pragma unroll
           for (int j = 0; j < 4; ++j) {
             a0[j] = fmaxf(fmaf(a0[j], sc0[j], sh0[j]), 0.f) * m;
             a1[j] = fmaxf(fmaf(a1[j], sc1[j], sh1[j]), 0.f) * m;
           }
+          }
         } else {
           a0 *= in_scale;
           a1 *= in_scale;
@@ -725,7 +797,7 @@
         uint32_t h[4], l[4];
         h3_split4(a0, h, l);
         h3_split4(a1, h + 2, l + 2);
-        char* base = lds + (d & 0x1FFFF);
+        char* base = lds + (d & 0x1FF80);
         *(wu32x4*)(base + (x6r_swz(2 * qd, q) << 4)) = (wu32x4){h[0], h[1], h[2], h[3]};
         *(wu32x4*)(base + (x6r_swz(2 * qd + 1, q) << 4)) = (wu32x4){l[0], l[1], l[2], l[3]};
       }
@@ -1505,6 +1577,28 @@
     H3QCFG_PF(8, 4, 640, 2, 1),
 };
 
+struct ConvH3RRes {
+  ConvH3RKernel kernel[2], stacked[2];
+};
+#define H3RRES(NW, TP, HALO, G)                                                    \
+  {{conv_h3r_kernel<NW, TP, 9, HALO, G, false, true, 1, false, true>,              \
+    conv_h3r_kernel<NW, TP, 9, HALO, G, true, true, 1, false, true>},              \
+   {conv_h3r_kernel<NW, TP, 9, HALO, G, false, true, 1, true, true>,               \
+    conv_h3r_kernel<NW, TP, 9, HALO, G, true, true, 1, true, true>}}
+#define H3QRES(NW, TP, HALO, HSTK, G, MINB)                                        \
+  {{conv_h3q_kernel<NW, TP, HALO, G, MINB, false, true, false, true>,              \
+    conv_h3q_kernel<NW, TP, HALO, G, MINB, true, true, false, true>},              \
+   {conv_h3q_kernel<NW, TP, HSTK, G, MINB, false, true, true, true>,               \
+    conv_h3q_kernel<NW, TP, HSTK, G, MINB, true, true, true, true>}}
+#define H3RRES_NONE {{nullptr, nullptr}, {nullptr, nullptr}}
+static const ConvH3RRes kH3RRes[] = {
+    H3RRES(7, 4, 600, 1), H3RRES_NONE, H3RRES(7, 3, 480, 1),
+    H3RRES(7, 4, 600, 2), H3RRES_NONE, H3RRES(7, 3, 480, 2),
+    H3QRES(4, 7, 600, 600, 2, 1), H3QRES(4, 4, 344, 352, 1, 2), H3RRES_NONE,
+};
+static_assert(sizeof(kH3RRes) / sizeof(kH3RRes[0]) == sizeof(kH3RConfigs) / sizeof(kH3RConfigs[0]),
+              "one RES entry per variant");
+
 int rnb_conv_h3r_num_variants() { return (int)(sizeof(kH3RConfigs) / sizeof(kH3RConfigs[0])); }
 
 static long long h3r_round_blocks(int variant) {
@@ -1585,9 +1679,17 @@
   return e == hipSuccess ? nb : -(int)e;
 }
 
-int rnb_conv_h3r_launch(const ConvF32Params* pp, int variant, hipStream_t stream, double* sums,
-                        const int* clip_seg, int stats_c, float in_scale, float out_scale,
-                        const float* in_ss, const int* in_seg) {
+int rnb_conv_h3r_res_ok(int variant, int stacked) {
+  if (variant < 0 || variant >= rnb_conv_h3r_num_variants()) return 0;
+  const ConvH3RRes& r = kH3RRes[variant];
+  return (stacked ? r.stacked[0] && r.stacked[1] : r.kernel[0] && r.kernel[1]) ? 1 : 0;
+}
+
+static int h3r_launch(const ConvF32Params* pp, int variant, hipStream_t stream, double* sums,
+                      const int* clip_seg, int stats_c, float in_scale, float out_scale,
+                      const float* in_ss, const int* in_seg, const float* in_res,
+                      long long res_rows, int res_stride, float* y_side, const int* res_coffs,
+                      int res_nseg) {
   if (variant < 0 || variant >= rnb_conv_h3r_num_variants()) return -1;
   ConvF32Params p = *pp;
   const ConvH3RConfig& cfg = kH3RConfigs[variant];
@@ -1632,9 +1734,36 @@
   st.in_seg = in_seg;
   st.oflag = g_h3_range_flag;
   const int kid = (sums ? 1 : 0) + (in_ss ? 2 : 0);
-  hipLaunchKernelGGL(stacked ? cfg.stacked[kid] : cfg.kernel[kid], dim3((unsigned)blocks),
-                     dim3(64 * cfg.nw), 0, stream, p, st);
+  ConvH3RKernel kernel = stacked ? cfg.stacked[kid] : cfg.kernel[kid];
+  if (in_res) {
+    if (!in_ss || !y_side || !res_coffs || res_nseg < 1) return -16;
+    if (!rnb_conv_h3r_res_ok(variant, stacked ? 1 : 0)) return -17;
+    if (res_stride != p.Cin_p || res_rows != (long long)p.N * p.T * p.H * p.W) return -19;
+    st.in_res = in_res;
+    st.y_side = y_side;
+    st.res_coffs = res_coffs;
+    st.res_nseg = res_nseg;
+    kernel = stacked ? kH3RRes[variant].stacked[sums ? 1 : 0] : kH3RRes[variant].kernel[sums ? 1 : 0];
+  }
+  hipLaunchKernelGGL(kernel, dim3((unsigned)blocks), dim3(64 * cfg.nw), 0, stream, p, st);
   return (int)hipGetLastError();
+}
+
+int rnb_conv_h3r_launch(const ConvF32Params* pp, int variant, hipStream_t stream, double* sums,
+                        const int* clip_seg, int stats_c, float in_scale, float out_scale,
+                        const float* in_ss, const int* in_seg) {
+  return h3r_launch(pp, variant, stream, sums, clip_seg, stats_c, in_scale, out_scale, in_ss,
+                    in_seg, nullptr, 0, 0, nullptr, nullptr, 0);
+}
+
+int rnb_conv_h3r_launch_res(const ConvF32Params* pp, int variant, hipStream_t stream,
+                            double* sums, const int* clip_seg, int stats_c, float in_scale,
+                            float out_scale, const float* in_ss, const int* in_seg,
+                            const float* in_res, long long res_rows, int res_stride,
+                            float* y_side, const int* res_coffs, int res_nseg) {
+  if (!in_res) return -16;
+  return h3r_launch(pp, variant, stream, sums, clip_seg, stats_c, in_scale, out_scale, in_ss,
+                    in_seg, in_res, res_rows, res_stride, y_side, res_coffs, res_nseg);
 }
 
 struct ConvH3TConfig {
diff --git a/csrc/x6d_common.h b/csrc/x6d_common.h
--- a/csrc/x6d_common.h
+++ b/csrc/x6d_common.h
@@ -50,6 +50,10 @@
   float in_scale, out_scale, acc_scale;
   const float* in_ss;
   const int* in_seg;
+  const float* in_res = nullptr;
+  float* y_side = nullptr;
+  const int* res_coffs = nullptr;
+  int res_nseg = 0;
   int* oflag = nullptr;
   BnAffSums aff = {};
 };
diff --git a/rnb_amd/models/r2p1d/engine.py b/rnb_amd/models/r2p1d/engine.py
--- a/rnb_amd/models/r2p1d/engine.py
+++ b/rnb_amd/models/r2p1d/engine.py
@@ -141,6 +141,10 @@
         self.head: Optional[Head] = None
         self._n = 0
         self.fused_choices: Dict[str, Optional[int]] = {}
+        self._res_on_load = True
+        self._res_consumers: List[ConvLayerF32] = []
+        self.fused_block_bn = 0
+        self.block_bn_applies = 0
         if backend == "module":
             self.module = net.to(device)
             self.module.train(bn_mode == "batch")
@@ -284,6 +288,41 @@
             for i, ok in enumerate(self._defer_ok):
                 if ok and not getattr(self.ops[i + 1].layer, "winot_ok", False):
                     self.ops[i + 1].layer.tune_with_affine = True
+        res_reader = {}
+        for j, op in enumerate(self.ops):
+            if op.res is not None and op.bn is not None:
+                res_reader.setdefault(op.res, j)
+        self._res_defer_ok = [
+            i + 1 < len(self.ops) and op.bn is not None and op.bn_relu and op.res is not None
+            and self.f32 and uses.get(op.dst, 0) == 2 and self.ops[i + 1].src == op.dst
+            and res_reader.get(op.dst, -1) > i + 1
+            for i, op in enumerate(self.ops)]
+        self._h3_defer = h3_defer
+        for i, ok in enumerate(self._res_defer_ok):
+            layer = self.ops[i + 1].layer if ok else None
+            if ok and isinstance(layer, ConvLayerF32) and layer.h3r_ok():
+                self._res_consumers.append(layer)
+        self.res_on_load = self._res_on_load
+
+    @property
+    def res_on_load(self) -> bool:
+        return self._res_on_load
+
+    @res_on_load.setter
+    def res_on_load(self, on: bool) -> None:
+        self._res_on_load = bool(on)
+        for layer in self._res_consumers:
+            if layer.tune_with_residual != self._res_on_load:
+                layer.tune_with_residual = self._res_on_load
+                layer._config.clear()
+                layer._res_untuned.clear()
+
+    def free_plan(self, fused=()) -> List[List[str]]:
+        plan = [list(names) for names in self._free_after]
+        for i in sorted(fused):
+            plan[i + 1] = plan[i + 1] + plan[i] + [self.ops[i].dst + ".z"]
+            plan[i] = []
+        return plan
 
     @property
     def in_channels_p(self) -> int:
@@ -425,6 +464,9 @@
         aff_max = min(2304, int(os.environ.get("RNB_BN_AFF_SUMS_MAX", "2304"))) if hip else 0
         aff_videos = int(os.environ.get("RNB_BN_AFF_SUMS_VIDEOS", "1"))
         pending_aff = None
+        pending_res = None
+        carry = []
+        res_defer = defer and self._res_on_load and self._h3_defer and h3_enabled()
         from ...ops.native import kernels as _kn
 
         def consume(fn):
@@ -464,6 +506,10 @@
                     if pending is not None:
                         kw["in_affine"] = pending
                         pending = None
+                    if pending_res is not None:
+                        src = pending_res[0]
+                        kw["in_residual"] = pending_res[1:]
+                        pending_res = None
                     sums = None
                     if (self.f32 and stats_fuse
                             and op.layer.emits_output_stats(src.shape)):
@@ -476,10 +522,20 @@
                         coffs = torch.tensor([0, x.shape[0]], dtype=torch.int32,
                                              device=x.device)
                     y = consume(lambda: op.layer.forward_hip(src, None, **kw))
+                    kw = None
                     thw = y.shape[1] * y.shape[2] * y.shape[3]
                     deferred = (defer and self._defer_ok[i] and self.f32
                                 and self.ops[i + 1].layer.accepts_input_affine(y.shape))
-                    if deferred:
+                    if (hip and res_defer and self._res_defer_ok[i] and res is not None
+                            and self.ops[i + 1].layer.accepts_input_residual(y.shape)):
+                        if clip_seg is None:
+                            clip_seg = self._clip_segments(coffs, x.shape[0], x.device)
+                        pending = (op.bn.scale_shift_f32(y, coffs, sums, rpc=thw), clip_seg)
+                        pending_res = (y, res, torch.empty_like(y), coffs)
+                        y = pending_res[2]
+                        carry = list(free_after[i])
+                        self.fused_block_bn += 1
+                    elif deferred:
                         if clip_seg is None:
                             clip_seg = self._clip_segments(coffs, x.shape[0], x.device)
                         if (sums is not None and aff_max > 0 and bn_mod._RUN_SINK[0] is not None
@@ -494,6 +550,8 @@
                             pending = (op.bn.scale_shift_f32(y, coffs, sums, rpc=thw), clip_seg)
                     else:
                         ind = out_indirect if i == len(self.ops) - 1 else None
+                        if res is not None:
+                            self.block_bn_applies += 1
                         from ...ops import bn as bn_mod
                         if (sums is not None and bn_mod._RUN_SINK[0] is not None
                                 and os.environ.get("RNB_BN_APPLY_SUMS", "1") != "0"):
@@ -520,8 +578,11 @@
                 y = op.layer.forward_torch(src, res, out_dtype=self.dtype)
             bufs[op.dst] = y
             del src, res
-            for name in free_after[i]:
+            if pending_res is not None and pending_res[2] is y:
+                continue
+            for name in free_after[i] + carry:
                 bufs.pop(name, None)
+            carry = []
         return bufs[self.out_name], coffs
 
     __call__ = forward
diff --git a/rnb_amd/ops/conv_f32.py b/rnb_amd/ops/conv_f32.py
--- a/rnb_amd/ops/conv_f32.py
+++ b/rnb_amd/ops/conv_f32.py
@@ -371,6 +371,8 @@
         self.k16 = pad_to(self.k_total, 16)
         self.tune_with_stats = False
         self.tune_with_affine = False
+        self.tune_with_residual = False
+        self._res_untuned = set()
         self._x6d = None
         self._h3d = None
         self._h3t = None
@@ -749,9 +751,10 @@
                 best, best_cost = cid, cost
         return best
 
-    def _tune_key(self, x_shape, device) -> str:
+    def _tune_key(self, x_shape, device, plain: bool = False) -> str:
         kind = ("f32st" if self.tune_with_stats else "f32") + \
-            ("aff" if self.tune_with_affine else "")
+            ("aff" if self.tune_with_affine else "") + \
+            ("affres" if self.tune_with_residual and not plain else "")
         return tuning.make_key(kind, self.geom, tuple(x_shape[:4]), _device_name(device))
 
     def config_for(self, x_shape) -> int:
@@ -776,6 +779,12 @@
             if cid is None:
                 N, T, H, W, _ = x_shape
                 cid = tuning.nearest(tkey, N * T * H * W)
+            if cid is None and self.tune_with_residual:
+                self._res_untuned.add(key)
+                tkey = self._tune_key(x_shape, self.device, plain=True)
+                cid = tuning.get(tkey)
+                if cid is None:
+                    cid = tuning.nearest(tkey, N * T * H * W)
             if cid is not None and cid in WINO_ALL and cid not in self.wino_ids:
                 cid = None
             if cid is not None and is_x6d(cid) and not is_h3(cid) and not x6_enabled():
@@ -870,10 +879,45 @@
         To, Ho, Wo = self.geom.out_thw(T, H, W)
         return kernels().conv_h3_affine_ok(conf, self.geom.cin_p, To * Ho * Wo)
 
-    def _launch_all(self, x, y, residual, cid, stream, in_affine=None, out_stats=None):
+    def residual_on_load_ok(self, cid: int, x_shape) -> bool:
+        if not is_h3r(cid) or not self.h3r_ok(x_shape):
+            return False
+        from .native import kernels
+        k = kernels()
+        N, T, H, W, _ = x_shape
+        v = cid - H3R_BASE
+        if not self.h3r_fits(v, x_shape, efficient=False):
+            return False
+        if self.chunk_clips(x_shape, self.out_shape(x_shape)) < N:
+            return False
+        return k.conv_h3r_res_ok(v, k.conv_h3r_stacked(v, N, T, H, W, self.geom.cout_p))
+
+    def accepts_input_residual(self, x_shape) -> bool:
+        if not self.tune_with_residual:
+            return False
+        cid = self.config_for(x_shape)
+        if tuple(x_shape[:4]) in self._res_untuned:
+            return False
+        return self.residual_on_load_ok(cid, x_shape)
+
+    def _launch_all(self, x, y, residual, cid, stream, in_affine=None, out_stats=None,
+                    in_residual=None):
         from .native import kernels
         k = kernels()
         N = x.shape[0]
+        if in_residual is not None:
+            r, y_side, coffs = in_residual
+            if in_affine is None or not self.residual_on_load_ok(cid, x.shape):
+                raise ValueError("%s: config %d has no residual-on-load form for x %s"
+                                 % (self.name, cid, tuple(x.shape)))
+            if (r.dtype != torch.float32 or not r.is_contiguous() or r.dim() != 5
+                    or y_side.shape != x.shape or y_side.dtype != torch.float32
+                    or not y_side.is_contiguous() or coffs.dtype != torch.int32
+                    or coffs.numel() < 2 or not coffs.is_contiguous()):
+                raise ValueError("%s: input residual %s / side output %s / clip offsets %s do "
+                                 "not match x %s" % (self.name, tuple(r.shape),
+                                                     tuple(y_side.shape), tuple(coffs.shape),
+                                                     tuple(x.shape)))
         if cid in WINO_ALL:
             step = self.chunk_clips(x.shape, y.shape,
                                     residual.shape[-1] if residual is not None else 0)
@@ -966,7 +1010,14 @@
                 _, _, s_in, s_out = self.h3d_buffers()
                 aff = ((in_affine[0].data_ptr(), in_affine[1].data_ptr() + 4 * n0)
                        if in_affine is not None else (0, 0))
-                if out_stats is not None:
+                if in_residual is not None:
+                    r, y_side, coffs = in_residual
+                    ost = ((out_stats[0].data_ptr(), out_stats[1].data_ptr(),
+                            out_stats[0].shape[2]) if out_stats is not None else (0, 0, 0))
+                    k.conv_h3r_res(p, cid - H3R_BASE, stream.cuda_stream, s_in, s_out, *ost,
+                                   *aff, r.data_ptr(), r.numel() // r.shape[-1], r.shape[-1],
+                                   y_side.data_ptr(), coffs.data_ptr(), coffs.numel() - 1)
+                elif out_stats is not None:
                     k.conv_h3r(p, cid - H3R_BASE, stream.cuda_stream, s_in, s_out,
                                out_stats[0].data_ptr(), out_stats[1].data_ptr() + 4 * n0,
                                out_stats[0].shape[2], *aff)
@@ -1026,6 +1077,7 @@
                                    (is_h3(cached) and h3_enabled()) or
                                    (is_x6d(cached) and not is_h3(cached) and x6_enabled())):
             self._config[tuple(x.shape[:4])] = cached
+            self._res_untuned.discard(tuple(x.shape[:4]))
             tuning.count("read")
             return cached
         tuning.count("tuned")
@@ -1044,15 +1096,46 @@
                 ss = torch.ones((1, 2, x.shape[-1]), dtype=torch.float32, device=x.device)
                 ss[:, 1] = 0.0
                 aff = (ss, torch.zeros(x.shape[0], dtype=torch.int32, device=x.device))
+        res_on = None
+        if self.tune_with_residual:
+            C, rows = x.shape[-1], x.numel() // x.shape[-1]
+            ss1 = torch.ones((1, 2, C), dtype=torch.float32, device=x.device)
+            ss1[:, 1] = 0.0
+            sums1 = torch.zeros((1, 2, C), dtype=torch.float64, device=x.device)
+            sums1[:, 1] = float(rows)
+            res_on = {
+                "aff": (ss1, torch.zeros(x.shape[0], dtype=torch.int32, device=x.device)),
+                "r": torch.zeros_like(x), "y_side": torch.empty_like(x),
+                "coffs": torch.tensor([0, x.shape[0]], dtype=torch.int32, device=x.device),
+                "sums": sums1, "gamma": torch.ones(C, dtype=torch.float32, device=x.device),
+                "beta": torch.zeros(C, dtype=torch.float32, device=x.device),
+                "rpc": rows // x.shape[0]}
+
+        def launch_one(cid, o, a):
+            if res_on is None:
+                self._launch_all(x, y, residual, cid, stream, in_affine=a, out_stats=o)
+            elif self.residual_on_load_ok(cid, x.shape):
+                self._launch_all(x, y, residual, cid, stream, in_affine=res_on["aff"],
+                                 out_stats=o, in_residual=(res_on["r"], res_on["y_side"],
+                                                           res_on["coffs"]))
+            else:
+                C = x.shape[-1]
+                kernels().bn_seg_apply_sums_f32(
+                    x.data_ptr(), x.data_ptr(), res_on["r"].data_ptr(),
+                    res_on["coffs"].data_ptr(), 1, res_on["rpc"], res_on["sums"].data_ptr(), C,
+                    res_on["gamma"].data_ptr(), res_on["beta"].data_ptr(), 1e-5, 1,
+                    x.numel() // C, C, C, C, C, stream.cuda_stream, None)
+                self._launch_all(x, y, residual, cid, stream, in_affine=a, out_stats=o)
+
         def time_one(cid, n):
             o = ost if ost is not None and (cid in WINO_ALL or is_x6d(cid)) else None
             a = aff if aff is not None and self.affine_ok(cid, x.shape) else None
-            self._launch_all(x, y, residual, cid, stream, in_affine=a, out_stats=o)
+            launch_one(cid, o, a)
             start = torch.cuda.Event(enable_timing=True)
             end = torch.cuda.Event(enable_timing=True)
             start.record(stream)
             for _ in range(n):
-                self._launch_all(x, y, residual, cid, stream, in_affine=a, out_stats=o)
+                launch_one(cid, o, a)
             end.record(stream)
             end.synchronize()
             return start.elapsed_time(end) / n
@@ -1072,7 +1155,9 @@
                 t = time_one(cid, reps)
                 times[cid] = min(times.get(cid, t), t)
         best = min(cands, key=lambda c: times[c])
+        self.last_tune_times = dict(times)
         self._config[tuple(x.shape[:4])] = best
+        self._res_untuned.discard(tuple(x.shape[:4]))
         tuning.put(tkey, best)
         return best
 
@@ -1092,7 +1177,7 @@
 
     def forward_hip(self, x: torch.Tensor, residual: Optional[torch.Tensor] = None,
                     out: Optional[torch.Tensor] = None, config: Optional[int] = None,
-                    in_affine=None, out_stats=None):
+                    in_affine=None, out_stats=None, in_residual=None):
         if x.dtype != torch.float32 or not x.is_contiguous():
             raise ValueError("%s: expected contiguous fp32 NDHWC input" % self.name)
         y = out if out is not None else torch.empty(self.out_shape(x.shape),
@@ -1108,7 +1193,7 @@
             return y
         cid = self.config_for(x.shape) if config is None else config
         self._launch_all(x, y, residual, cid, torch.cuda.current_stream(x.device), in_affine,
-                         out_stats)
+                         out_stats, in_residual)
         return y
 
     def forward_torch(self, x: torch.Tensor, residual: Optional[torch.Tensor] = None,
diff --git a/rnb_amd/ops/native.py b/rnb_amd/ops/native.py
--- a/rnb_amd/ops/native.py
+++ b/rnb_amd/ops/native.py
@@ -365,6 +365,12 @@
                                             ctypes.c_int, ctypes.c_float, ctypes.c_float,
                                             ctypes.c_void_p, ctypes.c_void_p]
         lib.rnb_conv_h3r_launch.restype = ctypes.c_int
+        lib.rnb_conv_h3r_launch_res.argtypes = lib.rnb_conv_h3r_launch.argtypes + [
+            ctypes.c_void_p, ctypes.c_longlong, ctypes.c_int, ctypes.c_void_p, ctypes.c_void_p,
+            ctypes.c_int]
+        lib.rnb_conv_h3r_launch_res.restype = ctypes.c_int
+        lib.rnb_conv_h3r_res_ok.argtypes = [ctypes.c_int, ctypes.c_int]
+        lib.rnb_conv_h3r_res_ok.restype = ctypes.c_int
         lib.rnb_conv_h3r_band_rows.argtypes = [ctypes.c_int] * 3
         lib.rnb_conv_h3r_band_rows.restype = ctypes.c_int
         lib.rnb_conv_h3r_pixels.argtypes = [ctypes.c_int]
@@ -531,6 +537,22 @@
                                             out_scale, in_ss or None, in_seg or None),
                "conv_h3r (variant %d)" % variant)
 
+    def conv_h3r_res(self, params: ConvParams, variant: int, stream: int, in_scale: float,
+                     out_scale: float, sums: int, clip_seg: int, stats_c: int, in_ss: int,
+                     in_seg: int, in_res: int, res_rows: int, res_stride: int, y_side: int,
+                     coffs: int, nseg: int, check: bool = True) -> int:
+        rc = self.lib.rnb_conv_h3r_launch_res(ctypes.byref(params), variant, stream,
+                                              sums or None, clip_seg or None, stats_c, in_scale,
+                                              out_scale, in_ss or None, in_seg or None,
+                                              in_res or None, res_rows, res_stride,
+                                              y_side or None, coffs or None, nseg)
+        if check:
+            _check(rc, "conv_h3r_res (variant %d)" % variant)
+        return rc
+
+    def conv_h3r_res_ok(self, variant: int, stacked: bool) -> bool:
+        return bool(self.lib.rnb_conv_h3r_res_ok(variant, 1 if stacked else 0))
+
     def conv_h3r_band_rows(self, variant: int, H: int, W: int) -> int:
         return self.lib.rnb_conv_h3r_band_rows(variant, H, W)
 
```
